# WHU-USI3DV/LaneMapping

Hardware: AMD Instinct MI355X
Metric: BEV tiles/sec end-to-end (LAS points -> polylines) (higher is better)
Workload: dtype f32; 1 GPU; on-GPU LAS->BEV raster (4,194,304 points/tile resident in HBM) + configs/Proj_polyline_fpn_vit_vertex_2.py, batch=16 per GPU, seeded random weights; lines_per_tile=45, streams=2, hip_graphs=True, points=resident, stream_check=not run (--full runs it), gather_check=n/a (1 rank), raster_check=not run (--full runs it), dist_ranks=1, rccl_ranks=1

## Files before the change

### include/lanemap_hip.h

```cpp
#ifndef LANEMAP_HIP_H
#define LANEMAP_HIP_H
#include <stdint.h>
#ifdef __cplusplus
extern "C" {
#endif

enum { LM_OK = 0, LM_ERR_ARG = 1, LM_ERR_HIP = 2, LM_ERR_NO_DEVICE = 3, LM_ERR_CAPACITY = 4 };
enum { LM_ACT_NONE = 0, LM_ACT_RELU = 1, LM_ACT_GELU = 2 };

int lm_abi_version(void);
const char* lm_last_error(void);
int lm_device_count(void);

int lm_conv2d_nhwc_mfma_f32(void* stream, const float* x, int ldx, const float* wp, int CoutP,
                            const float* scale, const float* shift, const float* res, int ldr, int res_rows,
                            float* y, int ldy, int B, int H, int W, int Cin, int Cout, int KH, int KW,
                            int stride, int pad_h, int pad_w, int dil, int act);
int lm_conv2d_nhwc_mfma_resup_f32(void* stream, const float* x, int ldx, const float* wp, int CoutP, const float* scale,
                                  const float* shift, const float* res_coarse, int ldr, int Hr, int Wr, float* y, int ldy,
                                  int B, int H, int W, int Cin, int Cout, int KH, int KW, int stride, int pad_h, int pad_w,
                                  int dil, int act);

int lm_winograd44_supported(int H, int W, int Cin, int dil);
int lm_winograd44_gn_chunks(int H, int W, int dil);
long lm_winograd44_tiles(int B, int H, int W, int dil);
long lm_winograd44_twin_workspace_bytes(int B, int H, int W, int Cin, int CoutP, int dil);
int lm_conv3x3_winograd44_f32(void* stream, const float* x, int ldx, const float* wu_frag, int CoutP, const float* scale,
                              const float* shift, const float* res, int ldr, float* y, int ldy, int B, int H, int W,
                              int Cin, int Cout, int dil, int act, double* gn_partial);
int lm_conv3x3_winograd44_twin_f32(void* stream, const float* x, int ldx, const float* wu, int CoutP, const float* scale,
                                   const float* shift, const float* res, int ldr, float* y, int ldy, int B, int H, int W,
                                   int Cin, int Cout, int dil, int act, void* workspace, long workspace_bytes);
int lm_wino44_split_fragments(void* stream, const float* frag, float* out, long n_quads);
int lm_conv3x3_winograd44_split_f32(void* stream, const float* x, int ldx, const float* wu_split, int CoutP, const float* scale,
                                    const float* shift, const float* res, int ldr, float* y, int ldy, int B, int H, int W,
                                    int Cin, int Cout, int dil, int act, double* gn_partial, float post);
int lm_conv3x3_winograd44_split_twin_f32(void* stream, const float* x, int ldx, const float* wu, int CoutP, const float* scale,
                                         const float* shift, const float* res, int ldr, float* y, int ldy, int B, int H, int W,
                                         int Cin, int Cout, int dil, int act, void* workspace, long workspace_bytes, float post);

int lm_conv2d_nhwc_mfma_f32_gnstats(void* stream, const float* x, int ldx, const float* wp, int CoutP, const float* shift,
                                    float* y, int ldy, double* gn_partial, int B, int H, int W, int Cin, int Cout,
                                    int KH, int KW, int stride, int pad_h, int pad_w, int dil);
int lm_gn_finalize(void* stream, const double* partial, float* stats, int B, int HW, int C, int nchunk, float eps);
int lm_gn_finalize_split(void* stream, const double* partial, float* stats, int B, int HW, int C, int nchunk, float eps, int split);

int lm_stem_conv7x7_bn_relu(void* stream, const float* x_chw, const float* w_k64, const float* scale,
                            const float* shift, float* y_nhwc, int B, int H, int W);
int lm_stem_conv7x7_bn_relu_u8(void* stream, const unsigned char* x_hwc3, const float* w_k64, const float* scale,
                               const float* shift, float* y_nhwc, int B, int H, int W);
int lm_maxpool3x3s2_nhwc(void* stream, const float* x, float* y, int B, int H, int W, int C);
int lm_conv2d_nhwc_small(void* stream, const float* x, int ldx, const float* w_tc16, const float* scale,
                         const float* shift, float* y, int ldy, int B, int H, int W, int Cin, int Cout,
                         int KH, int KW, int stride, int pad_h, int pad_w, int pre_relu, int act);

int lm_gn_stats(void* stream, const float* x, double* workspace, float* stats, int B, int HW, int C, float eps);
long lm_gn_stats_workspace_bytes(int B, int HW, int C);
int lm_gn_relu_upsample(void* stream, const float* x, const float* stats, const float* gamma, const float* beta,
                        float* y, int B, int Hi, int Wi, int Ho, int Wo, int C, int accumulate);
int lm_gn_relu_upsample_sum(void* stream, int n, const float* const* x, const float* const* stats, const int* Hi, const int* Wi,
                            const int* ldx , const float* gamma, const float* beta,
                            float* y, int B, int Ho, int Wo, int C);
int lm_gn_relu_upsample_sum_conv1x1(void* stream, int n, const float* const* x, const float* const* stats, const int* Hi, const int* Wi,
                                    const int* ldx, const float* gamma, const float* beta, float* y, int B, int Ho, int Wo, int C,
                                    const float* w_c16, const float* bias, int cout, float* y1, int ldy1);
int lm_upsample_bilinear_nhwc(void* stream, const float* x, int ldx, const float* add, int lda, float* y, int ldy,
                              int B, int Hi, int Wi, int Ho, int Wo, int C);
int lm_upsample_bilinear_to_chw(void* stream, const float* x, int ldx, float* y_chw, int B, int Hi, int Wi,
                                int Ho, int Wo, int C);
int lm_layernorm_rows(void* stream, const float* x, const float* gamma, const float* beta, float* y,
                      long rows, int D, float eps);
int lm_unpatchify(void* stream, const float* tokens, float* y_nhwc, int B, int G, int P, int C);
int lm_token_mix_mfma_f32(void* stream, const float* x, const float* wt, int ldw, const float* bias, const float* res, float* y,
                          int B, int M, int K, int N, int act);

int lm_attention_f32(void* stream, const float* qkv, float* out, int B, int N, int heads, int dim_head, float scale);
int lm_attention_masked_f32(void* stream, const float* qkv, float* out, const int* valid, int B, int N, int heads, int dim_head, float scale);

int lm_head_tokens(void* stream, const float* seg, const float* row_nhwc16, float* tok, float seg_bias,
                   int B, int P, int Hr, int Wr, int prop_width, int half_buff);
int lm_head_tokens_window(void* stream, const float* row_nhwc16, float* tok, int B, int P, int Hr, int Wr, int prop_width, int half_buff);
int lm_head_stage2(void* stream, const float* hid, int ldh, int D, const float* w2, const float* b2,
                   float* ext2, float* cls2, float* off2, long M);
int lm_head_proposal_conf(void* stream, const float* tok, const float* wt, const float* bias, float* conf,
                          int BP, int L);

int lm_decode_proposals(void* stream, const float* pconf, const float* ext2, const float* cls2, const float* off2,
                        float* prop_conf, float* v_ext, float* cls_conf, int* cls_idx, double* cls_offset,
                        int B, int P, int R, float exist_thre, int prop_width, int half_buff);
int lm_decode_orient(void* stream, const float* x_nhwc, int ldx, int C, unsigned char* y, long pixels);
int lm_decode_semantic(void* stream, const float* logit_chw3, unsigned char* sem, float* biseg, float* rows,
                       int B, int H, int W, float thre, int raw_mode);
long lm_endp_topk_workspace_bytes(int B);
int lm_endp_topk(void* stream, const float* endp_logit, void* workspace, int* out_idx, float* out_score,
                 int* out_status, int B, int H, int W, int clip, int K);

int lm_pack_segments(void* stream, int n, const void* const* src, const long* bytes, const long* dst_offsets, void* dst);


typedef struct {
    float quat[4];
    float trans[3];
    float bev_img_offset[2];
    float img_reso[2];
    float local_min_ele;
    float ele_reso;
    float inten_lo, inten_hi;
} LmRasterParams;
long lm_bev_raster_workspace_bytes(int B, long max_points_per_tile, int H, int W);
int lm_bev_raster_batch(void* stream, const float* points_xyzi, const long* tile_offsets, const LmRasterParams* params,
                        int B, void* workspace, long workspace_bytes, float* out_chw, unsigned char* out_hwc_u8,
                        int H, int W);
int lm_tile_ingest_u8(void* stream, const unsigned char* src_hwc, float* dst_chw, int B, int H, int W, int C);

typedef struct {
    double x0, y0, cell;
    int nx, ny;
} LmStripGrid;
int lm_strip_build_grid(const LmRasterParams* params, int T, int H, int W, double z_lo, double z_hi, LmStripGrid* grid,
                        unsigned short* cells, long cells_cap);
long lm_strip_bin_workspace_bytes(long N, int T);
int lm_strip_bin_points(void* hip_stream, const float* points_xyzi, long N, const LmRasterParams* params, int T, int H, int W,
                        double z_lo, double z_hi, void* workspace, long workspace_bytes, long* counts, long* offsets,
                        long* offsets_host, float* binned, long capacity);

int lm_endp_cluster(const int* topk_idx, int n_avail, int Wc, int clip, int k0, int k_step, int k_max, int radius,
                    int min_clusters, int* out_hw, int max_out, int* n_out, int* k_used);
int lm_polyline_assemble(const float* prop_conf, const float* prop_v_ext, const double* cls_offset,
                         const float* bi_seg_rows, const int* endp_hw, int n_endp, int P, int R, float obj_thre,
                         int min_vertices, double* out_lanes, int* endp_keep);
int lm_raster_polylines(const double* lanes, int P, int R, unsigned char* out);
int lm_line8(unsigned char* out, int x1, int y1, int x2, int y2, int colour);
int lm_trace_lines(const double* cols, int n, int R, const float* seg_rows, double* out);
int lm_polyline_backproject(unsigned char* bev_hwc, int H, int W, int C, const double* img_seqs, const int* seq_lens, int L,
                            int Vmax, const double* params13, const double* las_read_offset, double* out);

long lm_skeletonize_lee_2d(unsigned char* img, int H, int W);

void* lm_merge_create(void);
void lm_merge_destroy(void* merger);
int lm_merge_add_tile(void* merger, const double* points, const int* lens, int n);
long lm_merge_finish(void* merger, long* total_points);
int lm_merge_result(void* merger, double* points, int* lens);
int lm_downsample_seq(const double* seq, int n, double dist_min, double* out);

int lm_softmax_rows(void* stream, float* x, long rows, int cols);
int lm_rowref_select(void* stream, const float* ext, const float* cls, float* mean_out, int* valid, float thr_ext, int* corr,
                     int B, int H, int W, int L);
int lm_rowref_gather(void* stream, const float* x_nhwc8, const int* corr, float* tok, int B, int H, int W, int L);
int lm_rowref_scatter(void* stream, const float* x_nhwc8, const float* tok, const int* corr, const int* valid,
                      float* y_nhwc8, int B, int H, int W, int L);
int lm_rowref_decode(void* stream, const float* ext2, const float* cls2, unsigned char* conf, unsigned char* cls_map,
                     int* col_idx, int B, int H, int W, int L);

long lm_voxelize_workspace_bytes(long n_points);
long lm_scan_workspace_bytes(long n);
int lm_exclusive_scan_u32(void* stream, const unsigned* in, unsigned* out, long n, void* workspace, long workspace_bytes);
long lm_sort_pairs_workspace_bytes(long n);
int lm_sort_pairs_u32(void* stream, unsigned* keys_io, unsigned* vals_io, long n, int end_bit, void* workspace, long workspace_bytes);
int lm_voxelize_hard(void* stream, const float* points, long n, const float* range_lo_xyz, const float* voxel_size_xyz,
                     const int* grid_xyz, int max_points, int max_voxels, int batch_idx, const int* row_base, int cap_rows,
                     float* feats, int ldf, int* coords, int* row_end, int raster_order, void* workspace,
                     long workspace_bytes);
int lm_sparse_grid_build(void* stream, const int* coords, long n, int* grid, int B, int D, int H, int W);
long lm_sparse_conv_outputs_workspace_bytes(long out_cells);
int lm_sparse_conv_outputs(void* stream, const int* in_coords, long n_in, int B, const int* ksp_zyx9, int Do, int Ho, int Wo,
                           int* out_grid, int* out_coords, int cap_rows, int* out_count, void* workspace, long workspace_bytes);
int lm_sparse_rulebook(void* stream, const int* out_coords, long n_out, const int* in_grid, int B, int D, int H, int W,
                       const int* ksp_zyx9, int* nbr);
int lm_conv_gather_mfma_f32(void* stream, const float* x, int ldx, const int* nbr, int taps, const float* wp, int CoutP,
                            const float* scale, const float* shift, const float* res, int ldr, float* y, int ldy,
                            long M, int Cin, int Cout, int act);
int lm_sparse_to_dense_nhwc(void* stream, const float* feats, int ldf, const int* coords, long n, float* out, int B, int D,
                            int H, int W, int C, int flip_h);
int lm_upsample_bicubic_nhwc(void* stream, const float* x, float* y, int B, int H, int W, int C, int Ho, int Wo);

typedef struct {
    int version_major, version_minor, point_format, record_len;
    long n_points, offset_to_points;
    double scale[3], offset[3], min_xyz[3], max_xyz[3];
} LmLasHeader;
int lm_las_parse_header(const unsigned char* bytes, long len, LmLasHeader* out);
int lm_las_decode_points(void* stream, const unsigned char* records, int record_len, long n, const double* scale,
                         const double* offset, const double* shift, float inten_lo, float inten_hi, int normalise,
                         float* out_xyzi);

int lm_png_info(const unsigned char* data, long size, int* H, int* W, int* C);
int lm_png_decode_u8(const unsigned char* data, long size, unsigned char* out_hwc, long out_bytes);
int lm_png_decode_files_u8(const char* const* paths, int n, unsigned char* out_nhwc, int H, int W, int C, int threads);
int lm_zlib_inflate(const unsigned char* data, long size, unsigned char* out, long capacity, long* produced);

long lm_lane_json_text(const double* lane_vertexes, int n_lines, int row_size, int with_pervertex_semantics, char* out, long cap);
int lm_lane_json_write(const double* lane_vertexes, int n_lines, int row_size, int with_pervertex_semantics, const char* path);
int lm_seqs_json_write(const double* seqs, const int* lens, int L, int Vmax, int D, const char* path);

#ifdef __cplusplus
}
#endif
#endif
```

### lanemapping_amd/_lib.py

```python
import ctypes as C
import os

_HERE = os.path.dirname(os.path.abspath(__file__))
LIB_PATH = os.environ.get('LANEMAP_HIP_LIB') or os.path.join(_HERE, 'liblanemap_hip.so')

c_f32p = C.POINTER(C.c_float)
vp, i32, i64, f32 = C.c_void_p, C.c_int, C.c_long, C.c_float


class LmRasterParams(C.Structure):
    _fields_ = [('quat', C.c_float * 4), ('trans', C.c_float * 3), ('bev_img_offset', C.c_float * 2),
                ('img_reso', C.c_float * 2), ('local_min_ele', C.c_float), ('ele_reso', C.c_float),
                ('inten_lo', C.c_float), ('inten_hi', C.c_float)]


class LmLasHeader(C.Structure):
    _fields_ = [('version_major', C.c_int), ('version_minor', C.c_int), ('point_format', C.c_int), ('record_len', C.c_int),
                ('n_points', C.c_long), ('offset_to_points', C.c_long), ('scale', C.c_double * 3), ('offset', C.c_double * 3),
                ('min_xyz', C.c_double * 3), ('max_xyz', C.c_double * 3)]


class LmStripGrid(C.Structure):
    _fields_ = [('x0', C.c_double), ('y0', C.c_double), ('cell', C.c_double), ('nx', C.c_int), ('ny', C.c_int)]


SIGNATURES = {
    'lm_abi_version': (i32, []),
    'lm_last_error': (C.c_char_p, []),
    'lm_device_count': (i32, []),
    'lm_conv2d_nhwc_mfma_f32': (i32, [vp, vp, i32, vp, i32, vp, vp, vp, i32, i32, vp, i32,
                                      i32, i32, i32, i32, i32, i32, i32, i32, i32, i32, i32, i32]),
    'lm_conv2d_nhwc_mfma_resup_f32': (i32, [vp, vp, i32, vp, i32, vp, vp, vp, i32, i32, i32, vp, i32,
                                            i32, i32, i32, i32, i32, i32, i32, i32, i32, i32, i32, i32]),
    'lm_winograd44_supported': (i32, [i32, i32, i32, i32]),
    'lm_winograd44_gn_chunks': (i32, [i32, i32, i32]),
    'lm_winograd44_tiles': (i64, [i32, i32, i32, i32]),
    'lm_winograd44_twin_workspace_bytes': (i64, [i32, i32, i32, i32, i32, i32]),
    'lm_conv3x3_winograd44_f32': (i32, [vp, vp, i32, vp, i32, vp, vp, vp, i32, vp, i32, i32, i32, i32, i32, i32, i32, i32, vp]),
    'lm_conv3x3_winograd44_twin_f32': (i32, [vp, vp, i32, vp, i32, vp, vp, vp, i32, vp, i32, i32, i32, i32, i32, i32, i32, i32, vp, i64]),
    'lm_wino44_split_fragments': (i32, [vp, vp, vp, i64]),
    'lm_conv3x3_winograd44_split_f32': (i32, [vp, vp, i32, vp, i32, vp, vp, vp, i32, vp, i32, i32, i32, i32, i32, i32, i32, i32, vp, f32]),
    'lm_conv3x3_winograd44_split_twin_f32': (i32, [vp, vp, i32, vp, i32, vp, vp, vp, i32, vp, i32, i32, i32, i32, i32, i32, i32, i32, vp, i64, f32]),
    'lm_conv2d_nhwc_mfma_f32_gnstats': (i32, [vp, vp, i32, vp, i32, vp, vp, i32, vp] + [i32] * 11),
    'lm_gn_finalize': (i32, [vp, vp, vp, i32, i32, i32, i32, f32]),
    'lm_gn_finalize_split': (i32, [vp, vp, vp, i32, i32, i32, i32, f32, i32]),
    'lm_stem_conv7x7_bn_relu': (i32, [vp, vp, vp, vp, vp, vp, i32, i32, i32]),
    'lm_stem_conv7x7_bn_relu_u8': (i32, [vp, vp, vp, vp, vp, vp, i32, i32, i32]),
    'lm_maxpool3x3s2_nhwc': (i32, [vp, vp, vp, i32, i32, i32, i32]),
    'lm_conv2d_nhwc_small': (i32, [vp, vp, i32, vp, vp, vp, vp, i32, i32, i32, i32, i32, i32, i32, i32, i32, i32, i32, i32, i32]),
    'lm_gn_stats': (i32, [vp, vp, vp, vp, i32, i32, i32, f32]),
    'lm_gn_stats_workspace_bytes': (i64, [i32, i32, i32]),
    'lm_gn_relu_upsample': (i32, [vp, vp, vp, vp, vp, vp, i32, i32, i32, i32, i32, i32, i32]),
    'lm_gn_relu_upsample_sum': (i32, [vp, i32, vp, vp, vp, vp, vp, vp, vp, vp, i32, i32, i32, i32]),
    'lm_gn_relu_upsample_sum_conv1x1': (i32, [vp, i32, vp, vp, vp, vp, vp, vp, vp, vp, i32, i32, i32, i32, vp, vp, i32, vp, i32]),
    'lm_upsample_bilinear_nhwc': (i32, [vp, vp, i32, vp, i32, vp, i32, i32, i32, i32, i32, i32, i32]),
    'lm_upsample_bilinear_to_chw': (i32, [vp, vp, i32, vp, i32, i32, i32, i32, i32, i32]),
    'lm_layernorm_rows': (i32, [vp, vp, vp, vp, vp, i64, i32, f32]),
    'lm_token_mix_mfma_f32': (i32, [vp, vp, vp, i32, vp, vp, vp, i32, i32, i32, i32, i32]),
    'lm_unpatchify': (i32, [vp, vp, vp, i32, i32, i32, i32]),
    'lm_attention_f32': (i32, [vp, vp, vp, i32, i32, i32, i32, f32]),
    'lm_attention_masked_f32': (i32, [vp, vp, vp, vp, i32, i32, i32, i32, f32]),
    'lm_head_tokens': (i32, [vp, vp, vp, vp, f32, i32, i32, i32, i32, i32, i32]),
    'lm_head_tokens_window': (i32, [vp, vp, vp, i32, i32, i32, i32, i32, i32]),
    'lm_head_stage2': (i32, [vp, vp, i32, i32, vp, vp, vp, vp, vp, i64]),
    'lm_head_proposal_conf': (i32, [vp, vp, vp, vp, vp, i32, i32]),
    'lm_decode_proposals': (i32, [vp, vp, vp, vp, vp, vp, vp, vp, vp, vp, i32, i32, i32, f32, i32, i32]),
    'lm_decode_orient': (i32, [vp, vp, i32, i32, vp, i64]),
    'lm_decode_semantic': (i32, [vp, vp, vp, vp, vp, i32, i32, i32, f32, i32]),
    'lm_endp_topk_workspace_bytes': (i64, [i32]),
    'lm_endp_topk': (i32, [vp, vp, vp, vp, vp, vp, i32, i32, i32, i32, i32]),
    'lm_pack_segments': (i32, [vp, i32, vp, vp, vp, vp]),
    'lm_bev_raster_workspace_bytes': (i64, [i32, i64, i32, i32]),
    'lm_bev_raster_batch': (i32, [vp, vp, C.POINTER(i64), C.POINTER(LmRasterParams), i32, vp, i64, vp, vp, i32, i32]),
    'lm_tile_ingest_u8': (i32, [vp, vp, vp, i32, i32, i32, i32]),
    'lm_strip_build_grid': (i32, [C.POINTER(LmRasterParams), i32, i32, i32, C.c_double, C.c_double, C.POINTER(LmStripGrid), vp, i64]),
    'lm_strip_bin_workspace_bytes': (i64, [i64, i32]),
    'lm_strip_bin_points': (i32, [vp, vp, i64, C.POINTER(LmRasterParams), i32, i32, i32, C.c_double, C.c_double, vp, i64, vp, vp,
                                  C.POINTER(i64), vp, i64]),
    'lm_endp_cluster': (i32, [vp, i32, i32, i32, i32, i32, i32, i32, i32, vp, i32, vp, vp]),
    'lm_polyline_assemble': (i32, [vp, vp, vp, vp, vp, i32, i32, i32, f32, i32, vp, vp]),
    'lm_raster_polylines': (i32, [vp, i32, i32, vp]),
    'lm_line8': (i32, [vp, i32, i32, i32, i32, i32]),
    'lm_trace_lines': (i32, [vp, i32, i32, vp, vp]),
    'lm_polyline_backproject': (i32, [vp, i32, i32, i32, vp, vp, i32, i32, vp, vp, vp]),
    'lm_skeletonize_lee_2d': (i64, [vp, i32, i32]),
    'lm_merge_create': (vp, []),
    'lm_merge_destroy': (None, [vp]),
    'lm_merge_add_tile': (i32, [vp, vp, vp, i32]),
    'lm_merge_finish': (i64, [vp, C.POINTER(i64)]),
    'lm_merge_result': (i32, [vp, vp, vp]),
    'lm_downsample_seq': (i32, [vp, i32, C.c_double, vp]),
    'lm_softmax_rows': (i32, [vp, vp, i64, i32]),
    'lm_rowref_select': (i32, [vp, vp, vp, vp, vp, f32, vp, i32, i32, i32, i32]),
    'lm_rowref_gather': (i32, [vp, vp, vp, vp, i32, i32, i32, i32]),
    'lm_rowref_scatter': (i32, [vp, vp, vp, vp, vp, vp, i32, i32, i32, i32]),
    'lm_rowref_decode': (i32, [vp, vp, vp, vp, vp, vp, i32, i32, i32, i32]),
    'lm_voxelize_workspace_bytes': (i64, [i64]),
    'lm_scan_workspace_bytes': (i64, [i64]),
    'lm_exclusive_scan_u32': (i32, [vp, vp, vp, i64, vp, i64]),
    'lm_sort_pairs_workspace_bytes': (i64, [i64]),
    'lm_sort_pairs_u32': (i32, [vp, vp, vp, i64, i32, vp, i64]),
    'lm_voxelize_hard': (i32, [vp, vp, i64, c_f32p, c_f32p, C.POINTER(i32), i32, i32, i32, vp, i32, vp, i32, vp, vp, i32, vp, i64]),
    'lm_sparse_grid_build': (i32, [vp, vp, i64, vp, i32, i32, i32, i32]),
    'lm_sparse_conv_outputs_workspace_bytes': (i64, [i64]),
    'lm_sparse_conv_outputs': (i32, [vp, vp, i64, i32, C.POINTER(i32), i32, i32, i32, vp, vp, i32, vp, vp, i64]),
    'lm_sparse_rulebook': (i32, [vp, vp, i64, vp, i32, i32, i32, i32, C.POINTER(i32), vp]),
    'lm_conv_gather_mfma_f32': (i32, [vp, vp, i32, vp, i32, vp, i32, vp, vp, vp, i32, vp, i32, i64, i32, i32, i32]),
    'lm_sparse_to_dense_nhwc': (i32, [vp, vp, i32, vp, i64, vp, i32, i32, i32, i32, i32, i32]),
    'lm_upsample_bicubic_nhwc': (i32, [vp, vp, vp, i32, i32, i32, i32, i32, i32]),
    'lm_las_parse_header': (i32, [vp, i64, C.POINTER(LmLasHeader)]),
    'lm_las_decode_points': (i32, [vp, vp, i32, i64, C.POINTER(C.c_double), C.POINTER(C.c_double), C.POINTER(C.c_double), f32, f32,
                                   i32, vp]),
    'lm_png_info': (i32, [vp, i64, C.POINTER(i32), C.POINTER(i32), C.POINTER(i32)]),
    'lm_png_decode_u8': (i32, [vp, i64, vp, i64]),
    'lm_png_decode_files_u8': (i32, [C.POINTER(C.c_char_p), i32, vp, i32, i32, i32, i32]),
    'lm_zlib_inflate': (i32, [vp, i64, vp, i64, C.POINTER(i64)]),
    'lm_lane_json_text': (i64, [vp, i32, i32, i32, vp, i64]),
    'lm_lane_json_write': (i32, [vp, i32, i32, i32, C.c_char_p]),
    'lm_seqs_json_write': (i32, [vp, vp, i32, i32, i32, C.c_char_p]),
}

_lib = None


class LanemapHipError(RuntimeError):
    pass


def lib():
    global _lib
    if _lib is None:
        if not os.path.exists(LIB_PATH):
            raise LanemapHipError(
                f'{LIB_PATH} is missing: the HIP library is the only implementation of this package '
                '(no CPU fallback). Build it with `python -m lanemapping_amd.build`.')
        import torch
        L = C.CDLL(LIB_PATH)
        for name, (res, args) in SIGNATURES.items():
            fn = getattr(L, name)
            fn.restype = res
            fn.argtypes = args
        _lib = L
    return _lib


def check(code):
    if code != 0:
        raise LanemapHipError(f'lanemap_hip error {code}: {lib().lm_last_error().decode()}')
```

### lanemapping_amd/csrc/common.h

```cpp
#pragma once
#include <hip/hip_runtime.h>
#include <cstdarg>
#include <cstdint>
#include <cstdio>

#define LM_API extern "C" __attribute__((visibility("default")))

enum {
    LM_OK = 0,
    LM_ERR_ARG = 1,
    LM_ERR_HIP = 2,
    LM_ERR_NO_DEVICE = 3,
    LM_ERR_CAPACITY = 4
};

void lm_set_error(const char* fmt, ...);
int lm_ensure_dynamic_lds(const void* kernel, size_t bytes);

#define LM_REQUIRE(cond, ...)            \
    do {                                 \
        if (!(cond)) {                   \
            lm_set_error(__VA_ARGS__);   \
            return LM_ERR_ARG;           \
        }                                \
    } while (0)

#define LM_HIP(expr)                                                                  \
    do {                                                                              \
        hipError_t e_ = (expr);                                                       \
        if (e_ != hipSuccess) {                                                       \
            lm_set_error("%s failed: %s (%s:%d)", #expr, hipGetErrorString(e_), __FILE__, __LINE__); \
            return LM_ERR_HIP;                                                        \
        }                                                                             \
    } while (0)

#define LM_LAUNCH_CHECK() LM_HIP(hipGetLastError())

static inline int lm_cdiv(long a, long b) { return (int)((a + b - 1) / b); }

enum { LM_ACT_NONE = 0, LM_ACT_RELU = 1, LM_ACT_GELU = 2 };

#ifdef __HIPCC__
__device__ __forceinline__ void lm_bilin_axis_scaled(int o, int in, float scale, int& i0, int& i1, float& w0, float& w1) {
#pragma clang fp contract(off)
    const float src = scale * (float)o;
    i0 = (int)src;
    if (i0 > in - 1) i0 = in - 1;
    i1 = i0 + ((i0 < in - 1) ? 1 : 0);
    w1 = fminf(fmaxf(src - (float)i0, 0.f), 1.f);
    w0 = 1.f - w1;
}
__device__ __forceinline__ void lm_bilin_axis(int o, int in, int out, int& i0, int& i1, float& w0, float& w1) {
#pragma clang fp contract(off)
    const float scale = (out > 1) ? (float)(in - 1) / (float)(out - 1) : 0.f;
    lm_bilin_axis_scaled(o, in, scale, i0, i1, w0, w1);
}
#endif
struct LmFastDiv {
    unsigned d, mul, sh;
};
static inline LmFastDiv lm_fastdiv_make(unsigned d) {
    LmFastDiv f;
    f.d = d;
    f.sh = 0;
    while ((1ull << f.sh) < d) ++f.sh;
    f.mul = (unsigned)((((1ull << f.sh) - d) << 32) / d + 1);
    return f;
}
#ifdef __HIPCC__
__device__ __forceinline__ unsigned lm_fastdiv(unsigned n, const LmFastDiv& f) { return (__umulhi(n, f.mul) + n) >> f.sh; }
__device__ __forceinline__ void lm_gn_affine(float mean, float rstd, float gamma, float beta, float& a, float& g) {
#pragma clang fp contract(off)
    a = rstd * gamma;
    g = __builtin_fmaf(-mean, a, beta);
}
__device__ __forceinline__ float lm_gn_relu(float v, float a, float g) { return fmaxf(__builtin_fmaf(v, a, g), 0.f); }
__device__ __forceinline__ float lm_bilerp(float v00, float v01, float v10, float v11, float wy0, float wy1, float wx0, float wx1) {
#pragma clang fp contract(off)
    const float top = wx0 * v00 + wx1 * v01;
    const float bot = wx0 * v10 + wx1 * v11;
    return wy0 * top + wy1 * bot;
}
#endif
```

### lanemapping_amd/csrc/decode.hip

```cpp
#include "common.h"

#define LM_PACK_MAX_SEGMENTS 8

typedef float f32x4 __attribute__((ext_vector_type(4)));

namespace {

template <int N>
__device__ __forceinline__ int softmax_argmax(const float* in, float* out) {
    float m = in[0];
#pragma unroll
    for (int i = 1; i < N; ++i) m = fmaxf(m, in[i]);
    float s = 0.f;
#pragma unroll
    for (int i = 0; i < N; ++i) {
        out[i] = expf(in[i] - m);
        s += out[i];
    }
    int best = 0;
#pragma unroll
    for (int i = 0; i < N; ++i) {
        out[i] = out[i] / s;
        if (out[i] > out[best]) best = i;
    }
    return best;
}

template <int FW>
__global__ __launch_bounds__(256) void decode_proposals_kernel(
    const float* __restrict__ pconf, const float* __restrict__ ext2, const float* __restrict__ cls2,
    const float* __restrict__ off2, float* __restrict__ prop_conf, float* __restrict__ v_ext,
    float* __restrict__ cls_conf, int* __restrict__ cls_idx, double* __restrict__ cls_offset, int P, int R,
    float exist_thre, int prop_width, int half_buff, long total) {
    const long i = (long)blockIdx.x * 256 + threadIdx.x;
    if (i >= total) return;
    const int h = (int)(i % R);
    const long bp = i / R;
    const int p = (int)(bp % P);
    if (h == 0) {
        float o[2];
        softmax_argmax<2>(pconf + bp * 2, o);
        prop_conf[bp * 2] = o[0];
        prop_conf[bp * 2 + 1] = o[1];
    }
    float e[3];
    softmax_argmax<3>(ext2 + i * 3, e);
    float v = 0.f;
    if (e[1] > e[2] && e[1] > exist_thre) v = 1.f;
    if (e[2] > e[1] && e[2] > exist_thre) v = 2.f;
    v_ext[i] = v;
    float c[FW];
    const int idx = softmax_argmax<FW>(cls2 + i * FW, c);
#pragma unroll
    for (int k = 0; k < FW; ++k) cls_conf[i * FW + k] = c[k];
    cls_idx[i] = idx;
    const float fsum = (float)idx + off2[i * FW + idx];
    double co = (double)fsum;
    if (co > (double)FW) co = (double)FW;
    cls_offset[i] = co + (double)(prop_width * p - half_buff);
}

__global__ __launch_bounds__(256) void decode_orient_kernel(const float* __restrict__ x, int ldx, int C,
                                                            unsigned char* __restrict__ y, long total) {
    const long i = (long)blockIdx.x * 256 + threadIdx.x;
    if (i >= total) return;
    const float* xp = x + i * ldx;
    int best = 0;
    float bv = xp[0];
    for (int c = 1; c < C; ++c) {
        const float v = xp[c];
        if (v > bv) {
            bv = v;
            best = c;
        }
    }
    y[i] = (unsigned char)best;
}

__global__ __launch_bounds__(256) void decode_semantic_kernel(const float* __restrict__ logit, unsigned char* __restrict__ sem,
                                                              float* __restrict__ biseg, float* __restrict__ rows, int H, int W,
                                                              float thre, int raw_mode, long total) {
    const long i = (long)blockIdx.x * 256 + threadIdx.x;
    if (i >= total) return;
    const long HW = (long)H * W;
    const long b = i / HW, r = i - b * HW;
    const float* lp = logit + b * 3 * HW + r;
    const float l0 = lp[0], l1 = lp[HW], l2 = lp[2 * HW];
    float s1, s2;
    if (raw_mode) {
        s1 = l1;
        s2 = l2;
    } else {
        const float m = fmaxf(l0, fmaxf(l1, l2));
        const float e0 = expf(l0 - m), e1 = expf(l1 - m), e2 = expf(l2 - m);
        const float s = (e0 + e1) + e2;
        s1 = e1 / s;
        s2 = e2 / s;
    }
    unsigned char c = 0;
    if (s1 > s2 && s1 > thre) c = 1;
    if (s2 > s1 && s2 > thre) c = 2;
    sem[i] = c;
    if (biseg) {
        const float bs = s1 + s2;
        biseg[i] = bs;
        const int y = (int)(r / W);
        if (rows && (y & 7) == 3) rows[(b * (H / 8) + (y >> 3)) * W + (r - (long)y * W)] = bs;
    }
}

constexpr int NB = 1024;
constexpr int CAP = 4096;
struct TopkParams {
    const float* logit;
    unsigned* hist;
    unsigned* cand_cnt;
    unsigned long long* cand;
    int H, W, clip, K;
    LmFastDiv div_wc;
};

__device__ __forceinline__ unsigned score_key(float logit) {
    const float s = 1.0f / (1.0f + expf(-logit));
    return __float_as_uint(s);
}

__device__ __forceinline__ unsigned level_bin(unsigned key, int level) {
    return level == 0 ? (key >> 20) : (level == 1 ? ((key >> 10) & 1023u) : (key & 1023u));
}

__device__ void pick_bin_block(const unsigned* h, unsigned& need, unsigned& bin, unsigned* tmp) {
    const int t = threadIdx.x;
    unsigned c[4] = {0u, 0u, 0u, 0u}, s = 0;
    if (t < 256) {
        const uint4 v = *reinterpret_cast<const uint4*>(h + 4 * t);
        c[0] = v.x; c[1] = v.y; c[2] = v.z; c[3] = v.w;
        s = v.x + v.y + v.z + v.w;
        tmp[t] = s;
    }
    if (t == 0) {
        tmp[256] = need == 0 ? (unsigned)(NB - 1) : 0u;
        tmp[257] = 0u;
    }
    __syncthreads();
    for (int off = 1; off < 256; off <<= 1) {
        unsigned add = 0;
        if (t + off < 256) add = tmp[t + off];
        __syncthreads();
        if (t < 256) tmp[t] += add;
        __syncthreads();
    }
    if (t < 256 && need > 0) {
        const unsigned incl = tmp[t], above = incl - s;
        if (above < need && incl >= need) {
            unsigned acc = above;
#pragma unroll
            for (int k = 3; k >= 0; --k) {
                if (acc + c[k] >= need) {
                    tmp[256] = (unsigned)(4 * t + k);
                    tmp[257] = need - acc;
                    break;
                }
                acc += c[k];
            }
        }
    }
    __syncthreads();
    bin = tmp[256];
    need = tmp[257];
    __syncthreads();
}

__global__ __launch_bounds__(256) void zero_u32_kernel(unsigned* __restrict__ p, long n) {
    const long i = (long)blockIdx.x * 256 + threadIdx.x;
    if (i < n) p[i] = 0u;
}

template <int LEVEL>
__global__ __launch_bounds__(256) void topk_pass_kernel(TopkParams p) {
    __shared__ unsigned lh[NB];
    __shared__ unsigned pb_tmp[258];
    const int b = blockIdx.y;
    const int Hc = p.H - 2 * p.clip, Wc = p.W - 2 * p.clip;
    const long n = (long)Hc * Wc;
    unsigned* hist = p.hist + (long)b * 3 * NB;
    if (LEVEL < 3)
        for (int i = threadIdx.x; i < NB; i += 256) lh[i] = 0;
    unsigned prefix = 0;
    bool take_ties = false;
    {
        unsigned need = (unsigned)p.K, bin = 0;
#pragma unroll
        for (int lv = 0; lv < LEVEL && lv < 3; ++lv) {
            pick_bin_block(hist + lv * NB, need, bin, pb_tmp);
            prefix |= bin << (20 - 10 * lv);
        }
        if (LEVEL == 3) take_ties = hist[2 * NB + bin] == need;
    }
    __syncthreads();
    const float* lp = p.logit + (long)b * p.H * p.W;
    for (long i = (long)blockIdx.x * 256 + threadIdx.x; i < n; i += (long)gridDim.x * 256) {
        const int y = (int)lm_fastdiv((unsigned)i, p.div_wc), x = (int)((unsigned)i - (unsigned)y * (unsigned)Wc);
        const unsigned key = score_key(lp[(long)(y + p.clip) * p.W + x + p.clip]);
        if (LEVEL == 0) {
            atomicAdd(&lh[key >> 20], 1u);
        } else if (LEVEL == 1) {
            if ((key >> 20) == (prefix >> 20)) atomicAdd(&lh[(key >> 10) & 1023u], 1u);
        } else if (LEVEL == 2) {
            if ((key >> 10) == (prefix >> 10)) atomicAdd(&lh[key & 1023u], 1u);
        } else {
            if (key > prefix || (key == prefix && take_ties)) {
                const unsigned slot = atomicAdd(p.cand_cnt + b, 1u);
                if (slot < CAP) p.cand[(long)b * CAP + slot] = ((unsigned long long)key << 32) | (unsigned)(0xFFFFFFFFu - (unsigned)i);
            }
        }
    }
    if (LEVEL < 3) {
        __syncthreads();
        for (int i = threadIdx.x; i < NB; i += 256)
            if (lh[i]) atomicAdd(&hist[LEVEL * NB + i], lh[i]);
    }
}

__global__ __launch_bounds__(1024) void topk_ties_kernel(TopkParams p) {
    __shared__ unsigned sh[4];
    __shared__ unsigned wave_tot[16];
    const int b = blockIdx.x;
    const unsigned* hist = p.hist + (long)b * 3 * NB;
    __shared__ unsigned pb_tmp[258];
    unsigned need = (unsigned)p.K, bin = 0, T = 0;
#pragma unroll
    for (int lv = 0; lv < 3; ++lv) {
        pick_bin_block(hist + lv * NB, need, bin, pb_tmp);
        T |= bin << (20 - 10 * lv);
    }
    if (threadIdx.x == 0) sh[3] = p.cand_cnt[b];
    __syncthreads();
    const unsigned base = sh[3];
    if (hist[2 * NB + bin] == need || need == 0) return;
    const int Wc = p.W - 2 * p.clip;
    const long n = (long)(p.H - 2 * p.clip) * Wc;
    const float* lp = p.logit + (long)b * p.H * p.W;
    const int lane = threadIdx.x & 63, wave = threadIdx.x >> 6;
    unsigned taken = 0;
    for (long i0 = 0; i0 < n && taken < need; i0 += 1024) {
        const long i = i0 + threadIdx.x;
        bool tie = false;
        if (i < n) {
            const int y = (int)lm_fastdiv((unsigned)i, p.div_wc), x = (int)((unsigned)i - (unsigned)y * (unsigned)Wc);
            tie = score_key(lp[(long)(y + p.clip) * p.W + x + p.clip]) == T;
        }
        const unsigned long long m = __ballot(tie);
        const unsigned before = (unsigned)__popcll(m & ((1ull << lane) - 1ull));
        if (lane == 0) wave_tot[wave] = (unsigned)__popcll(m);
        __syncthreads();
        unsigned off = 0, tot = 0;
        for (int w = 0; w < 16; ++w) {
            if (w < wave) off += wave_tot[w];
            tot += wave_tot[w];
        }
        const unsigned rank = taken + off + before;
        if (tie && rank < need) p.cand[(long)b * CAP + base + rank] = ((unsigned long long)T << 32) | (unsigned)(0xFFFFFFFFu - (unsigned)i);
        taken += tot;
        __syncthreads();
    }
    if (threadIdx.x == 0) p.cand_cnt[b] = base + need;
}

__global__ __launch_bounds__(1024) void topk_sort_kernel(TopkParams p, int* __restrict__ out_idx, float* __restrict__ out_score,
                                                         int* __restrict__ out_status) {
    __shared__ unsigned long long v[CAP];
    const int b = blockIdx.x;
    const unsigned cnt = p.cand_cnt[b];
    const unsigned n = cnt < (unsigned)CAP ? cnt : (unsigned)CAP;
    for (int i = threadIdx.x; i < CAP; i += 1024) v[i] = (unsigned)i < n ? p.cand[(long)b * CAP + i] : 0ull;
    __syncthreads();
    for (int k = 2; k <= CAP; k <<= 1)
        for (int j = k >> 1; j > 0; j >>= 1) {
            for (int i = threadIdx.x; i < CAP; i += 1024) {
                const int l = i ^ j;
                if (l > i) {
                    const unsigned long long a = v[i], c = v[l];
                    const bool desc = (i & k) == 0;
                    if (desc ? (a < c) : (a > c)) {
                        v[i] = c;
                        v[l] = a;
                    }
                }
            }
            __syncthreads();
        }
    for (int i = threadIdx.x; i < p.K; i += 1024) {
        const unsigned long long e = v[i];
        const bool ok = (unsigned)i < n;
        out_idx[(long)b * p.K + i] = ok ? (int)(0xFFFFFFFFu - (unsigned)(e & 0xFFFFFFFFu)) : -1;
        out_score[(long)b * p.K + i] = ok ? __uint_as_float((unsigned)(e >> 32)) : 0.f;
    }
    if (threadIdx.x == 0) out_status[b] = (cnt > (unsigned)CAP) ? 1 : 0;
}


struct PackArgs {
    const void* src[LM_PACK_MAX_SEGMENTS];
    long offs[LM_PACK_MAX_SEGMENTS];
    long words[LM_PACK_MAX_SEGMENTS];
    long first_chunk[LM_PACK_MAX_SEGMENTS + 1];
    int n;
};

__global__ __launch_bounds__(256) void pack_segments_kernel(PackArgs a, unsigned char* __restrict__ dst) {
    const long c = (long)blockIdx.x * 256 + threadIdx.x;
    if (c >= a.first_chunk[a.n]) return;
    int s = 0;
#pragma unroll
    for (int k = 1; k < LM_PACK_MAX_SEGMENTS; ++k) s += (k < a.n && c >= a.first_chunk[k]) ? 1 : 0;
    const long w0 = (c - a.first_chunk[s]) * 4;
    const unsigned* src = static_cast<const unsigned*>(a.src[s]) + w0;
    unsigned* out = reinterpret_cast<unsigned*>(dst + a.offs[s]) + w0;
    const long left = a.words[s] - w0;
    if (left >= 4 && ((reinterpret_cast<unsigned long long>(src) & 15ull) == 0)) {
        *reinterpret_cast<uint4*>(out) = *reinterpret_cast<const uint4*>(src);
    } else {
        for (int e = 0; e < 4 && e < left; ++e) out[e] = src[e];
    }
}

}

LM_API int lm_decode_proposals(void* stream, const float* pconf, const float* ext2, const float* cls2, const float* off2,
                               float* prop_conf, float* v_ext, float* cls_conf, int* cls_idx, double* cls_offset,
                               int B, int P, int R, float exist_thre, int prop_width, int half_buff) {
    LM_REQUIRE(pconf && ext2 && cls2 && off2 && prop_conf && v_ext && cls_conf && cls_idx && cls_offset, "decode_proposals: null pointer");
    const int fw = prop_width + 2 * half_buff;
    LM_REQUIRE(fw == 10 || fw == 12 || fw == 16, "decode_proposals: prop_fea_width must be 10, 12 or 16 (got %d)", fw);
    const long total = (long)B * P * R;
    auto kernel = fw == 10 ? decode_proposals_kernel<10> : fw == 12 ? decode_proposals_kernel<12> : decode_proposals_kernel<16>;
    hipLaunchKernelGGL(kernel, dim3(lm_cdiv(total, 256)), dim3(256), 0, (hipStream_t)stream, pconf, ext2, cls2,
                       off2, prop_conf, v_ext, cls_conf, cls_idx, cls_offset, P, R, exist_thre, prop_width, half_buff, total);
    LM_LAUNCH_CHECK();
    return LM_OK;
}

LM_API int lm_decode_orient(void* stream, const float* x_nhwc, int ldx, int C, unsigned char* y, long pixels) {
    LM_REQUIRE(x_nhwc && y && C >= 1, "decode_orient: bad args");
    hipLaunchKernelGGL(decode_orient_kernel, dim3(lm_cdiv(pixels, 256)), dim3(256), 0, (hipStream_t)stream, x_nhwc, ldx, C, y, pixels);
    LM_LAUNCH_CHECK();
    return LM_OK;
}

LM_API int lm_decode_semantic(void* stream, const float* logit_chw3, unsigned char* sem, float* biseg, float* rows,
                              int B, int H, int W, float thre, int raw_mode) {
    LM_REQUIRE(logit_chw3 && sem, "decode_semantic: null pointer");
    LM_REQUIRE(!rows || H % 8 == 0, "decode_semantic: H must be a multiple of 8 for the row gather");
    const long total = (long)B * H * W;
    hipLaunchKernelGGL(decode_semantic_kernel, dim3(lm_cdiv(total, 256)), dim3(256), 0, (hipStream_t)stream, logit_chw3, sem,
                       biseg, rows, H, W, thre, raw_mode, total);
    LM_LAUNCH_CHECK();
    return LM_OK;
}

LM_API long lm_endp_topk_workspace_bytes(int B) {
    return (long)B * (3 * NB * sizeof(unsigned) + sizeof(unsigned) * 4 + (long)CAP * sizeof(unsigned long long));
}

LM_API int lm_endp_topk(void* stream, const float* endp_logit, void* workspace, int* out_idx, float* out_score,
                        int* out_status, int B, int H, int W, int clip, int K) {
    LM_REQUIRE(endp_logit && workspace && out_idx && out_score && out_status, "endp_topk: null pointer");
    LM_REQUIRE(K >= 1 && K <= CAP / 2 && H > 2 * clip && W > 2 * clip, "endp_topk: bad K=%d or crop", K);
    hipStream_t s = (hipStream_t)stream;
    TopkParams p;
    p.logit = endp_logit;
    char* ws = (char*)workspace;
    p.hist = (unsigned*)ws;
    p.cand_cnt = (unsigned*)(ws + (size_t)B * 3 * NB * sizeof(unsigned));
    p.cand = (unsigned long long*)(ws + (size_t)B * (3 * NB + 4) * sizeof(unsigned));
    p.H = H; p.W = W; p.clip = clip; p.K = K;
    LM_REQUIRE(W > 2 * clip && H > 2 * clip && (long)(H - 2 * clip) * (W - 2 * clip) < (1L << 31), "endp_topk: bad crop (H=%d W=%d clip=%d)", H, W, clip);
    p.div_wc = lm_fastdiv_make((unsigned)(W - 2 * clip));
    const long zero_words = (long)B * (3 * NB + 4);
    hipLaunchKernelGGL(zero_u32_kernel, dim3(lm_cdiv(zero_words, 256)), dim3(256), 0, s, (unsigned*)workspace, zero_words);
    LM_LAUNCH_CHECK();
    dim3 grid(256, B);
    hipLaunchKernelGGL(topk_pass_kernel<0>, grid, dim3(256), 0, s, p);
    LM_LAUNCH_CHECK();
    hipLaunchKernelGGL(topk_pass_kernel<1>, grid, dim3(256), 0, s, p);
    LM_LAUNCH_CHECK();
    hipLaunchKernelGGL(topk_pass_kernel<2>, grid, dim3(256), 0, s, p);
    LM_LAUNCH_CHECK();
    hipLaunchKernelGGL(topk_pass_kernel<3>, grid, dim3(256), 0, s, p);
    LM_LAUNCH_CHECK();
    hipLaunchKernelGGL(topk_ties_kernel, dim3(B), dim3(1024), 0, s, p);
    LM_LAUNCH_CHECK();
    hipLaunchKernelGGL(topk_sort_kernel, dim3(B), dim3(1024), 0, s, p, out_idx, out_score, out_status);
    LM_LAUNCH_CHECK();
    return LM_OK;
}

LM_API int lm_pack_segments(void* stream, int n, const void* const* src, const long* bytes, const long* dst_offsets, void* dst) {
    LM_REQUIRE(n >= 1 && n <= LM_PACK_MAX_SEGMENTS && src && bytes && dst_offsets && dst, "pack_segments: 1..%d segments", LM_PACK_MAX_SEGMENTS);
    PackArgs a;
    a.n = n;
    a.first_chunk[0] = 0;
    for (int s = 0; s < LM_PACK_MAX_SEGMENTS; ++s) {
        const bool on = s < n;
        LM_REQUIRE(!on || (src[s] && bytes[s] >= 0 && bytes[s] % 4 == 0 && dst_offsets[s] % 16 == 0), "pack_segments: segment %d: bytes %% 4, offset %% 16", s);
        a.src[s] = on ? src[s] : nullptr;
        a.offs[s] = on ? dst_offsets[s] : 0;
        a.words[s] = on ? bytes[s] / 4 : 0;
        a.first_chunk[s + 1] = a.first_chunk[s] + (a.words[s] + 3) / 4;
    }
    const long chunks = a.first_chunk[n];
    if (chunks == 0) return LM_OK;
    hipLaunchKernelGGL(pack_segments_kernel, dim3(lm_cdiv(chunks, 256)), dim3(256), 0, (hipStream_t)stream, a, static_cast<unsigned char*>(dst));
    LM_LAUNCH_CHECK();
    return LM_OK;
}
```

### lanemapping_amd/csrc/norm_resize.hip

```cpp
#include "common.h"

typedef float f32x4 __attribute__((ext_vector_type(4)));

namespace {

__device__ __forceinline__ void bilin_axis(int o, int in, int out, int& i0, int& i1, float& w0, float& w1) {
    lm_bilin_axis(o, in, out, i0, i1, w0, w1);
}

constexpr int GN_CHUNK = 512;

__global__ __launch_bounds__(256) void gn_partial_kernel(const float* __restrict__ x, double* __restrict__ part,
                                                         int HW, int C, int nchunk) {
    __shared__ double red[2][256];
    const int b = blockIdx.y, chunk = blockIdx.x;
    const int lanes_p = 256 / C;
    const int c = threadIdx.x % C, pl = threadIdx.x / C;
    const int p0 = chunk * GN_CHUNK;
    const int p1 = min(p0 + GN_CHUNK, HW);
    double s = 0.0, ss = 0.0;
    const float* xb = x + (long)b * HW * C;
    for (int p = p0 + pl; p < p1; p += lanes_p) {
        const double v = (double)xb[(long)p * C + c];
        s += v;
        ss += v * v;
    }
    red[0][threadIdx.x] = s;
    red[1][threadIdx.x] = ss;
    __syncthreads();
    if (pl == 0) {
        for (int q = 1; q < lanes_p; ++q) {
            s += red[0][q * C + c];
            ss += red[1][q * C + c];
        }
        double* o = part + (((long)b * nchunk + chunk) * C + c) * 2;
        o[0] = s;
        o[1] = ss;
    }
}

__global__ __launch_bounds__(256) void gn_final_kernel(const double* __restrict__ part, float* __restrict__ stats, int HW, int C,
                                                       int nchunk, float eps, int split) {
    __shared__ double red[2][8][32];
    const int b = blockIdx.y;
    const int cl = threadIdx.x & 31, kl = threadIdx.x >> 5;
    const int c = blockIdx.x * 32 + cl;
    double s = 0.0, ss = 0.0;
    if (c < C)
        for (int k = kl; k < nchunk; k += 8) {
            const double* o = part + (((long)b * nchunk + k) * C + c) * 2;
            s += o[0];
            ss += o[1];
        }
    red[0][kl][cl] = s;
    red[1][kl][cl] = ss;
    __syncthreads();
    if (kl == 0 && c < C) {
        for (int q = 1; q < 8; ++q) {
            s += red[0][q][cl];
            ss += red[1][q][cl];
        }
        const double mean = s / HW;
        double var = ss / HW - mean * mean;
        if (var < 0.0) var = 0.0;
        const int cg = C / split, g = c / cg;
        float* o = stats + (((long)g * gridDim.y + b) * cg + (c - g * cg)) * 2;
        o[0] = (float)mean;
        o[1] = (float)(1.0 / sqrt(var + (double)eps));
    }
}

__global__ __launch_bounds__(256) void gn_relu_upsample_kernel(const float* __restrict__ x, const float* __restrict__ stats,
                                                               const float* __restrict__ gamma, const float* __restrict__ beta,
                                                               float* __restrict__ y, int Hi, int Wi, int Ho, int Wo, int C,
                                                               int accumulate, long total4) {
    const long i = (long)blockIdx.x * 256 + threadIdx.x;
    if (i >= total4) return;
    const int c4n = C / 4;
    const int c = (int)(i % c4n) * 4;
    long t = i / c4n;
    const int ox = (int)(t % Wo);
    t /= Wo;
    const int oy = (int)(t % Ho);
    const int b = (int)(t / Ho);
    int y0, y1, x0, x1;
    float wy0, wy1, wx0, wx1;
    bilin_axis(oy, Hi, Ho, y0, y1, wy0, wy1);
    bilin_axis(ox, Wi, Wo, x0, x1, wx0, wx1);
    f32x4 a, g;
    {
        const f32x4* st = reinterpret_cast<const f32x4*>(stats + ((long)b * C + c) * 2);
        const f32x4 s0 = st[0], s1 = st[1], gm = *reinterpret_cast<const f32x4*>(gamma + c), bt = *reinterpret_cast<const f32x4*>(beta + c);
        const float mean[4] = {s0[0], s0[2], s1[0], s1[2]}, rstd[4] = {s0[1], s0[3], s1[1], s1[3]};
#pragma unroll
        for (int e = 0; e < 4; ++e) {
            float ae, ge;
            lm_gn_affine(mean[e], rstd[e], gm[e], bt[e], ae, ge);
            a[e] = ae;
            g[e] = ge;
        }
    }
    const float* xb = x + (long)b * Hi * Wi * C + c;
    auto tap = [&](int yy, int xx) {
        f32x4 v = *reinterpret_cast<const f32x4*>(xb + ((long)yy * Wi + xx) * C);
#pragma unroll
        for (int e = 0; e < 4; ++e) v[e] = lm_gn_relu(v[e], a[e], g[e]);
        return v;
    };
    const f32x4 v00 = tap(y0, x0), v01 = tap(y0, x1), v10 = tap(y1, x0), v11 = tap(y1, x1);
    f32x4 o;
#pragma unroll
    for (int e = 0; e < 4; ++e) o[e] = lm_bilerp(v00[e], v01[e], v10[e], v11[e], wy0, wy1, wx0, wx1);
    f32x4* yp = reinterpret_cast<f32x4*>(y + i * 4);
    if (accumulate) {
        const f32x4 prev = *yp;
#pragma unroll
        for (int e = 0; e < 4; ++e) o[e] = prev[e] + o[e];
    }
    *yp = o;
}

struct GnTerm {
    const float* x;
    const float* stats;
    int Hi, Wi, ld;
    float sy, sx;
};
struct GnSum {
    GnTerm t[3];
    int n;
};

struct Proj1x1 {
    const float* w;
    const float* bias;
    float* y1;
    int cout, ldy1;
};

__device__ __forceinline__ f32x4 ld_quad(const float* base, unsigned elem) {
    return *reinterpret_cast<const f32x4*>(reinterpret_cast<const char*>(base) + (elem << 2));
}

template <int N, int SAME>
__global__ __launch_bounds__(256) void gn_relu_upsample_sum_kernel(GnSum P, const float* __restrict__ gamma, const float* __restrict__ beta,
                                                                   float* __restrict__ y, int Ho, int Wo, int C, int c4shift, Proj1x1 Q) {
    __shared__ __attribute__((aligned(16))) float wl[256 * 8];
    const unsigned c4n = (unsigned)C / 4;
    const unsigned j0 = blockIdx.x * 256u + threadIdx.x;
    const bool live = j0 < (unsigned)Wo * c4n;
    const unsigned j = live ? j0 : 0u;
    const int ox = c4shift >= 0 ? (int)(j >> c4shift) : (int)(j / c4n);
    const int c = (int)(j - (unsigned)ox * c4n) * 4;
    const int oy = (int)blockIdx.y, b = (int)blockIdx.z;
    const unsigned i = ((unsigned)(b * Ho + oy) * (unsigned)Wo) * c4n + j;
    const f32x4 gm = *reinterpret_cast<const f32x4*>(gamma + c), bt = *reinterpret_cast<const f32x4*>(beta + c);
    f32x4 st0[N], st1[N], tap[N][4];
    float wy0[N], wy1[N], wx0[N], wx1[N];
#pragma unroll
    for (int k = 0; k < N; ++k) {
        const GnTerm& T = P.t[k];
        const float* stb = T.stats + (long)b * C * 2;
        st0[k] = ld_quad(stb, (unsigned)(c * 2));
        st1[k] = ld_quad(stb, (unsigned)(c * 2 + 4));
        const float* xb = T.x + (long)b * T.Hi * T.Wi * T.ld;
        if ((SAME >> k) & 1) {
            tap[k][0] = ld_quad(xb, (unsigned)((oy * T.Wi + ox) * T.ld + c));
        } else {
            int y0, y1, x0, x1;
            lm_bilin_axis_scaled(oy, T.Hi, T.sy, y0, y1, wy0[k], wy1[k]);
            lm_bilin_axis_scaled(ox, T.Wi, T.sx, x0, x1, wx0[k], wx1[k]);
            tap[k][0] = ld_quad(xb, (unsigned)((y0 * T.Wi + x0) * T.ld + c));
            tap[k][1] = ld_quad(xb, (unsigned)((y0 * T.Wi + x1) * T.ld + c));
            tap[k][2] = ld_quad(xb, (unsigned)((y1 * T.Wi + x0) * T.ld + c));
            tap[k][3] = ld_quad(xb, (unsigned)((y1 * T.Wi + x1) * T.ld + c));
        }
    }
    if (Q.w) {
        for (int k = threadIdx.x; k < C * 8; k += 256) wl[k] = (k & 7) < Q.cout ? Q.w[(k >> 3) * 16 + (k & 7)] : 0.f;
        __syncthreads();
    }
    if (!live) return;
    f32x4 acc = {0.f, 0.f, 0.f, 0.f};
#pragma unroll
    for (int k = 0; k < N; ++k) {
        f32x4 a, g;
        const float mean[4] = {st0[k][0], st0[k][2], st1[k][0], st1[k][2]}, rstd[4] = {st0[k][1], st0[k][3], st1[k][1], st1[k][3]};
#pragma unroll
        for (int e = 0; e < 4; ++e) {
            float ae, ge;
            lm_gn_affine(mean[e], rstd[e], gm[e], bt[e], ae, ge);
            a[e] = ae;
            g[e] = ge;
        }
        f32x4 o;
        if ((SAME >> k) & 1) {
#pragma unroll
            for (int e = 0; e < 4; ++e) o[e] = lm_gn_relu(tap[k][0][e], a[e], g[e]);
        } else {
            f32x4 v[4];
#pragma unroll
            for (int q = 0; q < 4; ++q)
#pragma unroll
                for (int e = 0; e < 4; ++e) v[q][e] = lm_gn_relu(tap[k][q][e], a[e], g[e]);
#pragma unroll
            for (int e = 0; e < 4; ++e) o[e] = lm_bilerp(v[0][e], v[1][e], v[2][e], v[3][e], wy0[k], wy1[k], wx0[k], wx1[k]);
        }
        if (k == 0) {
            acc = o;
        } else {
#pragma unroll
            for (int e = 0; e < 4; ++e) acc[e] = acc[e] + o[e];
        }
    }
    if (y) *reinterpret_cast<f32x4*>(y + (long)i * 4) = acc;
    if (Q.w) {
        float part[8];
#pragma unroll
        for (int n = 0; n < 8; ++n) part[n] = 0.f;
#pragma unroll
        for (int e = 0; e < 4; ++e) {
            const f32x4 w0 = *reinterpret_cast<const f32x4*>(wl + (c + e) * 8), w1 = *reinterpret_cast<const f32x4*>(wl + (c + e) * 8 + 4);
#pragma unroll
            for (int n = 0; n < 4; ++n) {
                part[n] = fmaf(acc[e], w0[n], part[n]);
                part[4 + n] = fmaf(acc[e], w1[n], part[4 + n]);
            }
        }
        const int lane = threadIdx.x & 63;
#pragma unroll
        for (int half = 4, mask = 1; half >= 1; half >>= 1, mask <<= 1) {
            const bool upper = (lane & mask) != 0;
#pragma unroll
            for (int jj = 0; jj < half; ++jj) {
                float lo = part[jj], hi = part[jj + half];
                asm volatile("" : "+v"(lo), "+v"(hi));
                const float send = upper ? lo : hi, keep = upper ? hi : lo;
                part[jj] = keep + __shfl_xor(send, mask);
            }
        }
        for (unsigned o = 8; o < c4n; o <<= 1) part[0] += __shfl_xor(part[0], (int)o);
        const unsigned li = (unsigned)c >> 2;
        const int n = 4 * (int)(li & 1) + 2 * (int)((li >> 1) & 1) + (int)((li >> 2) & 1);
        if (li < 8 && n < Q.cout) Q.y1[(long)((b * Ho + oy) * Wo + ox) * Q.ldy1 + n] = part[0] + (Q.bias ? Q.bias[n] : 0.f);
    }
}

constexpr int UT_R = 8, UT_C = 16;

__global__ __launch_bounds__(256) void gn_relu_up_lds_kernel(GnTerm T, const float* __restrict__ gamma, const float* __restrict__ beta,
                                                             float* __restrict__ y, int Ho, int Wo, int C, int SR, int SC) {
    extern __shared__ __attribute__((aligned(16))) float ups[];
    __shared__ int ty0[UT_R], ty1[UT_R], tx0[UT_C], tx1[UT_C];
    __shared__ float twy0[UT_R], twy1[UT_R], twx0[UT_C], twx1[UT_C];
    const int tid = threadIdx.x, c4n = C / 4;
    const int oy0 = blockIdx.y * UT_R, ox0 = blockIdx.x * UT_C, b = blockIdx.z;
    const int ny = min(UT_R, Ho - oy0), nx = min(UT_C, Wo - ox0);
    int sy0, sx0, i1;
    float w0, w1;
    lm_bilin_axis_scaled(oy0, T.Hi, T.sy, sy0, i1, w0, w1);
    lm_bilin_axis_scaled(ox0, T.Wi, T.sx, sx0, i1, w0, w1);
    if (tid < UT_R) {
        int a0, a1;
        lm_bilin_axis_scaled(min(oy0 + tid, Ho - 1), T.Hi, T.sy, a0, a1, w0, w1);
        ty0[tid] = a0 - sy0; ty1[tid] = a1 - sy0; twy0[tid] = w0; twy1[tid] = w1;
    } else if (tid >= 64 && tid < 64 + UT_C) {
        const int t = tid - 64;
        int a0, a1;
        lm_bilin_axis_scaled(min(ox0 + t, Wo - 1), T.Wi, T.sx, a0, a1, w0, w1);
        tx0[t] = a0 - sx0; tx1[t] = a1 - sx0; twx0[t] = w0; twx1[t] = w1;
    }
    const int cq = tid % c4n, pstep = 256 / c4n, p0 = tid / c4n;
    const int c = cq * 4;
    f32x4 a, g;
    {
        const f32x4 gm = *reinterpret_cast<const f32x4*>(gamma + c), bt = *reinterpret_cast<const f32x4*>(beta + c);
        const f32x4* st = reinterpret_cast<const f32x4*>(T.stats + ((long)b * C + c) * 2);
        const f32x4 st0 = st[0], st1 = st[1];
        const float mean[4] = {st0[0], st0[2], st1[0], st1[2]}, rstd[4] = {st0[1], st0[3], st1[1], st1[3]};
#pragma unroll
        for (int e = 0; e < 4; ++e) {
            float ae, ge;
            lm_gn_affine(mean[e], rstd[e], gm[e], bt[e], ae, ge);
            a[e] = ae;
            g[e] = ge;
        }
    }
    const int nsrc = SR * SC;
    const float* xb = T.x + (long)b * T.Hi * T.Wi * T.ld + c;
    constexpr int UNR = 4;
    for (int pb = p0; pb < nsrc; pb += pstep * UNR) {
        f32x4 v[UNR];
#pragma unroll
        for (int u = 0; u < UNR; ++u) {
            const int pp = pb + u * pstep;
            const int r = pp / SC, q = pp - r * SC;
            const int yy = min(sy0 + r, T.Hi - 1), xx = min(sx0 + q, T.Wi - 1);
            if (pp < nsrc) v[u] = *reinterpret_cast<const f32x4*>(xb + ((long)yy * T.Wi + xx) * T.ld);
        }
#pragma unroll
        for (int u = 0; u < UNR; ++u) {
            const int pp = pb + u * pstep;
            if (pp < nsrc) {
                f32x4 o;
#pragma unroll
                for (int e = 0; e < 4; ++e) o[e] = lm_gn_relu(v[u][e], a[e], g[e]);
                *reinterpret_cast<f32x4*>(ups + (long)pp * C + c) = o;
            }
        }
    }
    __syncthreads();
    const long obase = ((long)b * Ho + oy0) * Wo + ox0;
    for (int pp = p0; pp < UT_R * UT_C; pp += pstep) {
        const int r = pp / UT_C, q = pp % UT_C;
        if (r >= ny || q >= nx) continue;
        const float* s0 = ups + (long)(ty0[r] * SC) * C + c;
        const float* s1 = ups + (long)(ty1[r] * SC) * C + c;
        const f32x4 v00 = *reinterpret_cast<const f32x4*>(s0 + tx0[q] * C), v01 = *reinterpret_cast<const f32x4*>(s0 + tx1[q] * C);
        const f32x4 v10 = *reinterpret_cast<const f32x4*>(s1 + tx0[q] * C), v11 = *reinterpret_cast<const f32x4*>(s1 + tx1[q] * C);
        const float wy0 = twy0[r], wy1 = twy1[r], wx0 = twx0[q], wx1 = twx1[q];
        f32x4 o;
#pragma unroll
        for (int e = 0; e < 4; ++e) o[e] = lm_bilerp(v00[e], v01[e], v10[e], v11[e], wy0, wy1, wx0, wx1);
        __builtin_nontemporal_store(o, reinterpret_cast<f32x4*>(y + (obase + (long)r * Wo + q) * C + c));
    }
}

__global__ __launch_bounds__(256) void gn_sum3_lds_kernel(GnSum P, const float* __restrict__ gamma, const float* __restrict__ beta,
                                                          float* __restrict__ y, int Ho, int Wo, int C, int SR, int SC, Proj1x1 Q) {
    extern __shared__ __attribute__((aligned(16))) float ups[];
    __shared__ int ty0[UT_R], ty1[UT_R], tx0[UT_C], tx1[UT_C];
    __shared__ float twy0[UT_R], twy1[UT_R], twx0[UT_C], twx1[UT_C];
    const int tid = threadIdx.x, c4n = C / 4;
    const int oy0 = blockIdx.y * UT_R, ox0 = blockIdx.x * UT_C, b = blockIdx.z;
    const int ny = min(UT_R, Ho - oy0), nx = min(UT_C, Wo - ox0);
    const GnTerm& T0 = P.t[0];
    const GnTerm& T1 = P.t[1];
    const GnTerm& T2 = P.t[2];
    int sy0, sx0, i1;
    float w0, w1;
    lm_bilin_axis_scaled(oy0, T1.Hi, T1.sy, sy0, i1, w0, w1);
    lm_bilin_axis_scaled(ox0, T1.Wi, T1.sx, sx0, i1, w0, w1);
    if (tid < UT_R) {
        int a0, a1;
        lm_bilin_axis_scaled(min(oy0 + tid, Ho - 1), T1.Hi, T1.sy, a0, a1, w0, w1);
        ty0[tid] = a0 - sy0; ty1[tid] = a1 - sy0; twy0[tid] = w0; twy1[tid] = w1;
    } else if (tid >= 64 && tid < 64 + UT_C) {
        const int t = tid - 64;
        int a0, a1;
        lm_bilin_axis_scaled(min(ox0 + t, Wo - 1), T1.Wi, T1.sx, a0, a1, w0, w1);
        tx0[t] = a0 - sx0; tx1[t] = a1 - sx0; twx0[t] = w0; twx1[t] = w1;
    }
    const int cq = tid % c4n, pstep = 256 / c4n, p0 = tid / c4n;
    const int c = cq * 4;
    f32x4 a[3], g[3];
    {
        const f32x4 gm = *reinterpret_cast<const f32x4*>(gamma + c), bt = *reinterpret_cast<const f32x4*>(beta + c);
#pragma unroll
        for (int k = 0; k < 3; ++k) {
            const f32x4* st = reinterpret_cast<const f32x4*>(P.t[k].stats + ((long)b * C + c) * 2);
            const f32x4 st0 = st[0], st1 = st[1];
            const float mean[4] = {st0[0], st0[2], st1[0], st1[2]}, rstd[4] = {st0[1], st0[3], st1[1], st1[3]};
#pragma unroll
            for (int e = 0; e < 4; ++e) {
                float ae, ge;
                lm_gn_affine(mean[e], rstd[e], gm[e], bt[e], ae, ge);
                a[k][e] = ae;
                g[k][e] = ge;
            }
        }
    }
    float pw[4][8];
#pragma unroll
    for (int e = 0; e < 4; ++e)
#pragma unroll
        for (int n = 0; n < 8; ++n) pw[e][n] = n < Q.cout ? Q.w[(c + e) * 16 + n] : 0.f;
    const int nsrc = SR * SC;
    {
        const float* xb = T1.x + (long)b * T1.Hi * T1.Wi * T1.ld + c;
        constexpr int UNR = 4;
        for (int pb = p0; pb < nsrc; pb += pstep * UNR) {
            f32x4 v[UNR];
#pragma unroll
            for (int u = 0; u < UNR; ++u) {
                const int pp = pb + u * pstep;
                const int r = pp / SC, q = pp - r * SC;
                const int yy = min(sy0 + r, T1.Hi - 1), xx = min(sx0 + q, T1.Wi - 1);
                if (pp < nsrc) v[u] = *reinterpret_cast<const f32x4*>(xb + ((long)yy * T1.Wi + xx) * T1.ld);
            }
#pragma unroll
            for (int u = 0; u < UNR; ++u) {
                const int pp = pb + u * pstep;
                if (pp < nsrc) {
                    f32x4 o;
#pragma unroll
                    for (int e = 0; e < 4; ++e) o[e] = lm_gn_relu(v[u][e], a[1][e], g[1][e]);
                    *reinterpret_cast<f32x4*>(ups + (long)pp * C + c) = o;
                }
            }
        }
    }
    __syncthreads();
    const float* x0b = T0.x + (long)b * T0.Hi * T0.Wi * T0.ld + c;
    const float* x2b = T2.x + (long)b * T2.Hi * T2.Wi * T2.ld + c;
    const int lane = tid & 63;
    const unsigned li = (unsigned)cq;
    const int nsel = 4 * (int)(li & 1) + 2 * (int)((li >> 1) & 1) + (int)((li >> 2) & 1);
    const float pbias = (li < 8 && nsel < Q.cout && Q.bias) ? Q.bias[nsel] : 0.f;
    constexpr int UNR2 = 4;
    for (int pb = p0; pb < UT_R * UT_C; pb += pstep * UNR2) {
        f32x4 t0[UNR2], t2[UNR2];
        bool live[UNR2];
        int rr[UNR2], qq[UNR2];
#pragma unroll
        for (int u = 0; u < UNR2; ++u) {
            const int pp = pb + u * pstep;
            rr[u] = pp / UT_C; qq[u] = pp % UT_C;
            live[u] = rr[u] < ny && qq[u] < nx;
            const int oy = min(oy0 + rr[u], Ho - 1), ox = min(ox0 + qq[u], Wo - 1);
            t0[u] = *reinterpret_cast<const f32x4*>(x0b + ((long)oy * T0.Wi + ox) * T0.ld);
            t2[u] = *reinterpret_cast<const f32x4*>(x2b + ((long)oy * T2.Wi + ox) * T2.ld);
        }
#pragma unroll
        for (int u = 0; u < UNR2; ++u) {
            const int r = min(rr[u], UT_R - 1), q = qq[u];
            const float* s0 = ups + (long)(ty0[r] * SC) * C + c;
            const float* s1 = ups + (long)(ty1[r] * SC) * C + c;
            const f32x4 v00 = *reinterpret_cast<const f32x4*>(s0 + tx0[q] * C), v01 = *reinterpret_cast<const f32x4*>(s0 + tx1[q] * C);
            const f32x4 v10 = *reinterpret_cast<const f32x4*>(s1 + tx0[q] * C), v11 = *reinterpret_cast<const f32x4*>(s1 + tx1[q] * C);
            const float wy0 = twy0[r], wy1 = twy1[r], wx0 = twx0[q], wx1 = twx1[q];
            f32x4 acc;
#pragma unroll
            for (int e = 0; e < 4; ++e) {
#pragma clang fp contract(off)
                const float o0 = lm_gn_relu(t0[u][e], a[0][e], g[0][e]);
                const float o1 = lm_bilerp(v00[e], v01[e], v10[e], v11[e], wy0, wy1, wx0, wx1);
                const float o2 = lm_gn_relu(t2[u][e], a[2][e], g[2][e]);
                acc[e] = (o0 + o1) + o2;
            }
            const long opix = ((long)b * Ho + oy0 + rr[u]) * Wo + ox0 + qq[u];
            if (y && live[u]) *reinterpret_cast<f32x4*>(y + opix * C + c) = acc;
            float part[8];
#pragma unroll
            for (int n = 0; n < 8; ++n) part[n] = 0.f;
#pragma unroll
            for (int e = 0; e < 4; ++e)
#pragma unroll
                for (int n = 0; n < 8; ++n) part[n] = fmaf(acc[e], pw[e][n], part[n]);
#pragma unroll
            for (int half = 4, mask = 1; half >= 1; half >>= 1, mask <<= 1) {
                const bool upper = (lane & mask) != 0;
#pragma unroll
                for (int jj = 0; jj < half; ++jj) {
                    float lo = part[jj], hi = part[jj + half];
                    asm volatile("" : "+v"(lo), "+v"(hi));
                    const float send = upper ? lo : hi, keep = upper ? hi : lo;
                    part[jj] = keep + __shfl_xor(send, mask);
                }
            }
            for (unsigned o = 8; o < (unsigned)c4n; o <<= 1) part[0] += __shfl_xor(part[0], (int)o);
            if (live[u] && li < 8 && nsel < Q.cout) Q.y1[opix * Q.ldy1 + nsel] = part[0] + pbias;
        }
    }
}

__global__ __launch_bounds__(256) void upsample_nhwc_kernel(const float* __restrict__ x, int ldx, const float* __restrict__ add, int lda,
                                                            float* __restrict__ y, int ldy, int Hi, int Wi, int Ho, int Wo,
                                                            int C, long total4) {
    const long i = (long)blockIdx.x * 256 + threadIdx.x;
    if (i >= total4) return;
    const int c4n = C / 4;
    const int c = (int)(i % c4n) * 4;
    long t = i / c4n;
    const int ox = (int)(t % Wo);
    t /= Wo;
    const int oy = (int)(t % Ho);
    const int b = (int)(t / Ho);
    int y0, y1, x0, x1;
    float wy0, wy1, wx0, wx1;
    bilin_axis(oy, Hi, Ho, y0, y1, wy0, wy1);
    bilin_axis(ox, Wi, Wo, x0, x1, wx0, wx1);
    const float* xb = x + (long)b * Hi * Wi * ldx + c;
    const f32x4 v00 = *reinterpret_cast<const f32x4*>(xb + ((long)y0 * Wi + x0) * ldx);
    const f32x4 v01 = *reinterpret_cast<const f32x4*>(xb + ((long)y0 * Wi + x1) * ldx);
    const f32x4 v10 = *reinterpret_cast<const f32x4*>(xb + ((long)y1 * Wi + x0) * ldx);
    const f32x4 v11 = *reinterpret_cast<const f32x4*>(xb + ((long)y1 * Wi + x1) * ldx);
    const long opix = ((long)b * Ho + oy) * Wo + ox;
    f32x4 o;
#pragma unroll
    for (int e = 0; e < 4; ++e) o[e] = lm_bilerp(v00[e], v01[e], v10[e], v11[e], wy0, wy1, wx0, wx1);
    if (add) {
        const f32x4 r = *reinterpret_cast<const f32x4*>(add + opix * lda + c);
#pragma unroll
        for (int e = 0; e < 4; ++e) o[e] = o[e] + r[e];
    }
    *reinterpret_cast<f32x4*>(y + opix * ldy + c) = o;
}

__device__ __forceinline__ float upsample_blend(float v00, float v01, float v10, float v11, float wy0, float wy1, float wx0, float wx1) {
    return lm_bilerp(v00, v01, v10, v11, wy0, wy1, wx0, wx1);
}

__global__ __launch_bounds__(256) void upsample_to_chw_kernel(const float* __restrict__ x, int ldx, float* __restrict__ y,
                                                              int Hi, int Wi, int Ho, int Wo, int C, long total) {
    const long i = (long)blockIdx.x * 256 + threadIdx.x;
    if (i >= total) return;
    const int ox = (int)(i % Wo);
    long t = i / Wo;
    const int oy = (int)(t % Ho);
    t /= Ho;
    const int c = (int)(t % C);
    const int b = (int)(t / C);
    int y0, y1, x0, x1;
    float wy0, wy1, wx0, wx1;
    bilin_axis(oy, Hi, Ho, y0, y1, wy0, wy1);
    bilin_axis(ox, Wi, Wo, x0, x1, wx0, wx1);
    const float* xb = x + (long)b * Hi * Wi * ldx + c;
    const float v00 = xb[((long)y0 * Wi + x0) * ldx], v01 = xb[((long)y0 * Wi + x1) * ldx];
    const float v10 = xb[((long)y1 * Wi + x0) * ldx], v11 = xb[((long)y1 * Wi + x1) * ldx];
    y[i] = upsample_blend(v00, v01, v10, v11, wy0, wy1, wx0, wx1);
}

__global__ __launch_bounds__(256) void upsample_to_chw4_kernel(const float* __restrict__ x, int ldx, float* __restrict__ y,
                                                               int Hi, int Wi, int Ho, int Wo, int C, unsigned total4) {
    const unsigned i = blockIdx.x * 256u + threadIdx.x;
    if (i >= total4) return;
    const unsigned wq = (unsigned)Wo / 4;
    const int ox0 = (int)(i % wq) * 4;
    unsigned t = i / wq;
    const int oy = (int)(t % (unsigned)Ho);
    t /= (unsigned)Ho;
    const int c = (int)(t % (unsigned)C);
    const int b = (int)(t / (unsigned)C);
    int y0, y1;
    float wy0, wy1;
    bilin_axis(oy, Hi, Ho, y0, y1, wy0, wy1);
    const float* xb = x + (long)b * Hi * Wi * ldx + c;
    const float* r0 = xb + (long)y0 * Wi * ldx;
    const float* r1 = xb + (long)y1 * Wi * ldx;
    f32x4 o;
#pragma unroll
    for (int k = 0; k < 4; ++k) {
        int x0, x1;
        float wx0, wx1;
        bilin_axis(ox0 + k, Wi, Wo, x0, x1, wx0, wx1);
        const float v00 = r0[(long)x0 * ldx], v01 = r0[(long)x1 * ldx], v10 = r1[(long)x0 * ldx], v11 = r1[(long)x1 * ldx];
        o[k] = upsample_blend(v00, v01, v10, v11, wy0, wy1, wx0, wx1);
    }
    *reinterpret_cast<f32x4*>(y + (long)i * 4) = o;
}

template <int PER>
__global__ __launch_bounds__(256) void layernorm_kernel(const float* __restrict__ x, const float* __restrict__ gamma,
                                                        const float* __restrict__ beta, float* __restrict__ y, long rows,
                                                        float eps) {
    constexpr int D = PER * 64;
    const long row = (long)blockIdx.x * 4 + (threadIdx.x >> 6);
    if (row >= rows) return;
    const int lane = threadIdx.x & 63;
    const float* xr = x + row * D;
    float v[PER];
    float s = 0.f;
#pragma unroll
    for (int k = 0; k < PER; ++k) {
        v[k] = xr[k * 64 + lane];
        s += v[k];
    }
    for (int o = 32; o > 0; o >>= 1) s += __shfl_xor(s, o);
    const float mean = s / (float)D;
    float q = 0.f;
#pragma unroll
    for (int k = 0; k < PER; ++k) {
        const float d = v[k] - mean;
        q += d * d;
    }
    for (int o = 32; o > 0; o >>= 1) q += __shfl_xor(q, o);
    const float rstd = 1.0f / sqrtf(q / (float)D + eps);
    float* yr = y + row * D;
#pragma unroll
    for (int k = 0; k < PER; ++k) {
        const int c = k * 64 + lane;
        yr[c] = (v[k] - mean) * rstd * gamma[c] + beta[c];
    }
}

template <int PER>
__global__ __launch_bounds__(256) void layernorm_masked_kernel(const float* __restrict__ x, const float* __restrict__ gamma,
                                                               const float* __restrict__ beta, float* __restrict__ y, long rows, int D,
                                                               float eps) {
    const long row = (long)blockIdx.x * 4 + (threadIdx.x >> 6);
    if (row >= rows) return;
    const int lane = threadIdx.x & 63;
    const float* xr = x + row * D;
    float v[PER];
    float s = 0.f;
#pragma unroll
    for (int k = 0; k < PER; ++k) {
        const int c = k * 64 + lane;
        v[k] = c < D ? xr[c] : 0.f;
        s += v[k];
    }
    for (int o = 32; o > 0; o >>= 1) s += __shfl_xor(s, o);
    const float mean = s / (float)D;
    float q = 0.f;
#pragma unroll
    for (int k = 0; k < PER; ++k) {
        const float d = k * 64 + lane < D ? v[k] - mean : 0.f;
        q += d * d;
    }
    for (int o = 32; o > 0; o >>= 1) q += __shfl_xor(q, o);
    const float rstd = 1.0f / sqrtf(q / (float)D + eps);
    float* yr = y + row * D;
#pragma unroll
    for (int k = 0; k < PER; ++k) {
        const int c = k * 64 + lane;
        if (c < D) yr[c] = (v[k] - mean) * rstd * gamma[c] + beta[c];
    }
}

__global__ __launch_bounds__(256) void unpatchify_kernel(const float* __restrict__ t, float* __restrict__ y, int G, int P,
                                                         int C, long total) {
    const long i = (long)blockIdx.x * 256 + threadIdx.x;
    if (i >= total) return;
    const int c = (int)(i % C);
    long r = i / C;
    const int xx = (int)(r % (G * P));
    r /= (G * P);
    const int yy = (int)(r % (G * P));
    const int b = (int)(r / (G * P));
    const int gh = yy / P, p1 = yy % P, gw = xx / P, p2 = xx % P;
    y[i] = t[((long)b * G * G + gh * G + gw) * (P * P * C) + (p1 * P + p2) * C + c];
}

}

LM_API int lm_gn_stats(void* stream, const float* x, double* workspace, float* stats, int B, int HW, int C, float eps) {
    LM_REQUIRE(x && workspace && stats, "gn_stats: null pointer");
    LM_REQUIRE(C <= 256 && 256 % C == 0, "gn_stats: C=%d must divide 256", C);
    const int nchunk = lm_cdiv(HW, GN_CHUNK);
    hipLaunchKernelGGL(gn_partial_kernel, dim3(nchunk, B), dim3(256), 0, (hipStream_t)stream, x, workspace, HW, C, nchunk);
    LM_LAUNCH_CHECK();
    hipLaunchKernelGGL(gn_final_kernel, dim3(lm_cdiv(C, 32), B), dim3(256), 0, (hipStream_t)stream, workspace, stats, HW, C, nchunk, eps, 1);
    LM_LAUNCH_CHECK();
    return LM_OK;
}

LM_API int lm_gn_finalize(void* stream, const double* partial, float* stats, int B, int HW, int C, int nchunk, float eps) {
    LM_REQUIRE(partial && stats && nchunk >= 1, "gn_finalize: bad args");
    hipLaunchKernelGGL(gn_final_kernel, dim3(lm_cdiv(C, 32), B), dim3(256), 0, (hipStream_t)stream, partial, stats, HW, C, nchunk, eps, 1);
    LM_LAUNCH_CHECK();
    return LM_OK;
}

LM_API int lm_gn_finalize_split(void* stream, const double* partial, float* stats, int B, int HW, int C, int nchunk, float eps, int split) {
    LM_REQUIRE(partial && stats && nchunk >= 1 && split >= 1 && C % split == 0, "gn_finalize_split: bad args (C=%d split=%d)", C, split);
    hipLaunchKernelGGL(gn_final_kernel, dim3(lm_cdiv(C, 32), B), dim3(256), 0, (hipStream_t)stream, partial, stats, HW, C, nchunk, eps, split);
    LM_LAUNCH_CHECK();
    return LM_OK;
}

LM_API long lm_gn_stats_workspace_bytes(int B, int HW, int C) {
    return (long)B * lm_cdiv(HW, GN_CHUNK) * C * 2 * (long)sizeof(double);
}

LM_API int lm_gn_relu_upsample(void* stream, const float* x, const float* stats, const float* gamma, const float* beta,
                               float* y, int B, int Hi, int Wi, int Ho, int Wo, int C, int accumulate) {
    LM_REQUIRE(x && stats && gamma && beta && y && C % 4 == 0, "gn_relu_upsample: bad args");
    const long total4 = (long)B * Ho * Wo * (C / 4);
    hipLaunchKernelGGL(gn_relu_upsample_kernel, dim3(lm_cdiv(total4, 256)), dim3(256), 0, (hipStream_t)stream,
                       x, stats, gamma, beta, y, Hi, Wi, Ho, Wo, C, accumulate, total4);
    LM_LAUNCH_CHECK();
    return LM_OK;
}

namespace {
int up_block_extent(int in, int out, int tile) {
#pragma clang fp contract(off)
    const float scale = (out > 1) ? (float)(in - 1) / (float)(out - 1) : 0.f;
    auto tap0 = [&](int o) {
        int i0 = (int)(scale * (float)o);
        return i0 > in - 1 ? in - 1 : i0;
    };
    int ext = 1;
    for (int o0 = 0; o0 < out; o0 += tile) {
        const int ol = (o0 + tile - 1 < out ? o0 + tile - 1 : out - 1);
        const int last0 = tap0(ol), last1 = last0 + (last0 < in - 1 ? 1 : 0);
        const int e = last1 - tap0(o0) + 1;
        if (e > ext) ext = e;
    }
    return ext;
}

int launch_gn_sum(void* stream, int n, const float* const* x, const float* const* stats, const int* Hi, const int* Wi, const int* ldx,
                  const float* gamma, const float* beta, float* y, int B, int Ho, int Wo, int C, Proj1x1 Q) {
    LM_REQUIRE(n >= 1 && n <= 3 && x && stats && Hi && Wi && gamma && beta && C > 0 && C % 4 == 0, "gn_relu_upsample_sum: bad args");
    const long total4 = (long)B * Ho * Wo * (C / 4);
    LM_REQUIRE(total4 > 0 && total4 < (1L << 31), "gn_relu_upsample_sum: %ld output quads do not fit 32-bit indices", total4);
    GnSum P;
    P.n = n;
    for (int k = 0; k < 3; ++k) {
        const int q = k < n ? k : 0;
        LM_REQUIRE(x[q] && stats[q] && Hi[q] > 0 && Wi[q] > 0, "gn_relu_upsample_sum: bad term %d", q);
        const int ld = ldx ? ldx[q] : C;
        LM_REQUIRE(ld >= C && ld % 4 == 0, "gn_relu_upsample_sum: bad leading dimension %d of term %d", ld, q);
        LM_REQUIRE((long)Hi[q] * Wi[q] * ld < (1L << 30), "gn_relu_upsample_sum: term %d: an image of %ld elements does not fit 32-bit byte offsets", q,
                   (long)Hi[q] * Wi[q] * ld);
        P.t[k] = GnTerm{x[q], stats[q], Hi[q], Wi[q], ld, Ho > 1 ? (float)(Hi[q] - 1) / (float)(Ho - 1) : 0.f,
                        Wo > 1 ? (float)(Wi[q] - 1) / (float)(Wo - 1) : 0.f};
    }
    const int c4n = C / 4;
    LM_REQUIRE(256 % c4n == 0 || !Q.w, "gn_relu_upsample_sum: the fused 1x1 projection needs C/4 = %d to divide 256", c4n);
    LM_REQUIRE(Ho <= 65535 && B <= 65535, "gn_relu_upsample_sum: grid too large");
    int c4shift = -1;
    for (int sft = 0; sft < 16; ++sft)
        if ((1 << sft) == c4n) c4shift = sft;
    int same = 0;
    for (int k = 0; k < n; ++k)
        if (Hi[k] == Ho && Wi[k] == Wo) same |= 1 << k;
    if (n == 1 && same == 0 && !Q.w && y && 256 % c4n == 0 && Hi[0] > 1 && Wi[0] > 1 && Ho >= 2 * Hi[0] - 1 && Wo >= 2 * Wi[0] - 1) {
        static const bool lds_up = [] { const char* e = getenv("LM_GN_UP_LDS"); return !e || atoi(e) != 0; }();
        const int SR = up_block_extent(Hi[0], Ho, UT_R), SC = up_block_extent(Wi[0], Wo, UT_C);
        const size_t lds = (size_t)SR * SC * C * sizeof(float);
        if (lds_up && lds <= 72 * 1024) {
            if (int e = lm_ensure_dynamic_lds((const void*)gn_relu_up_lds_kernel, lds)) return e;
            hipLaunchKernelGGL(gn_relu_up_lds_kernel, dim3((unsigned)lm_cdiv(Wo, UT_C), (unsigned)lm_cdiv(Ho, UT_R), (unsigned)B), dim3(256), lds,
                               (hipStream_t)stream, P.t[0], gamma, beta, y, Ho, Wo, C, SR, SC);
            LM_LAUNCH_CHECK();
            return LM_OK;
        }
    }
    if (n == 3 && same == 5 && Q.w && c4n >= 8 && c4n <= 64 && (c4n & (c4n - 1)) == 0 && Hi[1] > 1 && Wi[1] > 1 && Ho >= 2 * Hi[1] - 1 &&
        Wo >= 2 * Wi[1] - 1) {
        static const bool lds_sum = [] { const char* e = getenv("LM_GN_SUM_LDS"); return !e || atoi(e) != 0; }();
        const int SR = up_block_extent(Hi[1], Ho, UT_R), SC = up_block_extent(Wi[1], Wo, UT_C);
        const size_t lds = (size_t)SR * SC * C * sizeof(float);
        if (lds_sum && lds <= 64 * 1024) {
            if (int e = lm_ensure_dynamic_lds((const void*)gn_sum3_lds_kernel, lds)) return e;
            hipLaunchKernelGGL(gn_sum3_lds_kernel, dim3((unsigned)lm_cdiv(Wo, UT_C), (unsigned)lm_cdiv(Ho, UT_R), (unsigned)B), dim3(256), lds,
                               (hipStream_t)stream, P, gamma, beta, y, Ho, Wo, C, SR, SC, Q);
            LM_LAUNCH_CHECK();
            return LM_OK;
        }
    }
    const dim3 grid((unsigned)lm_cdiv((long)Wo * c4n, 256), (unsigned)Ho, (unsigned)B);
#define LM_GNS(NN, SS)                                                                                                           \
    case (NN) * 8 + (SS):                                                                                                        \
        hipLaunchKernelGGL((gn_relu_upsample_sum_kernel<NN, SS>), grid, dim3(256), 0, (hipStream_t)stream, P, gamma, beta, y, Ho, Wo, C, \
                           c4shift, Q);                                                                                         \
        break;
    switch (n * 8 + same) {
        LM_GNS(1, 0) LM_GNS(1, 1)
        LM_GNS(2, 0) LM_GNS(2, 1) LM_GNS(2, 2) LM_GNS(2, 3)
        LM_GNS(3, 0) LM_GNS(3, 1) LM_GNS(3, 2) LM_GNS(3, 3) LM_GNS(3, 4) LM_GNS(3, 5) LM_GNS(3, 6) LM_GNS(3, 7)
    }
#undef LM_GNS
    LM_LAUNCH_CHECK();
    return LM_OK;
}
}

LM_API int lm_gn_relu_upsample_sum(void* stream, int n, const float* const* x, const float* const* stats, const int* Hi, const int* Wi,
                                   const int* ldx, const float* gamma, const float* beta, float* y, int B, int Ho, int Wo, int C) {
    LM_REQUIRE(y, "gn_relu_upsample_sum: null output");
    return launch_gn_sum(stream, n, x, stats, Hi, Wi, ldx, gamma, beta, y, B, Ho, Wo, C, Proj1x1{nullptr, nullptr, nullptr, 0, 0});
}

LM_API int lm_gn_relu_upsample_sum_conv1x1(void* stream, int n, const float* const* x, const float* const* stats, const int* Hi,
                                           const int* Wi, const int* ldx, const float* gamma, const float* beta, float* y, int B, int Ho,
                                           int Wo, int C, const float* w_c16, const float* bias, int cout, float* y1, int ldy1) {
    LM_REQUIRE(w_c16 && y1 && cout >= 1 && cout <= 8 && ldy1 >= cout, "gn_relu_upsample_sum_conv1x1: bad projection (cout=%d)", cout);
    const int c4n = C / 4;
    LM_REQUIRE(C % 4 == 0 && c4n >= 8 && c4n <= 64 && (c4n & (c4n - 1)) == 0,
               "gn_relu_upsample_sum_conv1x1: C=%d: C/4 must be a power of two in [8, 64] (one pixel per wave segment)", C);
    return launch_gn_sum(stream, n, x, stats, Hi, Wi, ldx, gamma, beta, y, B, Ho, Wo, C, Proj1x1{w_c16, bias, y1, cout, ldy1});
}

LM_API int lm_upsample_bilinear_nhwc(void* stream, const float* x, int ldx, const float* add, int lda, float* y, int ldy,
                                     int B, int Hi, int Wi, int Ho, int Wo, int C) {
    LM_REQUIRE(x && y && C % 4 == 0 && ldx % 4 == 0 && ldy % 4 == 0 && (!add || lda % 4 == 0), "upsample_nhwc: bad args");
    const long total4 = (long)B * Ho * Wo * (C / 4);
    hipLaunchKernelGGL(upsample_nhwc_kernel, dim3(lm_cdiv(total4, 256)), dim3(256), 0, (hipStream_t)stream,
                       x, ldx, add, lda, y, ldy, Hi, Wi, Ho, Wo, C, total4);
    LM_LAUNCH_CHECK();
    return LM_OK;
}

LM_API int lm_upsample_bilinear_to_chw(void* stream, const float* x, int ldx, float* y, int B, int Hi, int Wi,
                                       int Ho, int Wo, int C) {
    LM_REQUIRE(x && y && C >= 1, "upsample_to_chw: bad args");
    const long total = (long)B * C * Ho * Wo;
    if (Wo % 4 == 0 && total / 4 < (1L << 31) && ((uintptr_t)y & 15) == 0) {
        hipLaunchKernelGGL(upsample_to_chw4_kernel, dim3(lm_cdiv(total / 4, 256)), dim3(256), 0, (hipStream_t)stream,
                           x, ldx, y, Hi, Wi, Ho, Wo, C, (unsigned)(total / 4));
        LM_LAUNCH_CHECK();
        return LM_OK;
    }
    hipLaunchKernelGGL(upsample_to_chw_kernel, dim3(lm_cdiv(total, 256)), dim3(256), 0, (hipStream_t)stream,
                       x, ldx, y, Hi, Wi, Ho, Wo, C, total);
    LM_LAUNCH_CHECK();
    return LM_OK;
}

LM_API int lm_layernorm_rows(void* stream, const float* x, const float* gamma, const float* beta, float* y,
                             long rows, int D, float eps) {
    LM_REQUIRE(x && gamma && beta && y && D >= 32 && D <= 4096 && D % 32 == 0 && D != 768,
               "layernorm: D=%d must be 512 or 1024, or another multiple of 32 in [32, 4096] except 768", D);
    const dim3 grid(lm_cdiv(rows, 4));
    hipStream_t s = (hipStream_t)stream;
    if (D == 512)
        hipLaunchKernelGGL(layernorm_kernel<8>, grid, dim3(256), 0, s, x, gamma, beta, y, rows, eps);
    else if (D == 1024)
        hipLaunchKernelGGL(layernorm_kernel<16>, grid, dim3(256), 0, s, x, gamma, beta, y, rows, eps);
#define LM_LN_MASKED(PER) else if (D <= PER * 64) hipLaunchKernelGGL(layernorm_masked_kernel<PER>, grid, dim3(256), 0, s, x, gamma, beta, y, rows, D, eps);
    LM_LN_MASKED(1) LM_LN_MASKED(2) LM_LN_MASKED(4) LM_LN_MASKED(8) LM_LN_MASKED(16) LM_LN_MASKED(32) LM_LN_MASKED(64)
#undef LM_LN_MASKED
    LM_LAUNCH_CHECK();
    return LM_OK;
}

LM_API int lm_unpatchify(void* stream, const float* tokens, float* y_nhwc, int B, int G, int P, int C) {
    LM_REQUIRE(tokens && y_nhwc, "unpatchify: null pointer");
    const long total = (long)B * G * P * G * P * C;
    hipLaunchKernelGGL(unpatchify_kernel, dim3(lm_cdiv(total, 256)), dim3(256), 0, (hipStream_t)stream, tokens, y_nhwc, G, P, C, total);
    LM_LAUNCH_CHECK();
    return LM_OK;
}
```

### lanemapping_amd/net.py

```python
import torch
import torch.nn as nn

from . import ops, trace
from .registry import NET, build_pcencoder, build_backbone, build_heads


@NET.register_module
class Detector1stage(nn.Module):
    def __init__(self, head_type='seg', loss_type='row_ce', cfg=None):
        super().__init__()
        self.cfg = cfg
        self.conv1 = nn.Conv2d(144, 144, 3, 3)
        self.pcencoder = build_pcencoder(cfg)
        self.backbone = build_backbone(cfg)
        self.heads = build_heads(cfg)
        self.head_type, self.loss_type = head_type, loss_type

    def forward_raw(self, batch):
        fused = hasattr(self.pcencoder, 'fpn') and self.cfg.heads.type == 'ColumnProposal2'
        col = None
        if fused:
            proj = batch['proj']
            B, H, W = (proj.shape[0], proj.shape[1], proj.shape[2]) if proj.dtype == torch.uint8 else (proj.shape[0], proj.shape[2], proj.shape[3])
            col = ops.new_act(B, 16, H // 4, W // 4, proj.device)
            with trace.stage('pcencoder'):
                fea, fea_up, bi_seg, endp_est = self.pcencoder.fpn(proj, fea_up_out=col[:, 8:16])
        else:
            with trace.stage('pcencoder'):
                fea, fea_up, bi_seg, endp_est = self.pcencoder(batch)
        if self.cfg.vit_seg == True:
            with trace.stage('backbone'):
                fea = self.backbone(fea)
        with trace.stage('heads'):
            if self.cfg.heads.type == 'RowSharNotReducRef':
                out = self.heads(fea)
            else:
                out = self.heads(fea, fea_up, endp_est, col=col) if fused else self.heads(fea, fea_up, endp_est)
        out['semantic_seg'] = bi_seg
        out['endp_est'] = endp_est
        return out

    def forward(self, batch, is_get_features=False, stack_local_global_features=False):
        if self.training:
            raise NotImplementedError('lanemapping_amd implements the inference hot path only (call .eval())')
        if is_get_features:
            raise NotImplementedError('is_get_features is not on the hot path')
        output = {}
        with torch.no_grad():
            out = self.forward_raw(batch)
            output.update(self.heads.get_exist_coor_endp_dict(out))
            output['lane_maps'] = self.heads.get_lane_map_numpy_with_label(
                output, batch, is_flip=self.cfg.flip_label, is_img=self.cfg.view, is_get_1_stage_result=False,
                is_gt_avai=self.cfg.is_gt_avai)
            if self.cfg.show_result:
                output['pred_maps'] = self.heads.get_lane_map_on_source_image(output, batch)
        return output


@NET.register_module
class Segmentor(nn.Module):
    def __init__(self, head_type='seg', loss_type='ce', cfg=None):
        super().__init__()
        self.cfg = cfg
        self.pcencoder = build_pcencoder(cfg)
        self.head_type, self.loss_type = head_type, loss_type

    def forward(self, batch):
        if self.training:
            raise NotImplementedError('lanemapping_amd implements the inference hot path only (call .eval())')
        with torch.no_grad():
            _, _, bi_seg, endp_est = self.pcencoder(batch)
            pred = {'seg': bi_seg, 'endp': endp_est}
            return dict(self.pcencoder.infer_validate(pred, seg_thre=self.cfg.seg_thre, endp_thre=self.cfg.endp_thre))
```

### lanemapping_amd/ops.py

```python
import ctypes as C
import math

import torch

from ._lib import lib, check, LmRasterParams, LmStripGrid, LanemapHipError

ACT_NONE, ACT_RELU, ACT_GELU = 0, 1, 2


def _stream():
    return C.c_void_p(torch._C._cuda_getCurrentRawStream(torch._C._cuda_getDevice()))


def _ptr(t):
    if t is None:
        return None
    if not t.is_cuda:
        raise LanemapHipError('lanemapping_amd ops need tensors on an MI355X (HIP) device; no CPU fallback exists')
    if t.device.index != torch._C._cuda_getDevice():
        raise LanemapHipError(f'tensor on cuda:{t.device.index} but the current device is cuda:{torch._C._cuda_getDevice()}: '
                              'call torch.cuda.set_device() (one process drives one GPU)')
    return C.c_void_p(t.data_ptr())


def new_act(B, C_, H, W, device, dtype=torch.float32):
    return torch.empty((B, H, W, C_), device=device, dtype=dtype).permute(0, 3, 1, 2)


def as_nhwc(x):
    B, C_, H, W = x.shape
    sb, sc, sh, sw = x.stride()
    ok = (sc == 1 or C_ == 1) and sw >= C_ and (sh == W * sw or H == 1) and (sb == H * W * sw or B == 1)
    if not ok:
        x = x.permute(0, 2, 3, 1).contiguous().permute(0, 3, 1, 2)
        sw = C_
    return x, sw


def fold_bn(bn, conv_bias=None, eps=1e-5):
    scale = bn.weight / torch.sqrt(bn.running_var + eps)
    shift = bn.bias - bn.running_mean * scale
    if conv_bias is not None:
        shift = shift + conv_bias * scale
    return scale.float().contiguous(), shift.float().contiguous()


def pack_mfma(w):
    if w.dim() == 2:
        w = w[:, :, None, None]
    if w.dim() == 3:
        w = w[:, :, :, None]
    co, ci, kh, kw = w.shape
    cop = (co + 127) // 128 * 128
    p = torch.zeros((kh * kw, cop, ci), device=w.device, dtype=torch.float32)
    p[:, :co, :] = w.permute(2, 3, 0, 1).reshape(kh * kw, co, ci)
    return p.contiguous()


_W44_G = [[1 / 4, 0, 0], [-1 / 6, -1 / 6, -1 / 6], [-1 / 6, 1 / 6, -1 / 6], [1 / 24, 1 / 12, 1 / 6], [1 / 24, -1 / 12, 1 / 6], [0, 0, 1]]


def pack_wino44(w):
    co, ci, kh, kw = w.shape
    assert kh == 3 and kw == 3
    G = torch.tensor(_W44_G, device=w.device, dtype=torch.float64)
    U = torch.einsum('ij,ocjk,lk->iloc', G, w.double(), G).reshape(36, co, ci).float()
    cop = (co + 63) // 64 * 64
    p = torch.zeros((36, cop, ci), device=w.device, dtype=torch.float32)
    p[:, :co, :] = U
    return p.contiguous()


def pack_wino44_fragments(wu):
    xi, cop, ci = wu.shape
    assert xi == 36 and cop % 64 == 0 and ci % 16 == 0
    t = wu.reshape(36, cop // 32, 32, ci // 8, 2, 4)
    return t.permute(0, 3, 1, 4, 2, 5).contiguous().reshape(36, ci // 8, cop // 32, 64, 4)


class SplitFragments:
    __slots__ = ('words', 'post')

    def __init__(self, words, post):
        self.words, self.post = words, float(post)

    @property
    def shape(self):
        return self.words.shape


def split_scale(wu):
    m = float(wu.abs().max())
    return 1.0 if m == 0.0 else 2.0 ** (12 - math.floor(math.log2(m)))


def pack_wino44_fragments_split(wu):
    assert wu.is_cuda, 'the fragments are split on the device (no CPU path)'
    sc = split_scale(wu)
    frag = pack_wino44_fragments(wu * sc)
    out = torch.empty_like(frag)
    check(lib().lm_wino44_split_fragments(_stream(), _ptr(frag), _ptr(out), frag.numel() // 4))
    return SplitFragments(out, 1.0 / sc)


def pack_small(w):
    co, ci, kh, kw = w.shape
    if co > 16:
        assert co % 16 == 0 and co <= 64, f'pack_small: Cout={co} must be <= 16 or 32 / 48 / 64'
        return torch.stack([pack_small(w[16 * i:16 * (i + 1)]) for i in range(co // 16)]).contiguous()
    p = torch.zeros((kh * kw, ci, 16), device=w.device, dtype=torch.float32)
    p[:, :, :co] = w.permute(2, 3, 1, 0).reshape(kh * kw, ci, co)
    return p.contiguous()


def pack_token_mix(w):
    if w.dim() == 3:
        w = w[:, :, 0]
    m, k = w.shape
    p = torch.zeros(((k + 15) // 16 * 16, (m + 127) // 128 * 128), device=w.device, dtype=torch.float32)
    p[:k, :m] = w.t()
    return p.contiguous()


_conv_hook = None


def set_conv_hook(fn):
    global _conv_hook
    _conv_hook = fn


def conv_mfma(x, wp, cout, kh=1, kw=1, stride=1, pad=0, dil=1, scale=None, shift=None, res=None, act=ACT_NONE,
              out=None, res_rows=0, res_up=None):
    x, ldx = as_nhwc(x)
    B, cin, H, W = x.shape
    ph, pw = (pad, pad) if isinstance(pad, int) else pad
    Ho = (H + 2 * ph - dil * (kh - 1) - 1) // stride + 1
    Wo = (W + 2 * pw - dil * (kw - 1) - 1) // stride + 1
    if out is None:
        out = new_act(B, cout, Ho, Wo, x.device)
    out_, ldy = as_nhwc(out)
    assert out_.data_ptr() == out.data_ptr(), 'conv_mfma: `out` must already be NHWC-stored'
    ldr = 0
    if res is not None:
        if res.dim() == 4:
            res, ldr = as_nhwc(res)
        else:
            ldr = res.stride(0)
    if res_up is not None:
        assert res is None and res_rows == 0
        ru, ldu = as_nhwc(res_up)
        assert ru.shape[0] == B and ru.shape[1] == cout

    def launch():
        if res_up is not None:
            check(lib().lm_conv2d_nhwc_mfma_resup_f32(_stream(), _ptr(x), ldx, _ptr(wp), wp.shape[1], _ptr(scale), _ptr(shift),
                                                      _ptr(ru), ldu, ru.shape[2], ru.shape[3], _ptr(out), ldy, B, H, W, cin, cout,
                                                      kh, kw, stride, ph, pw, dil, act))
            return
        check(lib().lm_conv2d_nhwc_mfma_f32(_stream(), _ptr(x), ldx, _ptr(wp), wp.shape[1], _ptr(scale), _ptr(shift),
                                            _ptr(res), ldr, res_rows, _ptr(out), ldy, B, H, W, cin, cout, kh, kw,
                                            stride, ph, pw, dil, act))
    if _conv_hook is not None:
        _conv_hook(f'conv {cin}->{cout} k{kh}x{kw} s{stride} d{dil} @{H}x{W} B{B}', 2.0 * B * Ho * Wo * cout * cin * kh * kw, launch)
    else:
        launch()
    return out


def _hooked(kind, flops, launch, executed=None):
    if _conv_hook is not None:
        _conv_hook(kind, flops, launch, executed)
    else:
        launch()


def wino44_supported(H, W, cin, dil=1):
    return bool(lib().lm_winograd44_supported(int(H), int(W), int(cin), int(dil)))


def conv_wino44(x, wf, cout, dil=1, scale=None, shift=None, res=None, act=ACT_NONE, out=None, gn_eps=None, gn_split=1):
    x, ldx = as_nhwc(x)
    B, cin, H, W = x.shape
    cop = wf.shape[2] * 32
    y = out if out is not None else new_act(B, cout, H, W, x.device)
    y_, ldy = as_nhwc(y)
    assert y_.data_ptr() == y.data_ptr(), 'conv_wino44: `out` must already be NHWC-stored'
    r, ldr = (None, 0) if res is None else as_nhwc(res)
    part = None
    if gn_eps is not None:
        part = torch.empty((B, lib().lm_winograd44_gn_chunks(H, W, dil), cout, 2), device=x.device, dtype=torch.float64)
    tiles = lib().lm_winograd44_tiles(B, H, W, dil)
    if isinstance(wf, SplitFragments):
        _hooked(f'wino44split {cin}->{cout} k3x3 d{dil} @{H}x{W} B{B}', 2.0 * B * H * W * cout * cin * 9,
                lambda: check(lib().lm_conv3x3_winograd44_split_f32(_stream(), _ptr(x), ldx, _ptr(wf.words), cop, _ptr(scale), _ptr(shift), _ptr(r),
                                                                    ldr, _ptr(y), ldy, B, H, W, cin, cout, dil, act, _ptr(part), wf.post)),
                3 * 2.0 * 36 * tiles * cin * cout)
    else:
        _hooked(f'wino44 {cin}->{cout} k3x3 d{dil} @{H}x{W} B{B}', 2.0 * B * H * W * cout * cin * 9,
                lambda: check(lib().lm_conv3x3_winograd44_f32(_stream(), _ptr(x), ldx, _ptr(wf), cop, _ptr(scale), _ptr(shift), _ptr(r), ldr,
                                                              _ptr(y), ldy, B, H, W, cin, cout, dil, act, _ptr(part))),
                2.0 * 36 * tiles * cin * cout)
    if gn_eps is None:
        return y
    if gn_split > 1:
        stats = torch.empty((gn_split, B, cout // gn_split, 2), device=x.device, dtype=torch.float32)
        check(lib().lm_gn_finalize_split(_stream(), _ptr(part), _ptr(stats), B, H * W, cout, part.shape[1], gn_eps, gn_split))
        return y, stats
    stats = torch.empty((B, cout, 2), device=x.device, dtype=torch.float32)
    check(lib().lm_gn_finalize(_stream(), _ptr(part), _ptr(stats), B, H * W, cout, part.shape[1], gn_eps))
    return y, stats


def conv_wino44_twin(x, wu, cout, dil=1, scale=None, shift=None, res=None, act=ACT_NONE, out=None, split=False):
    x, ldx = as_nhwc(x)
    B, cin, H, W = x.shape
    cop = wu.shape[1]
    y = out if out is not None else new_act(B, cout, H, W, x.device)
    y_, ldy = as_nhwc(y)
    assert y_.data_ptr() == y.data_ptr(), 'conv_wino44_twin: `out` must already be NHWC-stored'
    r, ldr = (None, 0) if res is None else as_nhwc(res)
    need = lib().lm_winograd44_twin_workspace_bytes(B, H, W, cin, cop, dil)
    ws = torch.empty(need, device=x.device, dtype=torch.uint8)
    if split:
        sc = split_scale(wu)
        wus = (wu * sc).contiguous()
        check(lib().lm_conv3x3_winograd44_split_twin_f32(_stream(), _ptr(x), ldx, _ptr(wus), cop, _ptr(scale), _ptr(shift), _ptr(r), ldr,
                                                         _ptr(y), ldy, B, H, W, cin, cout, dil, act, _ptr(ws), need, 1.0 / sc))
        return y
    check(lib().lm_conv3x3_winograd44_twin_f32(_stream(), _ptr(x), ldx, _ptr(wu), cop, _ptr(scale), _ptr(shift), _ptr(r), ldr,
                                               _ptr(y), ldy, B, H, W, cin, cout, dil, act, _ptr(ws), need))
    return y


def conv_mfma_gnstats(x, wp, cout, kh, kw, stride, pad, dil, shift, eps=1e-5):
    x, ldx = as_nhwc(x)
    B, cin, H, W = x.shape
    Ho = (H + 2 * pad - dil * (kh - 1) - 1) // stride + 1
    Wo = (W + 2 * pad - dil * (kw - 1) - 1) // stride + 1
    out = new_act(B, cout, Ho, Wo, x.device)
    nchunk = Ho * Wo // 64
    part = torch.empty((B, nchunk, cout, 2), device=x.device, dtype=torch.float64)
    stats = torch.empty((B, cout, 2), device=x.device, dtype=torch.float32)
    def launch():
        check(lib().lm_conv2d_nhwc_mfma_f32_gnstats(_stream(), _ptr(x), ldx, _ptr(wp), wp.shape[1], _ptr(shift), _ptr(out), cout,
                                                    _ptr(part), B, H, W, cin, cout, kh, kw, stride, pad, pad, dil))
    if _conv_hook is not None:
        _conv_hook(f'conv+gn {cin}->{cout} k{kh}x{kw} s{stride} d{dil} @{H}x{W} B{B}', 2.0 * B * Ho * Wo * cout * cin * kh * kw, launch)
    else:
        launch()
    check(lib().lm_gn_finalize(_stream(), _ptr(part), _ptr(stats), B, Ho * Wo, cout, nchunk, eps))
    return out, stats


def linear_mfma(x2d, wp, n_out, scale=None, shift=None, res=None, res_rows=0, act=ACT_NONE, out=None):
    assert x2d.dim() == 2 and x2d.stride(1) == 1
    M, K = x2d.shape
    if out is None:
        out = torch.empty((M, n_out), device=x2d.device, dtype=torch.float32)
    ldr = res.stride(0) if res is not None else 0
    def launch():
        check(lib().lm_conv2d_nhwc_mfma_f32(_stream(), _ptr(x2d), x2d.stride(0), _ptr(wp), wp.shape[1], _ptr(scale),
                                            _ptr(shift), _ptr(res), ldr, res_rows, _ptr(out), out.stride(0),
                                            1, 1, M, K, n_out, 1, 1, 1, 0, 0, 1, act))
    if _conv_hook is not None:
        _conv_hook(f'gemm M{M} K{K} N{n_out}', 2.0 * M * n_out * K, launch)
    else:
        launch()
    return out


def token_mix(x2d, wt, M, bias, B, res=None, act=ACT_NONE, out=None):
    assert x2d.dim() == 2 and x2d.is_contiguous() and x2d.shape[0] % B == 0
    K, N = x2d.shape[0] // B, x2d.shape[1]
    assert wt.shape[0] >= K and wt.shape[1] >= M and bias.numel() == M
    if out is None:
        out = torch.empty((B * M, N), device=x2d.device, dtype=torch.float32)
    assert out.is_contiguous() and tuple(out.shape) == (B * M, N)
    if res is not None:
        assert res.is_contiguous() and tuple(res.shape) == (B * M, N)
    def launch():
        check(lib().lm_token_mix_mfma_f32(_stream(), _ptr(x2d), _ptr(wt), wt.shape[1], _ptr(bias), _ptr(res), _ptr(out),
                                          B, M, K, N, act))
    if _conv_hook is not None:
        _conv_hook(f'token_mix M{M} K{K} N{N} B{B}', 2.0 * B * M * K * N, launch)
    else:
        launch()
    return out


def conv_small(x, w16, cout, kh=1, kw=1, stride=1, pad=0, scale=None, shift=None, pre_relu=False, act=ACT_NONE, out=None):
    x, ldx = as_nhwc(x)
    B, cin, H, W = x.shape
    ph, pw = (pad, pad) if isinstance(pad, int) else pad
    Ho = (H + 2 * ph - kh) // stride + 1
    Wo = (W + 2 * pw - kw) // stride + 1
    if out is None:
        out = new_act(B, cout, Ho, Wo, x.device)
    out_, ldy = as_nhwc(out)
    assert out_.data_ptr() == out.data_ptr()
    check(lib().lm_conv2d_nhwc_small(_stream(), _ptr(x), ldx, _ptr(w16), _ptr(scale), _ptr(shift), _ptr(out), ldy,
                                     B, H, W, cin, cout, kh, kw, stride, ph, pw, int(pre_relu), act))
    return out


def stem(x, w_k64, scale, shift):
    x = x.contiguous()
    if x.dtype == torch.uint8:
        B, H, W, C_ = x.shape
        assert C_ == 3, 'u8 tiles are [B,H,W,3]'
    else:
        B, _, H, W = x.shape
    Ho, Wo = (H - 1) // 2 + 1, (W - 1) // 2 + 1
    out = new_act(B, 64, Ho, Wo, x.device)
    fn = lib().lm_stem_conv7x7_bn_relu_u8 if x.dtype == torch.uint8 else lib().lm_stem_conv7x7_bn_relu
    check(fn(_stream(), _ptr(x), _ptr(w_k64), _ptr(scale), _ptr(shift), _ptr(out), B, H, W))
    return out


def maxpool3x3s2(x):
    x, ld = as_nhwc(x)
    B, C_, H, W = x.shape
    assert ld == C_
    out = new_act(B, C_, (H - 1) // 2 + 1, (W - 1) // 2 + 1, x.device)
    check(lib().lm_maxpool3x3s2_nhwc(_stream(), _ptr(x), _ptr(out), B, H, W, C_))
    return out


def gn_stats(x, eps=1e-5):
    x, ld = as_nhwc(x)
    B, C_, H, W = x.shape
    assert ld == C_
    ws = torch.empty(lib().lm_gn_stats_workspace_bytes(B, H * W, C_) // 8, device=x.device, dtype=torch.float64)
    stats = torch.empty((B, C_, 2), device=x.device, dtype=torch.float32)
    check(lib().lm_gn_stats(_stream(), _ptr(x), _ptr(ws), _ptr(stats), B, H * W, C_, eps))
    return stats


def gn_relu_upsample(x, stats, gamma, beta, size, out=None, accumulate=False):
    x, ld = as_nhwc(x)
    B, C_, H, W = x.shape
    assert ld == C_
    Ho, Wo = size
    if out is None:
        assert not accumulate
        out = new_act(B, C_, Ho, Wo, x.device)
    check(lib().lm_gn_relu_upsample(_stream(), _ptr(x), _ptr(stats), _ptr(gamma), _ptr(beta), _ptr(out),
                                    B, H, W, Ho, Wo, C_, int(accumulate)))
    return out


def gn_relu_upsample_sum(terms, gamma, beta, size, out=None, proj=None, keep_sum=True):
    n = len(terms)
    xs = [as_nhwc(x) for x, _ in terms]
    B, C_ = xs[0][0].shape[:2]
    for (x, ld) in xs:
        assert ld >= C_ and ld % 4 == 0 and x.shape[0] == B and x.shape[1] == C_
    Ho, Wo = size
    dev = xs[0][0].device
    if out is None and (keep_sum or proj is None):
        out = new_act(B, C_, Ho, Wo, dev)
    vp_arr, i_arr = C.c_void_p * n, C.c_int * n
    head = (_stream(), n, vp_arr(*[_ptr(x) for x, _ in xs]), vp_arr(*[_ptr(st) for _, st in terms]),
            i_arr(*[x.shape[2] for x, _ in xs]), i_arr(*[x.shape[3] for x, _ in xs]), i_arr(*[ld for _, ld in xs]),
            _ptr(gamma), _ptr(beta))
    if proj is None:
        check(lib().lm_gn_relu_upsample_sum(*head, _ptr(out), B, Ho, Wo, C_))
        return out
    w16, bias, cout = proj[:3]
    out1 = proj[3] if len(proj) > 3 and proj[3] is not None else new_act(B, cout, Ho, Wo, dev)
    o1, ldy1 = as_nhwc(out1)
    assert o1.data_ptr() == out1.data_ptr()
    check(lib().lm_gn_relu_upsample_sum_conv1x1(*head, _ptr(out) if keep_sum else None, B, Ho, Wo, C_, _ptr(w16), _ptr(bias), cout,
                                                _ptr(out1), ldy1))
    return (out, out1) if keep_sum else out1


def upsample_nhwc(x, size, add=None, out=None):
    x, ldx = as_nhwc(x)
    B, C_, H, W = x.shape
    Ho, Wo = size
    if out is None and add is None and (Ho, Wo) == (H, W):
        return x
    if out is None:
        out = new_act(B, C_, Ho, Wo, x.device)
    out_, ldy = as_nhwc(out)
    assert out_.data_ptr() == out.data_ptr()
    lda = 0
    if add is not None:
        add, lda = as_nhwc(add)
    check(lib().lm_upsample_bilinear_nhwc(_stream(), _ptr(x), ldx, _ptr(add), lda, _ptr(out), ldy, B, H, W, Ho, Wo, C_))
    return out


def upsample_to_chw(x, size):
    x, ldx = as_nhwc(x)
    B, C_, H, W = x.shape
    Ho, Wo = size
    out = torch.empty((B, C_, Ho, Wo), device=x.device, dtype=torch.float32)
    check(lib().lm_upsample_bilinear_to_chw(_stream(), _ptr(x), ldx, _ptr(out), B, H, W, Ho, Wo, C_))
    return out


def layernorm(x2d, gamma, beta, eps=1e-5):
    assert x2d.is_contiguous()
    out = torch.empty_like(x2d)
    check(lib().lm_layernorm_rows(_stream(), _ptr(x2d), _ptr(gamma), _ptr(beta), _ptr(out), x2d.shape[0], x2d.shape[1], eps))
    return out


def unpatchify(tokens, B, G, P, C_):
    out = new_act(B, C_, G * P, G * P, tokens.device)
    check(lib().lm_unpatchify(_stream(), _ptr(tokens.contiguous()), _ptr(out), B, G, P, C_))
    return out


def attention(qkv, B, N, heads, dim_head, scale, valid=None):
    assert qkv.is_contiguous()
    out = torch.empty((B * N, heads * dim_head), device=qkv.device, dtype=torch.float32)
    if valid is None:
        check(lib().lm_attention_f32(_stream(), _ptr(qkv), _ptr(out), B, N, heads, dim_head, float(scale)))
    else:
        assert valid.dtype == torch.int32 and valid.is_contiguous() and tuple(valid.shape) == (B, N)
        check(lib().lm_attention_masked_f32(_stream(), _ptr(qkv), _ptr(out), _ptr(valid), B, N, heads, dim_head, float(scale)))
    return out


def head_tokens(seg, row, P, prop_width, half_buff, seg_bias):
    row, ld = as_nhwc(row)
    B, C_, Hr, Wr = row.shape
    assert C_ == 16 and ld == 16
    tok = torch.empty((B * P * Hr, 16 * (prop_width + 2 * half_buff)), device=row.device, dtype=torch.float32)
    if seg is None:
        check(lib().lm_head_tokens_window(_stream(), _ptr(row), _ptr(tok), B, P, Hr, Wr, prop_width, half_buff))
        return tok
    seg = seg.reshape(B, 2 * Hr, 2 * Wr).contiguous()
    check(lib().lm_head_tokens(_stream(), _ptr(seg), _ptr(row), _ptr(tok), float(seg_bias), B, P, Hr, Wr, prop_width, half_buff))
    return tok


def head_stage2(hid, D, w2, b2, B, P, R, w_small=None):
    M = hid.shape[0]
    FW = (w2.shape[0] - 3) // 2
    assert w2.shape == (3 + 2 * FW, D) and b2.numel() == 3 + 2 * FW and hid.shape[1] >= 3 * D and hid.stride(1) == 1
    ext2 = torch.empty((B, P, R, 3), device=hid.device, dtype=torch.float32)
    cls2 = torch.empty((B, P, R, FW), device=hid.device, dtype=torch.float32)
    off2 = torch.empty((B, P, R, FW), device=hid.device, dtype=torch.float32)
    if FW == 10:
        check(lib().lm_head_stage2(_stream(), _ptr(hid), hid.stride(0), D, _ptr(w2), _ptr(b2), _ptr(ext2), _ptr(cls2), _ptr(off2), M))
        return ext2, cls2, off2
    if w_small is None:
        raise ValueError(f'head_stage2: prop_fea_width {FW} runs through lm_conv2d_nhwc_small and needs the pack_small weights')
    bounds = (0, 3, 3 + FW, 3 + 2 * FW)
    for br, (y, w16) in enumerate(zip((ext2, cls2, off2), w_small)):
        n = bounds[br + 1] - bounds[br]
        assert tuple(w16.shape) == (1, D, 16)
        x = hid[:, br * D:(br + 1) * D]
        shift = b2[bounds[br]:bounds[br + 1]]
        check(lib().lm_conv2d_nhwc_small(_stream(), _ptr(x), hid.stride(0), _ptr(w16), None, _ptr(shift), _ptr(y), n,
                                         1, 1, M, D, n, 1, 1, 1, 0, 0, 0, ACT_NONE))
    return ext2, cls2, off2


def head_proposal_conf(tok, wt, bias, B, P):
    L = tok.numel() // (B * P)
    conf = torch.empty((B, P, 2), device=tok.device, dtype=torch.float32)
    check(lib().lm_head_proposal_conf(_stream(), _ptr(tok), _ptr(wt), _ptr(bias), _ptr(conf), B * P, L))
    return conf


def pack_readback(tensors, block=None):
    offs, sizes, off = [], [], 0
    for t in tensors:
        assert t.is_contiguous()
        nb = t.numel() * t.element_size()
        assert nb % 4 == 0, 'lm_pack_segments copies 4-byte words'
        off = (off + 255) // 256 * 256
        offs.append(off); sizes.append(nb)
        off += nb
    if block is None or block.numel() < off or block.device != tensors[0].device:
        block = torch.empty(max(off, 1), device=tensors[0].device, dtype=torch.uint8)
    n = len(tensors)
    src = (C.c_void_p * n)(*[t.data_ptr() for t in tensors])
    nby = (C.c_long * n)(*sizes)
    dof = (C.c_long * n)(*offs)
    check(lib().lm_pack_segments(_stream(), n, src, nby, dof, _ptr(block)))
    return block, list(zip(offs, sizes))


def decode_proposals(pconf, ext2, cls2, off2, exist_thre, prop_width, half_buff):
    B, P, R, FW = cls2.shape
    assert FW == prop_width + 2 * half_buff and off2.shape[-1] == FW, 'cls2 / offset2 are prop_fea_width wide'
    dev = cls2.device
    prop_conf = torch.empty((B, P, 2), device=dev, dtype=torch.float32)
    v_ext = torch.empty((B, P, R), device=dev, dtype=torch.float32)
    cls_conf = torch.empty((B, P, R, FW), device=dev, dtype=torch.float32)
    cls_idx = torch.empty((B, P, R), device=dev, dtype=torch.int32)
    cls_offset = torch.empty((B, P, R), device=dev, dtype=torch.float64)
    check(lib().lm_decode_proposals(_stream(), _ptr(pconf.contiguous()), _ptr(ext2.contiguous()), _ptr(cls2.contiguous()),
                                    _ptr(off2.contiguous()), _ptr(prop_conf), _ptr(v_ext), _ptr(cls_conf), _ptr(cls_idx),
                                    _ptr(cls_offset), B, P, R, float(exist_thre), prop_width, half_buff))
    return prop_conf, v_ext, cls_conf, cls_idx, cls_offset


def decode_orient(orient_logits):
    x, ld = as_nhwc(orient_logits)
    B, C_, H, W = x.shape
    out = torch.empty((B, H, W), device=x.device, dtype=torch.uint8)
    check(lib().lm_decode_orient(_stream(), _ptr(x), ld, C_, _ptr(out), B * H * W))
    return out


def decode_semantic(logits_chw, thre, raw_mode=False, want_biseg=True):
    x = logits_chw.contiguous()
    B, C_, H, W = x.shape
    assert C_ == 3
    sem = torch.empty((B, H, W), device=x.device, dtype=torch.uint8)
    biseg = rows = None
    if want_biseg:
        biseg = torch.empty((B, H, W), device=x.device, dtype=torch.float32)
        rows = torch.empty((B, H // 8, W), device=x.device, dtype=torch.float32)
    check(lib().lm_decode_semantic(_stream(), _ptr(x), _ptr(sem), _ptr(biseg), _ptr(rows), B, H, W, float(thre), int(raw_mode)))
    return sem, biseg, rows


def endp_topk(endp_logits, K=512, clip=20):
    x = endp_logits.contiguous()
    B, C_, H, W = x.shape
    assert C_ == 1
    ws = torch.empty(lib().lm_endp_topk_workspace_bytes(B), device=x.device, dtype=torch.uint8)
    idx = torch.empty((B, K), device=x.device, dtype=torch.int32)
    score = torch.empty((B, K), device=x.device, dtype=torch.float32)
    status = torch.empty((B,), device=x.device, dtype=torch.int32)
    check(lib().lm_endp_topk(_stream(), _ptr(x), _ptr(ws), _ptr(idx), _ptr(score), _ptr(status), B, H, W, clip, K))
    return idx, score, status


def make_raster_params(quat=(1, 0, 0, 0), trans=(0, 0, 0), bev_img_offset=(0, 0), img_reso=(0.05, 0.05),
                       local_min_ele=0.0, ele_reso=0.05, inten_lo=800.0, inten_hi=33000.0):
    p = LmRasterParams()
    p.quat[:] = [float(v) for v in quat]
    p.trans[:] = [float(v) for v in trans]
    p.bev_img_offset[:] = [float(v) for v in bev_img_offset]
    p.img_reso[:] = [float(v) for v in img_reso]
    p.local_min_ele, p.ele_reso, p.inten_lo, p.inten_hi = float(local_min_ele), float(ele_reso), float(inten_lo), float(inten_hi)
    return p


_raster_ws = {}


def bev_raster_batch(points, tile_offsets, params, H=1152, W=1152, out=None, want_u8=False, u8_only=False, out_u8=None):
    assert points.dim() == 2 and points.shape[1] == 4 and points.is_contiguous() and points.dtype == torch.float32
    B = len(params)
    assert len(tile_offsets) == B + 1
    offs = (C.c_long * (B + 1))(*[int(o) for o in tile_offsets])
    par = (LmRasterParams * B)(*params)
    cap = max([offs[b + 1] - offs[b] for b in range(B)] + [0])
    need = lib().lm_bev_raster_workspace_bytes(B, cap, H, W)
    key = (points.device, _stream().value)
    ws = _raster_ws.get(key)
    if ws is None or ws.numel() < need:
        ws = _raster_ws[key] = torch.empty(need, device=points.device, dtype=torch.uint8)
    want_u8 = want_u8 or u8_only or out_u8 is not None
    if out is None and not u8_only:
        out = torch.empty((B, 3, H, W), device=points.device, dtype=torch.float32)
    u8 = None
    if want_u8:
        u8 = out_u8 if out_u8 is not None else torch.empty((B, H, W, 3), device=points.device, dtype=torch.uint8)
        assert u8.dtype == torch.uint8 and u8.is_contiguous() and tuple(u8.shape) == (B, H, W, 3)
    check(lib().lm_bev_raster_batch(_stream(), _ptr(points) if points.numel() else None, offs, par, B, _ptr(ws), ws.numel(),
                                    None if u8_only else _ptr(out), _ptr(u8), H, W))
    if u8_only:
        return u8
    return (out, u8) if want_u8 else out


def bev_raster(points, params, H=1152, W=1152, want_u8=False):
    r = bev_raster_batch(points, [0, points.shape[0]], [params], H, W, want_u8=want_u8)
    return (r[0][0], r[1][0]) if want_u8 else r[0]


def strip_grid(params, H=1152, W=1152, z_range=None):
    import numpy as np
    T = len(params)
    par = (LmRasterParams * T)(*params)
    z_lo, z_hi = (float(z_range[0]), float(z_range[1])) if z_range is not None else (-math.inf, math.inf)
    g = LmStripGrid()
    check(lib().lm_strip_build_grid(par, T, H, W, z_lo, z_hi, C.byref(g), None, 0))
    cells = np.empty((g.ny, g.nx, 8), dtype=np.uint16)
    check(lib().lm_strip_build_grid(par, T, H, W, z_lo, z_hi, C.byref(g), C.c_void_p(cells.ctypes.data), g.nx * g.ny))
    return {'x0': g.x0, 'y0': g.y0, 'cell': g.cell, 'nx': g.nx, 'ny': g.ny}, cells


def _tilted(p):
    return p.quat[1] != 0.0 or p.quat[2] != 0.0


def strip_bin_points(points, params, H=1152, W=1152, z_range=None, capacity=None):
    if not points.is_cuda:
        _ptr(points)
    assert points.dim() == 2 and points.shape[1] == 4 and points.is_contiguous() and points.dtype == torch.float32
    T, N = len(params), points.shape[0]
    par = (LmRasterParams * T)(*params)
    if z_range is None and N and any(_tilted(p) for p in params):
        z = points[:, 2]
        z = z[torch.isfinite(z)]
        z_range = (float(z.min()), float(z.max())) if z.numel() else (0.0, 0.0)
    z_lo, z_hi = (float(z_range[0]), float(z_range[1])) if z_range is not None else (-math.inf, math.inf)
    if not (math.isfinite(z_lo) and math.isfinite(z_hi)) and any(_tilted(p) for p in params):
        if N:
            raise ValueError('strip_bin_points: tilted tiles need a finite z_range (or None: it is then taken from the points)')
        z_lo, z_hi = 0.0, 0.0
    need = lib().lm_strip_bin_workspace_bytes(N, T)
    if need <= 0:
        raise LanemapHipError(f'strip_bin_points: {T} tiles / {N} points are not supported (1 to 4096 tiles)')
    key = (points.device, _stream().value)
    ws = _raster_ws.get(key)
    if ws is None or ws.numel() < need:
        ws = _raster_ws[key] = torch.empty(need, device=points.device, dtype=torch.uint8)
    meta = torch.empty(2 * T + 1, device=points.device, dtype=torch.int64)
    offs = (C.c_long * (T + 1))()
    cap = int(capacity) if capacity is not None else N + N // 4
    binned = None
    for attempt in range(2):
        del binned
        binned = torch.empty((cap, 4), device=points.device, dtype=torch.float32)
        rc = lib().lm_strip_bin_points(_stream(), _ptr(points) if N else None, N, par, T, H, W, z_lo, z_hi, _ptr(ws), ws.numel(),
                                       C.c_void_p(meta.data_ptr()), C.c_void_p(meta.data_ptr() + 8 * T), offs, _ptr(binned) if cap else None, cap)
        if rc == 4 and attempt == 0 and capacity is None:
            cap = int(offs[T])
            continue
        check(rc)
        break
    return binned[:offs[T]], [int(o) for o in offs]


def tile_ingest(u8_hwc):
    x = u8_hwc.contiguous()
    B, H, W, C_ = x.shape
    out = torch.empty((B, 3, H, W), device=x.device, dtype=torch.float32)
    check(lib().lm_tile_ingest_u8(_stream(), _ptr(x), _ptr(out), B, H, W, C_))
    return out


_vox_ws = {}


def exclusive_scan_u32(x, out=None):
    x = x.contiguous()
    assert x.dim() == 1 and x.dtype in (torch.int32, torch.uint32)
    out = torch.empty_like(x) if out is None else out
    n = x.numel()
    ws = torch.empty((lib().lm_scan_workspace_bytes(n),), device=x.device, dtype=torch.uint8)
    check(lib().lm_exclusive_scan_u32(_stream(), _ptr(x), _ptr(out), n, _ptr(ws), ws.numel()))
    return out


def sort_pairs_u32_(keys, vals, end_bit=32):
    assert keys.dim() == 1 and keys.shape == vals.shape and keys.is_contiguous() and vals.is_contiguous()
    assert keys.dtype in (torch.int32, torch.uint32) and vals.dtype in (torch.int32, torch.uint32)
    n = keys.numel()
    ws = torch.empty((lib().lm_sort_pairs_workspace_bytes(n),), device=keys.device, dtype=torch.uint8)
    check(lib().lm_sort_pairs_u32(_stream(), _ptr(keys), _ptr(vals), n, int(end_bit), _ptr(ws), ws.numel()))
    return keys, vals


def voxelize_batch(points, range_lo, voxel_size, grid_xyz, max_points, max_voxels, ldf=16, raster_order=False):
    dev = points[0].device
    B = len(points)
    cells = int(grid_xyz[0]) * int(grid_xyz[1]) * int(grid_xyz[2])
    caps = [min(int(p.shape[0]), int(max_voxels), cells) for p in points]
    cap = max(1, sum(caps))
    feats = torch.empty((cap, ldf), device=dev, dtype=torch.float32)
    coords = torch.empty((cap, 4), device=dev, dtype=torch.int32)
    ends = torch.zeros((B,), device=dev, dtype=torch.int32)
    nmax = max(int(p.shape[0]) for p in points)
    need = lib().lm_voxelize_workspace_bytes(nmax)
    key = (dev.index, _stream().value)
    ws = _vox_ws.get(key)
    if ws is None or ws.numel() < need:
        ws = torch.empty((need,), device=dev, dtype=torch.uint8)
        _vox_ws[key] = ws
    lo = (C.c_float * 3)(*[float(v) for v in range_lo])
    vs = (C.c_float * 3)(*[float(v) for v in voxel_size])
    g = (C.c_int * 3)(*[int(v) for v in grid_xyz])
    for b, p in enumerate(points):
        if not p.is_cuda:
            raise LanemapHipError('voxelize_batch needs device tensors; no CPU fallback exists')
        p = p.contiguous().float()
        assert p.dim() == 2 and p.shape[1] == 4
        base = C.c_void_p(ends[b - 1:b].data_ptr()) if b > 0 else None
        check(lib().lm_voxelize_hard(_stream(), _ptr(p) if p.shape[0] else None, p.shape[0], lo, vs, g, int(max_points),
                                     int(max_voxels), b, base, cap, _ptr(feats), ldf, _ptr(coords),
                                     C.c_void_p(ends[b:b + 1].data_ptr()), int(raster_order), _ptr(ws), ws.numel()))
    row_ends = [int(v) for v in ends.cpu()]
    V = row_ends[-1]
    return feats[:V], coords[:V], row_ends


def _ksp(kernel, stride, padding):
    return (C.c_int * 9)(*[int(v) for v in (*kernel, *stride, *padding)])


def sparse_grid(coords, B, shape):
    D, H, W = shape
    grid = torch.empty((B, D, H, W), device=coords.device, dtype=torch.int32)
    check(lib().lm_sparse_grid_build(_stream(), _ptr(coords), coords.shape[0], _ptr(grid), B, D, H, W))
    return grid


def sparse_conv_outputs(in_coords, B, in_shape, kernel, stride, padding):
    out_shape = tuple((in_shape[a] + 2 * padding[a] - kernel[a]) // stride[a] + 1 for a in range(3))
    Do, Ho, Wo = out_shape
    dev = in_coords.device
    cells = B * Do * Ho * Wo
    n_in = in_coords.shape[0]
    taps_per_axis = [(kernel[a] + stride[a] - 1) // stride[a] for a in range(3)]
    cap = max(1, min(cells, n_in * taps_per_axis[0] * taps_per_axis[1] * taps_per_axis[2]))
    grid = torch.empty((B, Do, Ho, Wo), device=dev, dtype=torch.int32)
    coords = torch.empty((cap, 4), device=dev, dtype=torch.int32)
    count = torch.zeros((1,), device=dev, dtype=torch.int32)
    need = lib().lm_sparse_conv_outputs_workspace_bytes(cells)
    ws = torch.empty((need,), device=dev, dtype=torch.uint8)
    check(lib().lm_sparse_conv_outputs(_stream(), _ptr(in_coords), n_in, B, _ksp(kernel, stride, padding), Do, Ho, Wo,
                                       _ptr(grid), _ptr(coords), cap, _ptr(count), _ptr(ws), need))
    n = int(count.item())
    if n > cap:
        raise LanemapHipError(f'sparse_conv_outputs: {n} active sites exceed the bound {cap}')
    return grid, coords[:n], out_shape


def sparse_rulebook(out_coords, in_grid, kernel, stride, padding):
    B, D, H, W = in_grid.shape
    taps = kernel[0] * kernel[1] * kernel[2]
    nbr = torch.empty((out_coords.shape[0], taps), device=out_coords.device, dtype=torch.int32)
    check(lib().lm_sparse_rulebook(_stream(), _ptr(out_coords), out_coords.shape[0], _ptr(in_grid), B, D, H, W,
                                   _ksp(kernel, stride, padding), _ptr(nbr)))
    return nbr


def pack_sparse(w):
    kd, kh, kw, ci, co = w.shape
    taps = kd * kh * kw
    cop = (co + 127) // 128 * 128
    wt = w.reshape(taps, ci, co).permute(0, 2, 1).float()
    if ci <= 16:
        p = torch.zeros(((taps + 1) // 2 * 2, cop, 16), device=w.device, dtype=torch.float32)
        p[:taps, :co, :ci] = wt
        return p.reshape(-1, 2, cop, 16).permute(0, 2, 1, 3).reshape(-1, cop, 32).contiguous()
    cip = (ci + 31) // 32 * 32
    p = torch.zeros((taps, cop, cip), device=w.device, dtype=torch.float32)
    p[:, :co, :ci] = wt
    return p.contiguous()


def sparse_ld(c):
    return 16 if c <= 16 else (c + 31) // 32 * 32


def conv_gather(x, nbr, wp, cin, cout, scale=None, shift=None, res=None, act=ACT_NONE):
    M, taps = nbr.shape
    cin_k = sparse_ld(cin)
    assert x.stride(1) == 1 and x.stride(0) >= cin_k
    ldy = sparse_ld(cout)
    y = torch.zeros((M, ldy), device=x.device, dtype=torch.float32) if ldy != cout else \
        torch.empty((M, ldy), device=x.device, dtype=torch.float32)
    def launch():
        check(lib().lm_conv_gather_mfma_f32(_stream(), _ptr(x), x.stride(0), _ptr(nbr), taps, _ptr(wp), wp.shape[1], _ptr(scale),
                                            _ptr(shift), _ptr(res), res.stride(0) if res is not None else 0, _ptr(y), ldy,
                                            M, cin_k, cout, act))
    if _conv_hook is not None:
        _conv_hook(f'spconv M{M} taps{taps} {cin}->{cout}', 2.0 * M * taps * cin * cout, launch)
    else:
        launch()
    return y


def sparse_to_dense(feats, coords, B, shape, C_, flip_h):
    D, H, W = shape
    out = new_act(B, C_ * D, H, W, feats.device)
    check(lib().lm_sparse_to_dense_nhwc(_stream(), _ptr(feats), feats.stride(0), _ptr(coords), feats.shape[0], _ptr(out),
                                        B, D, H, W, C_, int(flip_h)))
    return out


def upsample_bicubic(x, size):
    x, ld = as_nhwc(x)
    B, C_, H, W = x.shape
    assert ld == C_
    out = new_act(B, C_, size[0], size[1], x.device)
    check(lib().lm_upsample_bicubic_nhwc(_stream(), _ptr(x), _ptr(out), B, H, W, C_, size[0], size[1]))
    return out
```

### lanemapping_amd/pcencoder.py

```python
import os

import torch
import torch.nn as nn

from . import ops, trace
from .registry import PCENCODER
from .packing import PackedModule

_LAYERS = {'resnet18': [2, 2, 2, 2], 'resnet34': [3, 4, 6, 3]}
MERGE_BRANCH_CONVS = os.environ.get('LANEMAP_MERGE_BRANCH_CONVS', '1') != '0'
WINO_F44 = os.environ.get('LANEMAP_WINO_F44', '1') != '0'
WINO_F44_MIN_CIN = int(os.environ.get('LANEMAP_WINO_F44_MIN_CIN', '64'))
WINO_SPLIT = os.environ.get('LANEMAP_WINO_SPLIT', '0') != '0'


def _frag44(w):
    if WINO_SPLIT:
        return ops.pack_wino44_fragments_split(ops.pack_wino44(w))
    return ops.pack_wino44_fragments(ops.pack_wino44(w))


def _f44_ok(conv):
    return WINO_F44 and conv.kernel_size == (3, 3) and conv.stride == (1, 1) and conv.in_channels >= WINO_F44_MIN_CIN and conv.in_channels % 16 == 0


class _ResBlock(nn.Module):

    def __init__(self, cin, cout, stride, dilation, with_down):
        super().__init__()
        self.conv1 = nn.Conv2d(cin, cout, 3, stride, dilation, dilation, bias=False)
        self.bn1 = nn.BatchNorm2d(cout)
        self.conv2 = nn.Conv2d(cout, cout, 3, 1, dilation, dilation, bias=False)
        self.bn2 = nn.BatchNorm2d(cout)
        self.downsample = nn.Sequential(nn.Conv2d(cin, cout, 1, stride, bias=False), nn.BatchNorm2d(cout)) if with_down else None
        self.stride, self.dilation = stride, dilation


def _stage(state, planes, blocks, stride, dilate):
    prev_dil = state[1]
    if dilate:
        state[1] *= stride
        stride = 1
    layers = [_ResBlock(state[0], planes, stride, prev_dil, stride != 1 or state[0] != planes)]
    state[0] = planes
    for _ in range(1, blocks):
        layers.append(_ResBlock(planes, planes, 1, state[1], False))
    return nn.Sequential(*layers)


class _BottomUp(nn.Module):

    def __init__(self, layers, dil, in_channels):
        super().__init__()
        self.conv1 = nn.Conv2d(3, 64, 7, 2, 3, bias=False)
        self.bn1 = nn.BatchNorm2d(64)
        st = [64, 1]
        self.layer1 = _stage(st, in_channels[0], layers[0], 1, False)
        self.layer2 = _stage(st, in_channels[1], layers[1], 2, dil[0])
        if in_channels[2] > 0:
            self.layer3 = _stage(st, in_channels[2], layers[2], 2, dil[1])
        if in_channels[3] > 0:
            self.layer4 = _stage(st, in_channels[3], layers[3], 2, dil[2])


class FPNEncoder(PackedModule):
    def __init__(self, resnet='resnet34', pretrained=False, replace_stride_with_dilation=(False, True, False),
                 out_conv=True, in_channels=(64, 128, 256, -1), cfg=None):
        super().__init__()
        if resnet not in _LAYERS:
            raise NotImplementedError(f'{resnet}: only BasicBlock ResNets are on the hot path')
        if in_channels[2] <= 0 or in_channels[3] > 0:
            raise NotImplementedError('hot path covers in_channels=[c1,c2,c3,-1] (all BASELINE configs)')
        dil = list(replace_stride_with_dilation)
        if len(dil) != 3:
            raise ValueError(f'replace_stride_with_dilation should be None or a 3-element tuple, got {dil}')
        layers = _LAYERS[resnet]
        self.cfg = cfg
        self.in_channels = list(in_channels)
        self.model_buttomup = _BottomUp(layers, dil, in_channels)
        self.conv1 = nn.Conv2d(3, 64, 7, 2, 3, bias=False)
        self.bn1 = nn.BatchNorm2d(64)
        st = [64, 1]
        self.layer1 = _stage(st, in_channels[0], layers[0], 1, False)
        self.layer2 = _stage(st, in_channels[1], layers[1], 2, dil[0])
        self.layer3 = _stage(st, in_channels[2], layers[2], 2, dil[1])
        c = st[0]
        self.out = nn.Conv2d(c, cfg.featuremap_out_channel, 1, bias=False) if out_conv else None
        self.toplayer = nn.Conv2d(c, 256, 1)
        self.smooth1 = nn.Conv2d(c, c, 3, 1, 1)
        self.smooth2 = nn.Conv2d(c, c, 3, 1, 1)
        self.smooth3 = nn.Conv2d(c, c, 3, 1, 1)
        self.latlayer1 = nn.Conv2d(in_channels[1], c, 1)
        self.latlayer2 = nn.Conv2d(in_channels[0], c, 1)
        self.semantic_branch = nn.Conv2d(c, c // 2, 3, 1, 1)
        self.semantic_branch2 = nn.Conv2d(c, c // 2, 3, 1, 1)
        self.conv2 = nn.Conv2d(c, c, 3, 1, 1)
        self.conv3 = nn.Conv2d(c, c, 3, 1, 1)
        self.feature_layer = nn.Conv2d(c // 2, 8, 1)
        self.output_layer_binary_seg = nn.Conv2d(8, 3, 1)
        self.output_layer_endp = nn.Conv2d(c // 2, 1, 1)
        self.gn11 = nn.GroupNorm(c // 2, c // 2)
        self.gn12 = nn.GroupNorm(c, c)
        self.gn21 = nn.GroupNorm(c // 2, c // 2)
        self.gn22 = nn.GroupNorm(c, c)

    def _pack(self):
        P = {}
        P['stem_w'] = self.conv1.weight.permute(2, 3, 1, 0).contiguous().float()
        P['stem_s'], P['stem_b'] = ops.fold_bn(self.bn1)
        for lname in ('layer1', 'layer2', 'layer3'):
            for i, blk in enumerate(getattr(self, lname)):
                k = f'{lname}.{i}'
                P[k + '.w1'] = ops.pack_mfma(blk.conv1.weight)
                P[k + '.s1'], P[k + '.b1'] = ops.fold_bn(blk.bn1)
                P[k + '.w2'] = ops.pack_mfma(blk.conv2.weight)
                P[k + '.s2'], P[k + '.b2'] = ops.fold_bn(blk.bn2)
                for q, conv in (('.w1q', blk.conv1), ('.w2q', blk.conv2)):
                    if _f44_ok(conv):
                        P[k + q] = _frag44(conv.weight)
                if blk.downsample is not None:
                    P[k + '.wd'] = ops.pack_mfma(blk.downsample[0].weight)
                    P[k + '.sd'], P[k + '.bd'] = ops.fold_bn(blk.downsample[1])
        for name in ('toplayer', 'smooth1', 'smooth2', 'smooth3', 'latlayer1', 'latlayer2', 'semantic_branch',
                     'semantic_branch2', 'conv2', 'conv3'):
            m = getattr(self, name)
            P[name + '.w'] = ops.pack_mfma(m.weight)
            P[name + '.b'] = m.bias.float().contiguous()
            if _f44_ok(m):
                P[name + '.wq'] = _frag44(m.weight)
        a, b2 = self.semantic_branch, self.semantic_branch2
        if (MERGE_BRANCH_CONVS and 'semantic_branch.wq' in P and 'semantic_branch2.wq' in P and a.out_channels == b2.out_channels
                and self.gn11.eps == self.gn21.eps):
            P['semantic_branch_ab.wq'] = _frag44(torch.cat([a.weight, b2.weight], dim=0))
            P['semantic_branch_ab.b'] = torch.cat([a.bias, b2.bias]).float().contiguous()
            if ('conv2.wq' in P and 'conv3.wq' in P and self.conv2.out_channels == self.conv3.out_channels
                    and self.gn12.eps == self.gn22.eps):
                P['conv23.wq'] = _frag44(torch.cat([self.conv2.weight, self.conv3.weight], dim=0))
                P['conv23.b'] = torch.cat([self.conv2.bias, self.conv3.bias]).float().contiguous()
        if self.out is not None:
            P['out.w'] = ops.pack_mfma(self.out.weight)
        for name in ('feature_layer', 'output_layer_binary_seg', 'output_layer_endp'):
            m = getattr(self, name)
            P[name + '.w'] = ops.pack_small(m.weight)
            P[name + '.b'] = m.bias.float().contiguous()
        for name in ('gn11', 'gn12', 'gn21', 'gn22'):
            m = getattr(self, name)
            P[name + '.g'], P[name + '.b'] = m.weight.float().contiguous(), m.bias.float().contiguous()
        return P

    @staticmethod
    def _c3(x, P, wkey, cout, stride, dil, **epi):
        if (wkey + 'q') in P and stride == 1 and ops.wino44_supported(x.shape[2], x.shape[3], x.shape[1], dil):
            return ops.conv_wino44(x, P[wkey + 'q'], cout, dil, **epi)
        return ops.conv_mfma(x, P[wkey], cout, 3, 3, stride, dil, dil, **epi)

    def _block(self, x, P, key, blk):
        cout = blk.conv1.out_channels
        y = self._c3(x, P, key + '.w1', cout, blk.stride, blk.dilation, scale=P[key + '.s1'], shift=P[key + '.b1'], act=ops.ACT_RELU)
        if blk.downsample is not None:
            x = ops.conv_mfma(x, P[key + '.wd'], cout, 1, 1, blk.stride, 0, 1, scale=P[key + '.sd'], shift=P[key + '.bd'])
        return self._c3(y, P, key + '.w2', cout, 1, blk.dilation, scale=P[key + '.s2'], shift=P[key + '.b2'], res=x, act=ops.ACT_RELU)

    def _conv3(self, x, P, name, cout):
        return self._c3(x, P, name + '.w', cout, 1, 1, shift=P[name + '.b'])

    def _conv_stats(self, P, src, conv, cout, gn):
        eps = getattr(self, gn).eps
        if (conv + '.wq') in P and ops.wino44_supported(src.shape[2], src.shape[3], src.shape[1], 1):
            return ops.conv_wino44(src, P[conv + '.wq'], cout, 1, shift=P[conv + '.b'], gn_eps=eps)
        if (src.shape[2] * src.shape[3]) % 128 == 0:
            return ops.conv_mfma_gnstats(src, P[conv + '.w'], cout, 3, 3, 1, 1, 1, P[conv + '.b'], eps)
        t = self._conv3(src, P, conv, cout)
        return t, ops.gn_stats(t, eps)

    def _semantic(self, P, p2, p3, p4, conv_a, gn_a, conv_b, gn_b, proj, pre=None, pre_a4=None):
        h, w = p2.shape[2:]
        c_half = self.semantic_branch.out_channels
        t, st = pre_a4 if pre_a4 is not None else self._conv_stats(P, p4, conv_a, p4.shape[1], gn_a)
        s4 = ops.gn_relu_upsample_sum([(t, st)], P[gn_a + '.g'], P[gn_a + '.b'], (h, w))
        terms = [pre[0] if pre is not None and pre[0] is not None else self._conv_stats(P, p2, conv_b, c_half, gn_b),
                 pre[1] if pre is not None and pre[1] is not None else self._conv_stats(P, p3, conv_b, c_half, gn_b)]
        terms.append(self._conv_stats(P, s4, conv_b, c_half, gn_b))
        return ops.gn_relu_upsample_sum(terms, P[gn_b + '.g'], P[gn_b + '.b'], (h, w), proj=proj, keep_sum=False)

    def forward(self, x, fea_up_out=None):
        from . import torch_ops
        if self.out is None:
            return self._forward_impl(x, fea_up_out)
        if fea_up_out is None:
            B, H, W = (x.shape[0], x.shape[1], x.shape[2]) if x.dtype == torch.uint8 else (x.shape[0], x.shape[2], x.shape[3])
            fea_up_out = ops.new_act(B, 8, (H + 3) // 4, (W + 3) // 4, x.device)
        fea, bi_seg, endp = torch_ops.fpn_encoder(x, fea_up_out, torch_ops.stage_weights(self), torch_ops.stage_name(self))
        return fea, fea_up_out, bi_seg, endp

    def _forward_impl(self, x, fea_up_out=None):
        P = self.packed()
        if x.dtype == torch.uint8:
            B, H, W, _ = x.shape
        else:
            B, _, H, W = x.shape
        with trace.stage('fpn.stem'):
            c1 = ops.maxpool3x3s2(ops.stem(x, P['stem_w'], P['stem_s'], P['stem_b']))
        feats = []
        t = c1
        for lname in ('layer1', 'layer2', 'layer3'):
            with trace.stage('fpn.' + lname):
                for i, blk in enumerate(getattr(self, lname)):
                    t = self._block(t, P, f'{lname}.{i}', blk)
            feats.append(t)
        c2, c3, c4 = feats
        trace.push('fpn.topdown')
        fea = ops.conv_mfma(c4, P['out.w'], self.out.out_channels) if self.out is not None else None
        p4 = ops.conv_mfma(c4, P['toplayer.w'], 256, shift=P['toplayer.b'])
        def lateral(c, name, coarse):
            if tuple(coarse.shape[2:]) == tuple(c.shape[2:]):
                return ops.conv_mfma(c, P[name + '.w'], 256, shift=P[name + '.b'], res=coarse)
            return ops.conv_mfma(c, P[name + '.w'], 256, shift=P[name + '.b'], res_up=coarse)

        p3 = lateral(c3, 'latlayer1', p4)
        p2 = lateral(c2, 'latlayer2', p3)
        del c1, c2, c3, c4, feats, t
        p4 = self._conv3(p4, P, 'smooth1', 256)
        p3 = self._conv3(p3, P, 'smooth2', 256)
        p2 = self._conv3(p2, P, 'smooth3', 256)
        trace.pop()
        trace.push('fpn.semantic')
        pre_a, pre_b = [None, None], [None, None]
        if 'semantic_branch_ab.wq' in P:
            ch = self.semantic_branch.out_channels
            for i, src in enumerate((p2, p3)):
                if ops.wino44_supported(src.shape[2], src.shape[3], src.shape[1], 1):
                    t, st = ops.conv_wino44(src, P['semantic_branch_ab.wq'], 2 * ch, 1, shift=P['semantic_branch_ab.b'],
                                            gn_eps=self.gn11.eps, gn_split=2)
                    pre_a[i], pre_b[i] = (t[:, :ch], st[0]), (t[:, ch:], st[1])
        a4 = b4 = None
        if 'conv23.wq' in P and ops.wino44_supported(p4.shape[2], p4.shape[3], p4.shape[1], 1):
            c4o = self.conv2.out_channels
            t, st = ops.conv_wino44(p4, P['conv23.wq'], 2 * c4o, 1, shift=P['conv23.b'], gn_eps=self.gn12.eps, gn_split=2)
            a4, b4 = (t[:, :c4o], st[0]), (t[:, c4o:], st[1])
        fea_up = self._semantic(P, p2, p3, p4, 'conv2', 'gn12', 'semantic_branch', 'gn11',
                                (P['feature_layer.w'], P['feature_layer.b'], 8, fea_up_out), pre_a, a4)
        seg288 = ops.conv_small(fea_up, P['output_layer_binary_seg.w'], 3, shift=P['output_layer_binary_seg.b'], pre_relu=True)
        bi_seg = ops.upsample_to_chw(seg288, (H, W))
        endp288 = self._semantic(P, p2, p3, p4, 'conv3', 'gn22', 'semantic_branch2', 'gn21',
                                 (P['output_layer_endp.w'], P['output_layer_endp.b'], 1, None), pre_b, b4)
        endp = ops.upsample_to_chw(endp288, (H, W))
        trace.pop()
        return fea, fea_up, bi_seg, endp


@PCENCODER.register_module
class PostProjector2(nn.Module):
    def __init__(self, resnet='resnet50', pretrained=False, replace_stride_with_dilation=[False, True, False],
                 out_conv=True, in_channels=[64, 128, 256, -1], cfg=None):
        super().__init__()
        self.cfg = cfg
        self.fpn = FPNEncoder(resnet=resnet, pretrained=pretrained, replace_stride_with_dilation=replace_stride_with_dilation,
                              out_conv=out_conv, in_channels=in_channels, cfg=cfg)

    def forward(self, sample):
        return self.fpn(sample['proj'])

    def infer_validate(self, preds, seg_thre=None, endp_thre=None, display=None):
        from .decode import segmentor_decode
        return segmentor_decode(preds['seg'], preds['endp'], seg_thre)
```

### lanemapping_amd/pipeline.py

```python
import collections
import os
import threading
import time
from concurrent.futures import ThreadPoolExecutor

import numpy as np
import torch

from . import decode, hostpost, ops, torch_ops, trace
from ._lib import LanemapHipError


class TilePipeline:
    def __init__(self, net, host_threads=8, use_graph=None, with_decode_endp=False):
        self.with_decode_endp = bool(with_decode_endp)
        self.use_graph = (os.environ.get('LANEMAP_GRAPHS', '0') != '0') if use_graph is None else bool(use_graph)
        self._graphs = collections.OrderedDict()
        self.net = net
        self.cfg = net.cfg
        self.rowref = net.cfg.heads.type == 'RowSharNotReducRef'
        if net.cfg.heads.type not in ('ColumnProposal2', 'RowSharNotReducRef'):
            raise NotImplementedError(f'TilePipeline has no decode / polyline tail for heads.type={net.cfg.heads.type!r}')
        self.pool = ThreadPoolExecutor(max_workers=host_threads)
        self._pending = None
        self._slots, self._slot_next = [], 0
        self.host_seconds = 0.0
        self.host_tiles = 0
        self._stats_lock = threading.Lock()

    HOST_SLOTS = 3

    def _host_slot(self, nbytes):
        if not self._slots:
            self._slots = [{'block': None, 'futs': []} for _ in range(self.HOST_SLOTS)]
        slot = self._slots[self._slot_next]
        self._slot_next = (self._slot_next + 1) % self.HOST_SLOTS
        assert self._pending is None or self._pending[4] is not slot, 'pinned staging ring too short for the pipeline depth'
        if slot['futs']:
            from concurrent.futures import wait
            wait(slot['futs'])
        slot['futs'] = []
        if slot['block'] is None or slot['block'].numel() < nbytes:
            slot['block'] = torch.empty(max(nbytes, 1), dtype=torch.uint8, pin_memory=True)
        return slot

    def _gpu_stage(self, proj):
        if self.use_graph and torch.is_tensor(proj):
            (block, layout), keep, crop = self._replay(proj)
        else:
            (block, layout), keep, crop = self._device_part(proj)
        total = block.numel()
        slot = self._host_slot(total)
        hb = slot['block']
        hb[:total].copy_(block, non_blocking=True)
        host = {k: hb[o:o + nb].view(dt).view(shape) for k, o, nb, dt, shape in layout}
        ev = torch.cuda.Event()
        ev.record()
        return host, ev, (keep, block), crop, slot

    def _pack(self, dev):
        names = list(dev)
        if len(names) == 1 and dev[names[0]].is_contiguous():
            t = dev[names[0]]
            return t.view(-1).view(torch.uint8), [(names[0], 0, t.numel() * t.element_size(), t.dtype, tuple(t.shape))]
        ts = [dev[k].contiguous() for k in names]
        block, segs = ops.pack_readback(ts)
        end = max(o + nb for o, nb in segs)
        return block[:end], [(k, o, nb, t.dtype, tuple(t.shape)) for k, t, (o, nb) in zip(names, ts, segs)]

    MAX_GRAPHS = 4

    def _weights_key(self):
        from .packing import PackedModule
        mods = self.__dict__.get('_packed_mods')
        if mods is None:
            mods = self.__dict__['_packed_mods'] = [m for m in self.net.modules() if isinstance(m, PackedModule)]
        return tuple(m.param_key() for m in mods)

    def clear_graphs(self):
        self._graphs.clear()

    def _replay(self, proj):
        key = (tuple(proj.shape), proj.dtype, proj.device)
        wkey = self._weights_key()
        ent = self._graphs.get(key)
        if ent is not None and ent[3] != wkey:
            del self._graphs[key]
            ent = None
        if ent is None:
            static_in = torch.empty_like(proj)
            static_in.copy_(proj)
            self._device_part(static_in)
            torch.cuda.synchronize()
            graph = torch.cuda.CUDAGraph()
            with torch.cuda.graph(graph, stream=torch.cuda.Stream(device=proj.device)):
                out = self._device_part(static_in)
            ent = (graph, static_in, out, wkey)
            self._graphs[key] = ent
            while len(self._graphs) > self.MAX_GRAPHS:
                self._graphs.popitem(last=False)
        self._graphs.move_to_end(key)
        graph, static_in, out, _ = ent
        static_in.copy_(proj, non_blocking=True)
        graph.replay()
        return out

    def _device_part(self, proj):
        heads, cfg = self.net.heads, self.cfg
        batch = proj if isinstance(proj, dict) else ({'points': list(proj)} if isinstance(proj, (list, tuple)) else {'proj': proj})
        raw = self.net.forward_raw(batch)
        if self.rowref:
            dev = {'col': heads.decode_columns(raw)}
            keep = (raw, dev)
            crop = 0
        else:
            trace.push('decode')
            prop_conf, v_ext, cls_conf, cls_idx, cls_offset = torch_ops.decode_proposals(
                raw['proposal_conf'], raw['ext2'], raw['cls2'], raw['offset2'], float(cfg.exist_thre), heads.prop_width, heads.prop_half_buff)
            orient = torch_ops.decode_orient(raw['orient'])
            sem, biseg, rows = torch_ops.decode_semantic(raw['semantic_seg'], float(cfg.coor_thre))
            idx, score, status = torch_ops.endp_topk(raw['endp_est'], decode.TOPK, decode.CLIP)
            trace.pop()
            dev = {'prop_conf': prop_conf, 'v_ext': v_ext, 'cls_offset': cls_offset, 'rows': rows, 'idx': idx, 'status': status}
            keep = (raw, sem, biseg, orient, cls_conf, cls_idx, dev)
            crop = raw['endp_est'].shape[-1]
        return self._pack(dev), keep, crop

    def _tile_task(self, host, b, crop_w):
        t0 = time.perf_counter()
        if self.rowref:
            heads = self.net.heads
            cols = heads.lines_from_columns(host['col'][b].numpy(), heads.row_size)
            lanes = np.full((72, 144, 2), -1.0)
            lanes[:, :, 1] = 0.0
            lanes[:cols.shape[0], :, 0] = cols
            lanes[:cols.shape[0], :, 1] = (cols > 0).astype(np.float64)
            kept = pts = np.zeros((0, 2), dtype=np.int32)
        else:
            pts, _ = hostpost.cluster_endpoints(host['idx'][b].numpy(), crop_w=crop_w, clip=decode.CLIP,
                                                k0=self.net.heads.num_cls * 2 * 10, k_max=500)
            lanes, kept = hostpost.assemble_polylines(host['prop_conf'][b].numpy(), host['v_ext'][b].numpy(),
                                                      host['cls_offset'][b].numpy(), host['rows'][b].numpy(), pts,
                                                      self.cfg.proposal_obj_thre)
            if lanes.shape[0] < 72:
                pad = np.full((72 - lanes.shape[0],) + lanes.shape[1:], -1.0)
                pad[:, :, 1] = 0.0
                lanes = np.concatenate([lanes, pad])
        dt = time.perf_counter() - t0
        with self._stats_lock:
            self.host_seconds += dt
            self.host_tiles += 1
        return (lanes, kept, pts) if self.with_decode_endp else (lanes, kept)

    def _finish(self, pending):
        host, ev, keep, W, slot = pending
        ev.synchronize()
        if not self.rowref and int(host['status'].max()) != 0:
            raise LanemapHipError('endpoint top-K candidate overflow')
        B = next(iter(host.values())).shape[0]
        futs = [self.pool.submit(self._tile_task, host, b, W - 2 * decode.CLIP) for b in range(B)]
        slot['futs'] = futs
        return futs

    def submit(self, proj):
        with torch.no_grad():
            new = self._gpu_stage(proj)
        futs = self._finish(self._pending) if self._pending is not None else []
        self._pending = new
        return futs

    def flush(self):
        futs = self._finish(self._pending) if self._pending is not None else []
        self._pending = None
        return futs

    def run_batch(self, proj):
        assert self._pending is None
        self.submit(proj)
        return [f.result() for f in self.flush()]
```

### lanemapping_amd/torch_ops.py

```python
import itertools
import weakref
from typing import List, Optional, Tuple

import numpy as np
import torch
from torch import Tensor

from . import ops as _ops

_STAGES = weakref.WeakValueDictionary()
_STAGE_COUNTER = itertools.count()


def stage_name(module):
    n = module.__dict__.get('_lanemap_stage_name')
    if n is None:
        n = module.__dict__['_lanemap_stage_name'] = f'{type(module).__name__}#{next(_STAGE_COUNTER)}'
    _STAGES[n] = module
    return n


def stage_weights(module):
    return [d[n] for d, n in module._slots() if d[n] is not None]


class _with_weights:

    def __init__(self, spec, weights):
        m = _STAGES.get(spec)
        if m is None:
            raise RuntimeError(f'lanemap_hip: no live stage module registered as {spec!r}')
        slots = [(d, n) for d, n in m._slots() if d[n] is not None]
        if len(slots) != len(weights):
            raise RuntimeError(f'lanemap_hip: stage {spec} has {len(slots)} weight tensors, the op was handed {len(weights)}')
        self.m, self.swap = m, [(d, n, d[n], w) for (d, n), w in zip(slots, weights) if d[n] is not w]
        for d, n, own, w in self.swap:
            if own.shape != w.shape or own.dtype != w.dtype:
                raise RuntimeError(f'lanemap_hip: stage {spec}: weight {n} is {tuple(w.shape)} {w.dtype}, expected {tuple(own.shape)} {own.dtype}')

    def __enter__(self):
        for d, n, own, w in self.swap:
            d[n] = w if not isinstance(own, torch.nn.Parameter) or isinstance(w, torch.nn.Parameter) else torch.nn.Parameter(w, requires_grad=False)
        return self.m

    def __exit__(self, *exc):
        for d, n, own, w in self.swap:
            d[n] = own
        return False


def _stage(spec):
    m = _STAGES.get(spec)
    if m is None:
        raise RuntimeError(f'lanemap_hip: no live stage module registered as {spec!r}')
    return m


def _fake_act(like, B, C, H, W, dtype=torch.float32):
    return like.new_empty((B, H, W, C), dtype=dtype).permute(0, 3, 1, 2)


def _out_hw(H, W, kh, kw, stride, pad, dil):
    return (H + 2 * pad - dil * (kh - 1) - 1) // stride + 1, (W + 2 * pad - dil * (kw - 1) - 1) // stride + 1


def _define(name, fn, fake, mutates=(), device='cuda'):
    op = torch.library.custom_op(f'lanemap_hip::{name}', fn, mutates_args=mutates, device_types=device)
    op.register_fake(fake)
    return op


def _conv2d_mfma(x: Tensor, w_packed: Tensor, cout: int, kh: int, kw: int, stride: int, pad: int, dil: int,
                 scale: Optional[Tensor], shift: Optional[Tensor], res: Optional[Tensor], act: int) -> Tensor:
    return _ops.conv_mfma(x, w_packed, cout, kh, kw, stride, pad, dil, scale=scale, shift=shift, res=res, act=act)


def _conv2d_mfma_fake(x, w_packed, cout, kh, kw, stride, pad, dil, scale, shift, res, act):
    Ho, Wo = _out_hw(x.shape[2], x.shape[3], kh, kw, stride, pad, dil)
    return _fake_act(x, x.shape[0], cout, Ho, Wo)


def _conv3x3_winograd44(x: Tensor, wu_frag: Tensor, cout: int, dil: int, scale: Optional[Tensor], shift: Optional[Tensor],
                        res: Optional[Tensor], act: int) -> Tensor:
    return _ops.conv_wino44(x, wu_frag, cout, dil, scale=scale, shift=shift, res=res, act=act)


def _conv3x3_fake(x, w, cout, dil, scale, shift, res, act):
    return _fake_act(x, x.shape[0], cout, x.shape[2], x.shape[3])


def _stem(x: Tensor, w_k64: Tensor, scale: Tensor, shift: Tensor) -> Tensor:
    return _ops.stem(x, w_k64, scale, shift)


def _stem_fake(x, w_k64, scale, shift):
    B, H, W = (x.shape[0], x.shape[1], x.shape[2]) if x.dtype == torch.uint8 else (x.shape[0], x.shape[2], x.shape[3])
    return _fake_act(x, B, 64, (H - 1) // 2 + 1, (W - 1) // 2 + 1)


def _maxpool(x: Tensor) -> Tensor:
    return _ops.maxpool3x3s2(x)


def _maxpool_fake(x):
    return _fake_act(x, x.shape[0], x.shape[1], (x.shape[2] - 1) // 2 + 1, (x.shape[3] - 1) // 2 + 1)


def _gn_stats(x: Tensor, eps: float) -> Tensor:
    return _ops.gn_stats(x, eps)


def _gn_stats_fake(x, eps):
    return x.new_empty((x.shape[0], x.shape[1], 2))


def _gn_relu_upsample(x: Tensor, stats: Tensor, gamma: Tensor, beta: Tensor, Ho: int, Wo: int) -> Tensor:
    return _ops.gn_relu_upsample(x, stats, gamma, beta, (Ho, Wo))


def _upsample_bilinear(x: Tensor, Ho: int, Wo: int) -> Tensor:
    y = _ops.upsample_nhwc(x, (Ho, Wo))
    return y.clone() if y.data_ptr() == x.data_ptr() else y


def _resize_fake(x, *a):
    return _fake_act(x, x.shape[0], x.shape[1], a[-2], a[-1])


def _layernorm_rows(x: Tensor, gamma: Tensor, beta: Tensor, eps: float) -> Tensor:
    return _ops.layernorm(x, gamma, beta, eps)


def _attention(qkv: Tensor, B: int, N: int, heads: int, dim_head: int, scale: float) -> Tensor:
    return _ops.attention(qkv, B, N, heads, dim_head, scale)


def _linear_mfma(x: Tensor, w_packed: Tensor, n_out: int, scale: Optional[Tensor], shift: Optional[Tensor], res: Optional[Tensor],
                 res_rows: int, act: int) -> Tensor:
    return _ops.linear_mfma(x, w_packed, n_out, scale=scale, shift=shift, res=res, res_rows=res_rows, act=act)


def _token_mix(x: Tensor, wt: Tensor, M: int, bias: Tensor, B: int, res: Optional[Tensor], act: int) -> Tensor:
    return _ops.token_mix(x, wt, M, bias, B, res=res, act=act)


def _tile_ingest(u8_hwc: Tensor) -> Tensor:
    return _ops.tile_ingest(u8_hwc)


def _decode_proposals(pconf: Tensor, ext2: Tensor, cls2: Tensor, off2: Tensor, exist_thre: float, prop_width: int,
                      half_buff: int) -> Tuple[Tensor, Tensor, Tensor, Tensor, Tensor]:
    return _ops.decode_proposals(pconf, ext2, cls2, off2, exist_thre, prop_width, half_buff)


def _decode_proposals_fake(pconf, ext2, cls2, off2, exist_thre, prop_width, half_buff):
    B, P, R, FW = cls2.shape
    return (cls2.new_empty((B, P, 2)), cls2.new_empty((B, P, R)), cls2.new_empty((B, P, R, FW)),
            cls2.new_empty((B, P, R), dtype=torch.int32), cls2.new_empty((B, P, R), dtype=torch.float64))


def _decode_semantic(logits: Tensor, thre: float) -> Tuple[Tensor, Tensor, Tensor]:
    return _ops.decode_semantic(logits, thre)


def _decode_semantic_fake(logits, thre):
    B, _, H, W = logits.shape
    return logits.new_empty((B, H, W), dtype=torch.uint8), logits.new_empty((B, H, W)), logits.new_empty((B, H // 8, W))


def _decode_orient(orient_logits: Tensor) -> Tensor:
    return _ops.decode_orient(orient_logits)


def _endp_topk(endp_logits: Tensor, K: int, clip: int) -> Tuple[Tensor, Tensor, Tensor]:
    return _ops.endp_topk(endp_logits, K=K, clip=clip)


def _endp_topk_fake(endp_logits, K, clip):
    B = endp_logits.shape[0]
    return (endp_logits.new_empty((B, K), dtype=torch.int32), endp_logits.new_empty((B, K)), endp_logits.new_empty((B,), dtype=torch.int32))


conv2d_mfma = _define('conv2d_mfma', _conv2d_mfma, _conv2d_mfma_fake)
conv3x3_winograd44 = _define('conv3x3_winograd44', _conv3x3_winograd44, _conv3x3_fake)
stem_conv7x7 = _define('stem_conv7x7', _stem, _stem_fake)
maxpool3x3s2 = _define('maxpool3x3s2', _maxpool, _maxpool_fake)
gn_stats = _define('gn_stats', _gn_stats, _gn_stats_fake)
gn_relu_upsample = _define('gn_relu_upsample', _gn_relu_upsample, lambda x, stats, gamma, beta, Ho, Wo: _resize_fake(x, Ho, Wo))
upsample_bilinear = _define('upsample_bilinear', _upsample_bilinear, lambda x, Ho, Wo: _resize_fake(x, Ho, Wo))
layernorm_rows = _define('layernorm_rows', _layernorm_rows, lambda x, gamma, beta, eps: torch.empty_like(x))
attention = _define('attention', _attention, lambda qkv, B, N, heads, dim_head, scale: qkv.new_empty((B * N, heads * dim_head)))
linear_mfma = _define('linear_mfma', _linear_mfma,
                      lambda x, w_packed, n_out, scale, shift, res, res_rows, act: x.new_empty((x.shape[0], n_out)))
token_mix = _define('token_mix', _token_mix, lambda x, wt, M, bias, B, res, act: x.new_empty((B * M, x.shape[1])))
tile_ingest = _define('tile_ingest', _tile_ingest,
                      lambda u8: u8.new_empty((u8.shape[0], 3, u8.shape[1], u8.shape[2]), dtype=torch.float32))
decode_proposals = _define('decode_proposals', _decode_proposals, _decode_proposals_fake)
decode_semantic = _define('decode_semantic', _decode_semantic, _decode_semantic_fake)
decode_orient = _define('decode_orient', _decode_orient,
                        lambda o: o.new_empty((o.shape[0], o.shape[2], o.shape[3]), dtype=torch.uint8))
endp_topk = _define('endp_topk', _endp_topk, _endp_topk_fake)


def _bev_raster(points: Tensor, tile_offsets: List[int], params: Tensor, H: int, W: int) -> Tensor:
    p = params.detach().cpu().float().numpy()
    pars = [_ops.make_raster_params(quat=r[0:4], trans=r[4:7], bev_img_offset=r[7:9], img_reso=r[9:11], local_min_ele=r[11],
                                    ele_reso=r[12], inten_lo=r[13], inten_hi=r[14]) for r in p]
    return _ops.bev_raster_batch(points, tile_offsets, pars, H, W, u8_only=True)


bev_raster = _define('bev_raster', _bev_raster,
                     lambda points, tile_offsets, params, H, W: points.new_empty((len(tile_offsets) - 1, H, W, 3), dtype=torch.uint8))


def raster_params_tensor(params):
    rows = [[*p.quat, *p.trans, *p.bev_img_offset, *p.img_reso, p.local_min_ele, p.ele_reso, p.inten_lo, p.inten_hi] for p in params]
    return torch.tensor(rows, dtype=torch.float32)


def _fpn_encoder(proj: Tensor, fea_up_out: Tensor, weights: List[Tensor], stage: str) -> Tuple[Tensor, Tensor, Tensor]:
    with _with_weights(stage, weights) as m:
        fea, _, bi_seg, endp = m._forward_impl(proj, fea_up_out)
    return fea, bi_seg, endp


def _fpn_encoder_fake(proj, fea_up_out, weights, stage):
    B, H, W = (proj.shape[0], proj.shape[1], proj.shape[2]) if proj.dtype == torch.uint8 else (proj.shape[0], proj.shape[2], proj.shape[3])
    m = _stage(stage)
    cf = m.out.out_channels if m.out is not None else 256
    return (_fake_act(proj, B, cf, H // 8, W // 8), proj.new_empty((B, 3, H, W), dtype=torch.float32),
            proj.new_empty((B, 1, H, W), dtype=torch.float32))


fpn_encoder = _define('fpn_encoder', _fpn_encoder, _fpn_encoder_fake, mutates=('fea_up_out',))


def _vit_backbone(fea: Tensor, weights: List[Tensor], stage: str) -> Tensor:
    with _with_weights(stage, weights) as m:
        return m._forward_impl(fea)


def _vit_backbone_fake(fea, weights, stage):
    m = _stage(stage)
    c = m.shared_mlp.out_channels if m.is_with_shared_mlp else m.out_c
    return _fake_act(fea, fea.shape[0], c, m.grid * m.patch, m.grid * m.patch)


vit_backbone = _define('vit_backbone', _vit_backbone, _vit_backbone_fake)


def _mixer_backbone(fea: Tensor, weights: List[Tensor], stage: str) -> Tensor:
    with _with_weights(stage, weights) as m:
        return m._forward_impl(fea)


def _mixer_backbone_fake(fea, weights, stage):
    m = _stage(stage)
    return _fake_act(fea, fea.shape[0], m.output_channels, m.grid * m.patch, m.grid * m.patch)


mixer_backbone = _define('mixer_backbone', _mixer_backbone, _mixer_backbone_fake)


def _colprop_head(x: Tensor, col: Tensor, weights: List[Tensor], stage: str) -> Tuple[Tensor, Tensor, Tensor, Tensor, Tensor]:
    with _with_weights(stage, weights) as m:
        o = m._forward_impl(x, None, None, col=col)
    return o['proposal_conf'], o['ext2'], o['cls2'], o['offset2'], o['orient']


def _colprop_head_fake(x, col, weights, stage):
    m = _stage(stage)
    B, R, P, FW = x.shape[0], x.shape[2], m.num_prop, m.prop_fea_width
    return (x.new_empty((B, P, 2)), x.new_empty((B, P, R, 3)), x.new_empty((B, P, R, FW)), x.new_empty((B, P, R, FW)),
            _fake_act(x, B, m.num_orients, x.shape[2], x.shape[3]))


colprop_head = _define('colprop_head', _colprop_head, _colprop_head_fake, mutates=('col',))


def _endp_cluster(topk_idx: Tensor, crop_w: int, clip: int, k0: int, k_max: int) -> Tensor:
    from . import hostpost
    pts, _ = hostpost.cluster_endpoints(topk_idx.numpy(), crop_w=crop_w, clip=clip, k0=k0, k_max=k_max)
    return torch.from_numpy(pts.astype(np.int32).reshape(-1, 2))


def _endp_cluster_fake(topk_idx, crop_w, clip, k0, k_max):
    n = torch.library.get_ctx().new_dynamic_size()
    return topk_idx.new_empty((n, 2), dtype=torch.int32)


endp_cluster = _define('endp_cluster', _endp_cluster, _endp_cluster_fake, device='cpu')


def _polyline_assemble(prop_conf: Tensor, prop_v_ext: Tensor, cls_offset: Tensor, bi_seg_rows: Tensor, endp_hw: Tensor,
                       obj_thre: float) -> Tuple[Tensor, Tensor]:
    from . import hostpost
    lanes, kept = hostpost.assemble_polylines(prop_conf.numpy(), prop_v_ext.numpy(), cls_offset.numpy(), bi_seg_rows.numpy(),
                                              endp_hw.numpy(), obj_thre)
    return torch.from_numpy(lanes), torch.from_numpy(np.ascontiguousarray(kept, dtype=np.int32).reshape(-1, 2))


def _polyline_assemble_fake(prop_conf, prop_v_ext, cls_offset, bi_seg_rows, endp_hw, obj_thre):
    n = torch.library.get_ctx().new_dynamic_size()
    P, R = prop_v_ext.shape
    return prop_conf.new_empty((P, R, 2), dtype=torch.float64), endp_hw.new_empty((n, 2), dtype=torch.int32)


polyline_assemble = _define('polyline_assemble', _polyline_assemble, _polyline_assemble_fake, device='cpu')

OP_NAMES = ['conv2d_mfma', 'conv3x3_winograd44', 'stem_conv7x7', 'maxpool3x3s2', 'gn_stats', 'gn_relu_upsample',
            'upsample_bilinear', 'layernorm_rows', 'attention', 'linear_mfma', 'token_mix', 'tile_ingest', 'decode_proposals', 'decode_semantic',
            'decode_orient', 'endp_topk', 'bev_raster', 'fpn_encoder', 'vit_backbone', 'mixer_backbone', 'colprop_head', 'endp_cluster', 'polyline_assemble']
```

Baseline: 390.3 tiles/s.

## Fuse bilinear upsampling into semantic-row and endpoint top-k decode kernels

Adds low-resolution decode paths that bilinearly sample the quarter-resolution semantic and endpoint logits on the fly instead of first materialising full-resolution CHW maps. The semantic decode now computes only the gathered rows (every 8th row), and top-k samples endpoint logits directly from the NHWC low-res tensor. This removes two full-resolution upsample writes and their reads, but drops the full-res sem/biseg outputs and recomputes the interpolation on each of the several top-k passes. It is enabled by default via an environment flag when the FPN encoder is used.

Result: no change. 393.9 tiles/s, median of 6 (+0.9%).

```diff
diff --git a/include/lanemap_hip.h b/include/lanemap_hip.h
--- a/include/lanemap_hip.h
+++ b/include/lanemap_hip.h
@@ -94,6 +94,9 @@
 long lm_endp_topk_workspace_bytes(int B);
 int lm_endp_topk(void* stream, const float* endp_logit, void* workspace, int* out_idx, float* out_score,
                  int* out_status, int B, int H, int W, int clip, int K);
+int lm_decode_semantic_rows_lowres(void* hip_stream, const float* seg_nhwc, int ldx, float* rows, int B, int Hi, int Wi, int Ho, int Wo);
+int lm_endp_topk_lowres(void* hip_stream, const float* endp_nhwc, int ldx, int Hi, int Wi, void* workspace, int* out_idx,
+                        float* out_score, int* out_status, int B, int H, int W, int clip, int K);
 
 int lm_pack_segments(void* stream, int n, const void* const* src, const long* bytes, const long* dst_offsets, void* dst);
 
diff --git a/lanemapping_amd/_lib.py b/lanemapping_amd/_lib.py
--- a/lanemapping_amd/_lib.py
+++ b/lanemapping_amd/_lib.py
@@ -69,6 +69,8 @@
     'lm_decode_semantic': (i32, [vp, vp, vp, vp, vp, i32, i32, i32, f32, i32]),
     'lm_endp_topk_workspace_bytes': (i64, [i32]),
     'lm_endp_topk': (i32, [vp, vp, vp, vp, vp, vp, i32, i32, i32, i32, i32]),
+    'lm_decode_semantic_rows_lowres': (i32, [vp, vp, i32, vp, i32, i32, i32, i32, i32]),
+    'lm_endp_topk_lowres': (i32, [vp, vp, i32, i32, i32, vp, vp, vp, vp, i32, i32, i32, i32, i32]),
     'lm_pack_segments': (i32, [vp, i32, vp, vp, vp, vp]),
     'lm_bev_raster_workspace_bytes': (i64, [i32, i64, i32, i32]),
     'lm_bev_raster_batch': (i32, [vp, vp, C.POINTER(i64), C.POINTER(LmRasterParams), i32, vp, i64, vp, vp, i32, i32]),
diff --git a/lanemapping_amd/csrc/common.h b/lanemapping_amd/csrc/common.h
--- a/lanemapping_amd/csrc/common.h
+++ b/lanemapping_amd/csrc/common.h
@@ -81,4 +81,12 @@
     const float bot = wx0 * v10 + wx1 * v11;
     return wy0 * top + wy1 * bot;
 }
+__device__ __forceinline__ float lm_upsample_sample(const float* __restrict__ r0, const float* __restrict__ r1, int ldx, int ox, int Wi,
+                                                    int Wo, float wy0, float wy1) {
+    int x0, x1;
+    float wx0, wx1;
+    lm_bilin_axis(ox, Wi, Wo, x0, x1, wx0, wx1);
+    const float v00 = r0[(long)x0 * ldx], v01 = r0[(long)x1 * ldx], v10 = r1[(long)x0 * ldx], v11 = r1[(long)x1 * ldx];
+    return lm_bilerp(v00, v01, v10, v11, wy0, wy1, wx0, wx1);
+}
 #endif
diff --git a/lanemapping_amd/csrc/decode.hip b/lanemapping_amd/csrc/decode.hip
--- a/lanemapping_amd/csrc/decode.hip
+++ b/lanemapping_amd/csrc/decode.hip
@@ -77,6 +77,19 @@
     y[i] = (unsigned char)best;
 }
 
+__device__ __forceinline__ void semantic_scores(float l0, float l1, float l2, int raw_mode, float& s1, float& s2) {
+    if (raw_mode) {
+        s1 = l1;
+        s2 = l2;
+    } else {
+        const float m = fmaxf(l0, fmaxf(l1, l2));
+        const float e0 = expf(l0 - m), e1 = expf(l1 - m), e2 = expf(l2 - m);
+        const float s = (e0 + e1) + e2;
+        s1 = e1 / s;
+        s2 = e2 / s;
+    }
+}
+
 __global__ __launch_bounds__(256) void decode_semantic_kernel(const float* __restrict__ logit, unsigned char* __restrict__ sem,
                                                               float* __restrict__ biseg, float* __restrict__ rows, int H, int W,
                                                               float thre, int raw_mode, long total) {
@@ -87,16 +100,7 @@
     const float* lp = logit + b * 3 * HW + r;
     const float l0 = lp[0], l1 = lp[HW], l2 = lp[2 * HW];
     float s1, s2;
-    if (raw_mode) {
-        s1 = l1;
-        s2 = l2;
-    } else {
-        const float m = fmaxf(l0, fmaxf(l1, l2));
-        const float e0 = expf(l0 - m), e1 = expf(l1 - m), e2 = expf(l2 - m);
-        const float s = (e0 + e1) + e2;
-        s1 = e1 / s;
-        s2 = e2 / s;
-    }
+    semantic_scores(l0, l1, l2, raw_mode, s1, s2);
     unsigned char c = 0;
     if (s1 > s2 && s1 > thre) c = 1;
     if (s2 > s1 && s2 > thre) c = 2;
@@ -109,10 +113,33 @@
     }
 }
 
+__global__ __launch_bounds__(256) void decode_rows_lowres_kernel(const float* __restrict__ x, int ldx, float* __restrict__ rows, int Hi,
+                                                                 int Wi, int Ho, int Wo, unsigned total) {
+    const unsigned i = blockIdx.x * 256u + threadIdx.x;
+    if (i >= total) return;
+    const int ox = (int)(i % (unsigned)Wo);
+    const unsigned t = i / (unsigned)Wo;
+    const int r = (int)(t % (unsigned)(Ho / 8)), b = (int)(t / (unsigned)(Ho / 8));
+    int y0, y1;
+    float wy0, wy1;
+    lm_bilin_axis(8 * r + 3, Hi, Ho, y0, y1, wy0, wy1);
+    const float* xb = x + (long)b * Hi * Wi * ldx;
+    const float* r0 = xb + (long)y0 * Wi * ldx;
+    const float* r1 = xb + (long)y1 * Wi * ldx;
+    const float l0 = lm_upsample_sample(r0, r1, ldx, ox, Wi, Wo, wy0, wy1);
+    const float l1 = lm_upsample_sample(r0 + 1, r1 + 1, ldx, ox, Wi, Wo, wy0, wy1);
+    const float l2 = lm_upsample_sample(r0 + 2, r1 + 2, ldx, ox, Wi, Wo, wy0, wy1);
+    float s1, s2;
+    semantic_scores(l0, l1, l2, 0, s1, s2);
+    rows[i] = s1 + s2;
+}
+
 constexpr int NB = 1024;
 constexpr int CAP = 4096;
 struct TopkParams {
     const float* logit;
+    const float* src;
+    int ld, Hi, Wi;
     unsigned* hist;
     unsigned* cand_cnt;
     unsigned long long* cand;
@@ -123,6 +150,18 @@
 __device__ __forceinline__ unsigned score_key(float logit) {
     const float s = 1.0f / (1.0f + expf(-logit));
     return __float_as_uint(s);
+}
+
+template <bool LOWRES>
+__device__ __forceinline__ float topk_logit(const TopkParams& p, int b, int y, int x) {
+    if (LOWRES) {
+        int y0, y1;
+        float wy0, wy1;
+        lm_bilin_axis(y, p.Hi, p.H, y0, y1, wy0, wy1);
+        const float* xb = p.src + (long)b * p.Hi * p.Wi * p.ld;
+        return lm_upsample_sample(xb + (long)y0 * p.Wi * p.ld, xb + (long)y1 * p.Wi * p.ld, p.ld, x, p.Wi, p.W, wy0, wy1);
+    }
+    return p.logit[(long)b * p.H * p.W + (long)y * p.W + x];
 }
 
 __device__ __forceinline__ unsigned level_bin(unsigned key, int level) {
@@ -176,7 +215,7 @@
     if (i < n) p[i] = 0u;
 }
 
-template <int LEVEL>
+template <int LEVEL, bool LOWRES>
 __global__ __launch_bounds__(256) void topk_pass_kernel(TopkParams p) {
     __shared__ unsigned lh[NB];
     __shared__ unsigned pb_tmp[258];
@@ -198,10 +237,9 @@
         if (LEVEL == 3) take_ties = hist[2 * NB + bin] == need;
     }
     __syncthreads();
-    const float* lp = p.logit + (long)b * p.H * p.W;
     for (long i = (long)blockIdx.x * 256 + threadIdx.x; i < n; i += (long)gridDim.x * 256) {
         const int y = (int)lm_fastdiv((unsigned)i, p.div_wc), x = (int)((unsigned)i - (unsigned)y * (unsigned)Wc);
-        const unsigned key = score_key(lp[(long)(y + p.clip) * p.W + x + p.clip]);
+        const unsigned key = score_key(topk_logit<LOWRES>(p, b, y + p.clip, x + p.clip));
         if (LEVEL == 0) {
             atomicAdd(&lh[key >> 20], 1u);
         } else if (LEVEL == 1) {
@@ -222,6 +260,7 @@
     }
 }
 
+template <bool LOWRES>
 __global__ __launch_bounds__(1024) void topk_ties_kernel(TopkParams p) {
     __shared__ unsigned sh[4];
     __shared__ unsigned wave_tot[16];
@@ -240,7 +279,6 @@
     if (hist[2 * NB + bin] == need || need == 0) return;
     const int Wc = p.W - 2 * p.clip;
     const long n = (long)(p.H - 2 * p.clip) * Wc;
-    const float* lp = p.logit + (long)b * p.H * p.W;
     const int lane = threadIdx.x & 63, wave = threadIdx.x >> 6;
     unsigned taken = 0;
     for (long i0 = 0; i0 < n && taken < need; i0 += 1024) {
@@ -248,7 +286,7 @@
         bool tie = false;
         if (i < n) {
             const int y = (int)lm_fastdiv((unsigned)i, p.div_wc), x = (int)((unsigned)i - (unsigned)y * (unsigned)Wc);
-            tie = score_key(lp[(long)(y + p.clip) * p.W + x + p.clip]) == T;
+            tie = score_key(topk_logit<LOWRES>(p, b, y + p.clip, x + p.clip)) == T;
         }
         const unsigned long long m = __ballot(tie);
         const unsigned before = (unsigned)__popcll(m & ((1ull << lane) - 1ull));
@@ -359,41 +397,72 @@
     return LM_OK;
 }
 
+LM_API int lm_decode_semantic_rows_lowres(void* hip_stream, const float* seg_nhwc, int ldx, float* rows, int B, int Hi, int Wi, int Ho,
+                                          int Wo) {
+    LM_REQUIRE(seg_nhwc && rows && ldx >= 3 && B >= 1 && Hi >= 1 && Wi >= 1 && Wo >= 1, "decode_semantic_rows_lowres: bad args");
+    LM_REQUIRE(Ho >= 8 && Ho % 8 == 0, "decode_semantic_rows_lowres: Ho must be a multiple of 8 for the row gather");
+    const long total = (long)B * (Ho / 8) * Wo;
+    LM_REQUIRE(total < (1L << 31), "decode_semantic_rows_lowres: %ld outputs do not fit 32-bit indices", total);
+    hipLaunchKernelGGL(decode_rows_lowres_kernel, dim3(lm_cdiv(total, 256)), dim3(256), 0, (hipStream_t)hip_stream, seg_nhwc, ldx, rows,
+                       Hi, Wi, Ho, Wo, (unsigned)total);
+    LM_LAUNCH_CHECK();
+    return LM_OK;
+}
+
 LM_API long lm_endp_topk_workspace_bytes(int B) {
     return (long)B * (3 * NB * sizeof(unsigned) + sizeof(unsigned) * 4 + (long)CAP * sizeof(unsigned long long));
+}
+
+namespace {
+template <bool LOWRES>
+int launch_endp_topk(hipStream_t s, TopkParams p, void* workspace, int* out_idx, float* out_score, int* out_status, int B) {
+    char* ws = (char*)workspace;
+    p.hist = (unsigned*)ws;
+    p.cand_cnt = (unsigned*)(ws + (size_t)B * 3 * NB * sizeof(unsigned));
+    p.cand = (unsigned long long*)(ws + (size_t)B * (3 * NB + 4) * sizeof(unsigned));
+    p.div_wc = lm_fastdiv_make((unsigned)(p.W - 2 * p.clip));
+    const long zero_words = (long)B * (3 * NB + 4);
+    hipLaunchKernelGGL(zero_u32_kernel, dim3(lm_cdiv(zero_words, 256)), dim3(256), 0, s, (unsigned*)workspace, zero_words);
+    LM_LAUNCH_CHECK();
+    dim3 grid(256, B);
+    hipLaunchKernelGGL((topk_pass_kernel<0, LOWRES>), grid, dim3(256), 0, s, p);
+    LM_LAUNCH_CHECK();
+    hipLaunchKernelGGL((topk_pass_kernel<1, LOWRES>), grid, dim3(256), 0, s, p);
+    LM_LAUNCH_CHECK();
+    hipLaunchKernelGGL((topk_pass_kernel<2, LOWRES>), grid, dim3(256), 0, s, p);
+    LM_LAUNCH_CHECK();
+    hipLaunchKernelGGL((topk_pass_kernel<3, LOWRES>), grid, dim3(256), 0, s, p);
+    LM_LAUNCH_CHECK();
+    hipLaunchKernelGGL(topk_ties_kernel<LOWRES>, dim3(B), dim3(1024), 0, s, p);
+    LM_LAUNCH_CHECK();
+    hipLaunchKernelGGL(topk_sort_kernel, dim3(B), dim3(1024), 0, s, p, out_idx, out_score, out_status);
+    LM_LAUNCH_CHECK();
+    return LM_OK;
+}
 }
 
 LM_API int lm_endp_topk(void* stream, const float* endp_logit, void* workspace, int* out_idx, float* out_score,
                         int* out_status, int B, int H, int W, int clip, int K) {
     LM_REQUIRE(endp_logit && workspace && out_idx && out_score && out_status, "endp_topk: null pointer");
     LM_REQUIRE(K >= 1 && K <= CAP / 2 && H > 2 * clip && W > 2 * clip, "endp_topk: bad K=%d or crop", K);
-    hipStream_t s = (hipStream_t)stream;
-    TopkParams p;
+    LM_REQUIRE(W > 2 * clip && H > 2 * clip && (long)(H - 2 * clip) * (W - 2 * clip) < (1L << 31), "endp_topk: bad crop (H=%d W=%d clip=%d)", H, W, clip);
+    TopkParams p = {};
     p.logit = endp_logit;
-    char* ws = (char*)workspace;
-    p.hist = (unsigned*)ws;
-    p.cand_cnt = (unsigned*)(ws + (size_t)B * 3 * NB * sizeof(unsigned));
-    p.cand = (unsigned long long*)(ws + (size_t)B * (3 * NB + 4) * sizeof(unsigned));
     p.H = H; p.W = W; p.clip = clip; p.K = K;
-    LM_REQUIRE(W > 2 * clip && H > 2 * clip && (long)(H - 2 * clip) * (W - 2 * clip) < (1L << 31), "endp_topk: bad crop (H=%d W=%d clip=%d)", H, W, clip);
-    p.div_wc = lm_fastdiv_make((unsigned)(W - 2 * clip));
-    const long zero_words = (long)B * (3 * NB + 4);
-    hipLaunchKernelGGL(zero_u32_kernel, dim3(lm_cdiv(zero_words, 256)), dim3(256), 0, s, (unsigned*)workspace, zero_words);
-    LM_LAUNCH_CHECK();
-    dim3 grid(256, B);
-    hipLaunchKernelGGL(topk_pass_kernel<0>, grid, dim3(256), 0, s, p);
-    LM_LAUNCH_CHECK();
-    hipLaunchKernelGGL(topk_pass_kernel<1>, grid, dim3(256), 0, s, p);
-    LM_LAUNCH_CHECK();
-    hipLaunchKernelGGL(topk_pass_kernel<2>, grid, dim3(256), 0, s, p);
-    LM_LAUNCH_CHECK();
-    hipLaunchKernelGGL(topk_pass_kernel<3>, grid, dim3(256), 0, s, p);
-    LM_LAUNCH_CHECK();
-    hipLaunchKernelGGL(topk_ties_kernel, dim3(B), dim3(1024), 0, s, p);
-    LM_LAUNCH_CHECK();
-    hipLaunchKernelGGL(topk_sort_kernel, dim3(B), dim3(1024), 0, s, p, out_idx, out_score, out_status);
-    LM_LAUNCH_CHECK();
-    return LM_OK;
+    return launch_endp_topk<false>((hipStream_t)stream, p, workspace, out_idx, out_score, out_status, B);
+}
+
+LM_API int lm_endp_topk_lowres(void* hip_stream, const float* endp_nhwc, int ldx, int Hi, int Wi, void* workspace, int* out_idx,
+                               float* out_score, int* out_status, int B, int H, int W, int clip, int K) {
+    LM_REQUIRE(endp_nhwc && workspace && out_idx && out_score && out_status, "endp_topk_lowres: null pointer");
+    LM_REQUIRE(ldx >= 1 && Hi >= 1 && Wi >= 1 && B >= 1 && clip >= 0, "endp_topk_lowres: bad source (ldx=%d Hi=%d Wi=%d)", ldx, Hi, Wi);
+    LM_REQUIRE(K >= 1 && K <= CAP / 2 && H > 2 * clip && W > 2 * clip && (long)(H - 2 * clip) * (W - 2 * clip) < (1L << 31),
+               "endp_topk_lowres: bad K=%d or crop (H=%d W=%d clip=%d)", K, H, W, clip);
+    TopkParams p = {};
+    p.src = endp_nhwc;
+    p.ld = ldx; p.Hi = Hi; p.Wi = Wi;
+    p.H = H; p.W = W; p.clip = clip; p.K = K;
+    return launch_endp_topk<true>((hipStream_t)hip_stream, p, workspace, out_idx, out_score, out_status, B);
 }
 
 LM_API int lm_pack_segments(void* stream, int n, const void* const* src, const long* bytes, const long* dst_offsets, void* dst) {
diff --git a/lanemapping_amd/csrc/norm_resize.hip b/lanemapping_amd/csrc/norm_resize.hip
--- a/lanemapping_amd/csrc/norm_resize.hip
+++ b/lanemapping_amd/csrc/norm_resize.hip
@@ -497,10 +497,6 @@
     *reinterpret_cast<f32x4*>(y + opix * ldy + c) = o;
 }
 
-__device__ __forceinline__ float upsample_blend(float v00, float v01, float v10, float v11, float wy0, float wy1, float wx0, float wx1) {
-    return lm_bilerp(v00, v01, v10, v11, wy0, wy1, wx0, wx1);
-}
-
 __global__ __launch_bounds__(256) void upsample_to_chw_kernel(const float* __restrict__ x, int ldx, float* __restrict__ y,
                                                               int Hi, int Wi, int Ho, int Wo, int C, long total) {
     const long i = (long)blockIdx.x * 256 + threadIdx.x;
@@ -511,14 +507,11 @@
     t /= Ho;
     const int c = (int)(t % C);
     const int b = (int)(t / C);
-    int y0, y1, x0, x1;
-    float wy0, wy1, wx0, wx1;
+    int y0, y1;
+    float wy0, wy1;
     bilin_axis(oy, Hi, Ho, y0, y1, wy0, wy1);
-    bilin_axis(ox, Wi, Wo, x0, x1, wx0, wx1);
     const float* xb = x + (long)b * Hi * Wi * ldx + c;
-    const float v00 = xb[((long)y0 * Wi + x0) * ldx], v01 = xb[((long)y0 * Wi + x1) * ldx];
-    const float v10 = xb[((long)y1 * Wi + x0) * ldx], v11 = xb[((long)y1 * Wi + x1) * ldx];
-    y[i] = upsample_blend(v00, v01, v10, v11, wy0, wy1, wx0, wx1);
+    y[i] = lm_upsample_sample(xb + (long)y0 * Wi * ldx, xb + (long)y1 * Wi * ldx, ldx, ox, Wi, Wo, wy0, wy1);
 }
 
 __global__ __launch_bounds__(256) void upsample_to_chw4_kernel(const float* __restrict__ x, int ldx, float* __restrict__ y,
@@ -540,13 +533,7 @@
     const float* r1 = xb + (long)y1 * Wi * ldx;
     f32x4 o;
 #pragma unroll
-    for (int k = 0; k < 4; ++k) {
-        int x0, x1;
-        float wx0, wx1;
-        bilin_axis(ox0 + k, Wi, Wo, x0, x1, wx0, wx1);
-        const float v00 = r0[(long)x0 * ldx], v01 = r0[(long)x1 * ldx], v10 = r1[(long)x0 * ldx], v11 = r1[(long)x1 * ldx];
-        o[k] = upsample_blend(v00, v01, v10, v11, wy0, wy1, wx0, wx1);
-    }
+    for (int k = 0; k < 4; ++k) o[k] = lm_upsample_sample(r0, r1, ldx, ox0 + k, Wi, Wo, wy0, wy1);
     *reinterpret_cast<f32x4*>(y + (long)i * 4) = o;
 }
 
diff --git a/lanemapping_amd/net.py b/lanemapping_amd/net.py
--- a/lanemapping_amd/net.py
+++ b/lanemapping_amd/net.py
@@ -16,15 +16,17 @@
         self.heads = build_heads(cfg)
         self.head_type, self.loss_type = head_type, loss_type
 
-    def forward_raw(self, batch):
+    def forward_raw(self, batch, lowres_heads=False):
         fused = hasattr(self.pcencoder, 'fpn') and self.cfg.heads.type == 'ColumnProposal2'
+        if lowres_heads and not fused:
+            raise ValueError('forward_raw(lowres_heads=True) needs the FPN encoder with the ColumnProposal2 head')
         col = None
         if fused:
             proj = batch['proj']
             B, H, W = (proj.shape[0], proj.shape[1], proj.shape[2]) if proj.dtype == torch.uint8 else (proj.shape[0], proj.shape[2], proj.shape[3])
             col = ops.new_act(B, 16, H // 4, W // 4, proj.device)
             with trace.stage('pcencoder'):
-                fea, fea_up, bi_seg, endp_est = self.pcencoder.fpn(proj, fea_up_out=col[:, 8:16])
+                fea, fea_up, bi_seg, endp_est = self.pcencoder.fpn(proj, fea_up_out=col[:, 8:16], lowres_heads=lowres_heads)
         else:
             with trace.stage('pcencoder'):
                 fea, fea_up, bi_seg, endp_est = self.pcencoder(batch)
@@ -36,8 +38,11 @@
                 out = self.heads(fea)
             else:
                 out = self.heads(fea, fea_up, endp_est, col=col) if fused else self.heads(fea, fea_up, endp_est)
-        out['semantic_seg'] = bi_seg
-        out['endp_est'] = endp_est
+        if lowres_heads:
+            out['semantic_seg_lr'], out['endp_est_lr'], out['img_hw'] = bi_seg, endp_est, (H, W)
+        else:
+            out['semantic_seg'] = bi_seg
+            out['endp_est'] = endp_est
         return out
 
     def forward(self, batch, is_get_features=False, stack_local_global_features=False):
diff --git a/lanemapping_amd/ops.py b/lanemapping_amd/ops.py
--- a/lanemapping_amd/ops.py
+++ b/lanemapping_amd/ops.py
@@ -533,6 +533,29 @@
     score = torch.empty((B, K), device=x.device, dtype=torch.float32)
     status = torch.empty((B,), device=x.device, dtype=torch.int32)
     check(lib().lm_endp_topk(_stream(), _ptr(x), _ptr(ws), _ptr(idx), _ptr(score), _ptr(status), B, H, W, clip, K))
+    return idx, score, status
+
+
+def decode_semantic_rows_lowres(seg_lr, size):
+    x, ldx = as_nhwc(seg_lr)
+    B, C_, Hi, Wi = x.shape
+    assert C_ == 3
+    Ho, Wo = size
+    rows = torch.empty((B, Ho // 8, Wo), device=x.device, dtype=torch.float32)
+    check(lib().lm_decode_semantic_rows_lowres(_stream(), _ptr(x), ldx, _ptr(rows), B, Hi, Wi, Ho, Wo))
+    return rows
+
+
+def endp_topk_lowres(endp_lr, size, K=512, clip=20):
+    x, ldx = as_nhwc(endp_lr)
+    B, C_, Hi, Wi = x.shape
+    assert C_ == 1
+    H, W = size
+    ws = torch.empty(lib().lm_endp_topk_workspace_bytes(B), device=x.device, dtype=torch.uint8)
+    idx = torch.empty((B, K), device=x.device, dtype=torch.int32)
+    score = torch.empty((B, K), device=x.device, dtype=torch.float32)
+    status = torch.empty((B,), device=x.device, dtype=torch.int32)
+    check(lib().lm_endp_topk_lowres(_stream(), _ptr(x), ldx, Hi, Wi, _ptr(ws), _ptr(idx), _ptr(score), _ptr(status), B, H, W, clip, K))
     return idx, score, status
 
 
diff --git a/lanemapping_amd/pcencoder.py b/lanemapping_amd/pcencoder.py
--- a/lanemapping_amd/pcencoder.py
+++ b/lanemapping_amd/pcencoder.py
@@ -183,17 +183,18 @@
         terms.append(self._conv_stats(P, s4, conv_b, c_half, gn_b))
         return ops.gn_relu_upsample_sum(terms, P[gn_b + '.g'], P[gn_b + '.b'], (h, w), proj=proj, keep_sum=False)
 
-    def forward(self, x, fea_up_out=None):
+    def forward(self, x, fea_up_out=None, lowres_heads=False):
         from . import torch_ops
         if self.out is None:
-            return self._forward_impl(x, fea_up_out)
+            return self._forward_impl(x, fea_up_out, lowres_heads)
         if fea_up_out is None:
             B, H, W = (x.shape[0], x.shape[1], x.shape[2]) if x.dtype == torch.uint8 else (x.shape[0], x.shape[2], x.shape[3])
             fea_up_out = ops.new_act(B, 8, (H + 3) // 4, (W + 3) // 4, x.device)
-        fea, bi_seg, endp = torch_ops.fpn_encoder(x, fea_up_out, torch_ops.stage_weights(self), torch_ops.stage_name(self))
+        fea, bi_seg, endp = torch_ops.fpn_encoder(x, fea_up_out, torch_ops.stage_weights(self), torch_ops.stage_name(self),
+                                                  bool(lowres_heads))
         return fea, fea_up_out, bi_seg, endp
 
-    def _forward_impl(self, x, fea_up_out=None):
+    def _forward_impl(self, x, fea_up_out=None, lowres_heads=False):
         P = self.packed()
         if x.dtype == torch.uint8:
             B, H, W, _ = x.shape
@@ -241,10 +242,10 @@
         fea_up = self._semantic(P, p2, p3, p4, 'conv2', 'gn12', 'semantic_branch', 'gn11',
                                 (P['feature_layer.w'], P['feature_layer.b'], 8, fea_up_out), pre_a, a4)
         seg288 = ops.conv_small(fea_up, P['output_layer_binary_seg.w'], 3, shift=P['output_layer_binary_seg.b'], pre_relu=True)
-        bi_seg = ops.upsample_to_chw(seg288, (H, W))
+        bi_seg = seg288 if lowres_heads else ops.upsample_to_chw(seg288, (H, W))
         endp288 = self._semantic(P, p2, p3, p4, 'conv3', 'gn22', 'semantic_branch2', 'gn21',
                                  (P['output_layer_endp.w'], P['output_layer_endp.b'], 1, None), pre_b, b4)
-        endp = ops.upsample_to_chw(endp288, (H, W))
+        endp = endp288 if lowres_heads else ops.upsample_to_chw(endp288, (H, W))
         trace.pop()
         return fea, fea_up, bi_seg, endp
 
diff --git a/lanemapping_amd/pipeline.py b/lanemapping_amd/pipeline.py
--- a/lanemapping_amd/pipeline.py
+++ b/lanemapping_amd/pipeline.py
@@ -12,13 +12,15 @@
 
 
 class TilePipeline:
-    def __init__(self, net, host_threads=8, use_graph=None, with_decode_endp=False):
+    def __init__(self, net, host_threads=8, use_graph=None, with_decode_endp=False, fused_decode=None):
         self.with_decode_endp = bool(with_decode_endp)
         self.use_graph = (os.environ.get('LANEMAP_GRAPHS', '0') != '0') if use_graph is None else bool(use_graph)
         self._graphs = collections.OrderedDict()
         self.net = net
         self.cfg = net.cfg
         self.rowref = net.cfg.heads.type == 'RowSharNotReducRef'
+        want_fused = (os.environ.get('LANEMAP_FUSED_DECODE', '1') != '0') if fused_decode is None else bool(fused_decode)
+        self.fused_decode = want_fused and not self.rowref and hasattr(net.pcencoder, 'fpn')
         if net.cfg.heads.type not in ('ColumnProposal2', 'RowSharNotReducRef'):
             raise NotImplementedError(f'TilePipeline has no decode / polyline tail for heads.type={net.cfg.heads.type!r}')
         self.pool = ThreadPoolExecutor(max_workers=host_threads)
@@ -108,7 +110,8 @@
     def _device_part(self, proj):
         heads, cfg = self.net.heads, self.cfg
         batch = proj if isinstance(proj, dict) else ({'points': list(proj)} if isinstance(proj, (list, tuple)) else {'proj': proj})
-        raw = self.net.forward_raw(batch)
+        lowres = self.fused_decode and 'proj' in batch
+        raw = self.net.forward_raw(batch, lowres_heads=True) if lowres else self.net.forward_raw(batch)
         if self.rowref:
             dev = {'col': heads.decode_columns(raw)}
             keep = (raw, dev)
@@ -118,12 +121,19 @@
             prop_conf, v_ext, cls_conf, cls_idx, cls_offset = torch_ops.decode_proposals(
                 raw['proposal_conf'], raw['ext2'], raw['cls2'], raw['offset2'], float(cfg.exist_thre), heads.prop_width, heads.prop_half_buff)
             orient = torch_ops.decode_orient(raw['orient'])
-            sem, biseg, rows = torch_ops.decode_semantic(raw['semantic_seg'], float(cfg.coor_thre))
-            idx, score, status = torch_ops.endp_topk(raw['endp_est'], decode.TOPK, decode.CLIP)
+            if lowres:
+                H, W = raw['img_hw']
+                sem = biseg = None
+                rows = torch_ops.decode_semantic_rows_lowres(raw['semantic_seg_lr'], H, W)
+                idx, score, status = torch_ops.endp_topk_lowres(raw['endp_est_lr'], H, W, decode.TOPK, decode.CLIP)
+                crop = W
+            else:
+                sem, biseg, rows = torch_ops.decode_semantic(raw['semantic_seg'], float(cfg.coor_thre))
+                idx, score, status = torch_ops.endp_topk(raw['endp_est'], decode.TOPK, decode.CLIP)
+                crop = raw['endp_est'].shape[-1]
             trace.pop()
             dev = {'prop_conf': prop_conf, 'v_ext': v_ext, 'cls_offset': cls_offset, 'rows': rows, 'idx': idx, 'status': status}
             keep = (raw, sem, biseg, orient, cls_conf, cls_idx, dev)
-            crop = raw['endp_est'].shape[-1]
         return self._pack(dev), keep, crop
 
     def _tile_task(self, host, b, crop_w):
diff --git a/lanemapping_amd/torch_ops.py b/lanemapping_amd/torch_ops.py
--- a/lanemapping_amd/torch_ops.py
+++ b/lanemapping_amd/torch_ops.py
@@ -179,6 +179,14 @@
 def _endp_topk_fake(endp_logits, K, clip):
     B = endp_logits.shape[0]
     return (endp_logits.new_empty((B, K), dtype=torch.int32), endp_logits.new_empty((B, K)), endp_logits.new_empty((B,), dtype=torch.int32))
+
+
+def _decode_semantic_rows_lowres(seg_lr: Tensor, Ho: int, Wo: int) -> Tensor:
+    return _ops.decode_semantic_rows_lowres(seg_lr, (Ho, Wo))
+
+
+def _endp_topk_lowres(endp_lr: Tensor, H: int, W: int, K: int, clip: int) -> Tuple[Tensor, Tensor, Tensor]:
+    return _ops.endp_topk_lowres(endp_lr, (H, W), K=K, clip=clip)
 
 
 conv2d_mfma = _define('conv2d_mfma', _conv2d_mfma, _conv2d_mfma_fake)
@@ -200,6 +208,9 @@
 decode_orient = _define('decode_orient', _decode_orient,
                         lambda o: o.new_empty((o.shape[0], o.shape[2], o.shape[3]), dtype=torch.uint8))
 endp_topk = _define('endp_topk', _endp_topk, _endp_topk_fake)
+decode_semantic_rows_lowres = _define('decode_semantic_rows_lowres', _decode_semantic_rows_lowres,
+                                      lambda seg_lr, Ho, Wo: seg_lr.new_empty((seg_lr.shape[0], Ho // 8, Wo)))
+endp_topk_lowres = _define('endp_topk_lowres', _endp_topk_lowres, lambda endp_lr, H, W, K, clip: _endp_topk_fake(endp_lr, K, clip))
 
 
 def _bev_raster(points: Tensor, tile_offsets: List[int], params: Tensor, H: int, W: int) -> Tensor:
@@ -218,16 +229,20 @@
     return torch.tensor(rows, dtype=torch.float32)
 
 
-def _fpn_encoder(proj: Tensor, fea_up_out: Tensor, weights: List[Tensor], stage: str) -> Tuple[Tensor, Tensor, Tensor]:
+def _fpn_encoder(proj: Tensor, fea_up_out: Tensor, weights: List[Tensor], stage: str,
+                 lowres_heads: bool = False) -> Tuple[Tensor, Tensor, Tensor]:
     with _with_weights(stage, weights) as m:
-        fea, _, bi_seg, endp = m._forward_impl(proj, fea_up_out)
+        fea, _, bi_seg, endp = m._forward_impl(proj, fea_up_out, lowres_heads)
     return fea, bi_seg, endp
 
 
-def _fpn_encoder_fake(proj, fea_up_out, weights, stage):
+def _fpn_encoder_fake(proj, fea_up_out, weights, stage, lowres_heads=False):
     B, H, W = (proj.shape[0], proj.shape[1], proj.shape[2]) if proj.dtype == torch.uint8 else (proj.shape[0], proj.shape[2], proj.shape[3])
     m = _stage(stage)
     cf = m.out.out_channels if m.out is not None else 256
+    if lowres_heads:
+        h, w = fea_up_out.shape[2], fea_up_out.shape[3]
+        return _fake_act(proj, B, cf, H // 8, W // 8), _fake_act(proj, B, 3, h, w), _fake_act(proj, B, 1, h, w)
     return (_fake_act(proj, B, cf, H // 8, W // 8), proj.new_empty((B, 3, H, W), dtype=torch.float32),
             proj.new_empty((B, 1, H, W), dtype=torch.float32))
 
@@ -310,4 +325,4 @@
 
 OP_NAMES = ['conv2d_mfma', 'conv3x3_winograd44', 'stem_conv7x7', 'maxpool3x3s2', 'gn_stats', 'gn_relu_upsample',
             'upsample_bilinear', 'layernorm_rows', 'attention', 'linear_mfma', 'token_mix', 'tile_ingest', 'decode_proposals', 'decode_semantic',
-            'decode_orient', 'endp_topk', 'bev_raster', 'fpn_encoder', 'vit_backbone', 'mixer_backbone', 'colprop_head', 'endp_cluster', 'polyline_assemble']
+            'decode_orient', 'endp_topk', 'decode_semantic_rows_lowres', 'endp_topk_lowres', 'bev_raster', 'fpn_encoder', 'vit_backbone', 'mixer_backbone', 'colprop_head', 'endp_cluster', 'polyline_assemble']
```
